# RWAlgorithms/ConjugateGradientOptim.jl

Hardware: AMD Instinct MI355X
Metric: CG iterations/sec at n=1e8 (outer iterations of minimizeobjective, PR-CG) (higher is better)
Workload: dtype f64

## Files before the change

conjugategradientoptim.jl_amd/_lib.py:

```python
from __future__ import annotations

import ctypes as C
import os
import subprocess

_PKG = os.path.dirname(os.path.abspath(__file__))
LIB_PATH = os.environ.get("CGO_LIB_PATH") or os.path.join(_PKG, "lib", "libcgo_hip.so")
CSRC = os.path.join(_PKG, "csrc")

dp = C.POINTER(C.c_double)
i64p = C.POINTER(C.c_int64)


class BetaConfig(C.Structure):
    _fields_ = [("kind", C.c_int32), ("lbfgs_m", C.c_int32), ("mu", C.c_double)]


class CGConfigC(C.Structure):
    _fields_ = [("eps", C.c_double), ("beta", BetaConfig), ("max_iters", C.c_int64),
                ("verbose", C.c_int32), ("trace_enabled", C.c_int32)]


class LSConfigC(C.Structure):
    _fields_ = [("kind", C.c_int32), ("cond_kind", C.c_int32), ("c1", C.c_double),
# ... 24 lines not shown

class BatchPolicyC(C.Structure):
    _fields_ = [("size", C.c_int32), ("rows", C.c_int32), ("reserved", C.c_int32 * 6)]


class SolverPolicyC(C.Structure):
    _fields_ = [("size", C.c_int32), ("points", C.c_int32), ("resident", C.c_int32), ("controller_depth", C.c_int32),
                ("controller_graph", C.c_int32), ("controller_fused", C.c_int32), ("stored_gradient", C.c_int32),
                ("fused_tail", C.c_int32), ("strict_tail", C.c_int32), ("placement_search", C.c_int32),
                ("placement_stages", C.c_int32), ("placement_max_bytes", C.c_int64), ("lbfgs_form", C.c_int32),
                ("lbfgs_fuse_grad", C.c_int32), ("lbfgs_fuse_trial", C.c_int32), ("lse_fixed_reference", C.c_int32),
                ("resident_points", C.c_int32), ("resident_chunk", C.c_int32), ("hbm_stream_bytes", C.c_double),
                ("reserved", C.c_int32 * 8)]


class LbfgsProbeC(C.Structure):
    _fields_ = [("pass_", C.c_int32), ("slot", C.c_int32), ("count", C.c_int32), ("list", C.c_int32 * 16),
                ("a", C.c_double), ("a_s", C.c_double), ("a_trial", C.c_double), ("cg", C.c_double), ("M", C.c_double),
                ("S", C.c_double), ("cy", C.c_double * 16), ("cs", C.c_double * 16), ("deferred_push", C.c_int32),
                ("lite_slot", C.c_int32), ("a_lite", C.c_double), ("a_s_lite", C.c_double), ("M_lite", C.c_double),
                ("S_lite", C.c_double), ("loop_mode", C.c_int32), ("final_step", C.c_int32), ("apply_scale", C.c_int32),
                ("k", C.c_int32), ("q_from_g", C.c_int32), ("v_ring", C.c_int32), ("v_slot", C.c_int32), ("w_ring", C.c_int32),
                ("w_slot", C.c_int32), ("dot_count", C.c_int32), ("rho", C.c_double), ("scale", C.c_double),
                ("dot_host", C.c_double), ("dots", dp), ("alpha", C.c_double * 64), ("spec_check", C.c_int32),
                ("spec_slot", C.c_int32), ("spec_count", C.c_int32), ("spec_list", C.c_int32 * 16), ("spec_a_x", C.c_double),
                ("spec_a_s", C.c_double), ("spec_ok", C.c_int32), ("new_in_list", C.c_int32), ("sums_len", C.c_int32),
                ("reserved", C.c_int32), ("gram", C.c_double * 85), ("sums", C.c_double * 64), ("symbol", C.c_char * 256)]


class ResidentPassC(C.Structure):
    _fields_ = [("kind", C.c_int32), ("k", C.c_int32), ("a", C.c_double * 7), ("a_acc", C.c_double), ("beta", C.c_double)]


class ResidentPassOutC(C.Structure):
    _fields_ = [("ts", (C.c_double * 7) * 7), ("gu", C.c_double), ("uu", C.c_double), ("width", C.c_int64)]


class ResidentProbeC(C.Structure):
    _fields_ = [("npass", C.c_int32), ("reserved", C.c_int32), ("pass_", ResidentPassC * 32), ("grid", C.c_int32),
                ("points", C.c_int32), ("chunk", C.c_int64), ("round0", C.c_int64), ("err_word", C.c_uint32),
                ("wrote_back", C.c_int32), ("out", ResidentPassOutC * 32), ("symbol", C.c_char * 128)]


class CtlStateC(C.Structure):
    _fields_ = [("f_x", C.c_double), ("gg", C.c_double), ("a_acc", C.c_double), ("beta", C.c_double), ("a", C.c_double * 7),
                ("npts", C.c_int32), ("go", C.c_int32), ("it", C.c_int64)]


class CtlArgsC(C.Structure):
    _fields_ = [("a_acc", C.c_double), ("beta", C.c_double), ("a", C.c_double * 7), ("go", C.c_int64)]


class CtlRecordC(C.Structure):
    _fields_ = [("sums", C.c_double * 56), ("a_acc", C.c_double), ("beta", C.c_double), ("a", C.c_double * 7),
                ("npts", C.c_int32), ("accepted", C.c_int32), ("xwait", C.c_int64)]


class ArmedProbeC(C.Structure):
    _fields_ = [("rounds", C.c_int32), ("form", C.c_int32), ("use_eps", C.c_int32), ("reserved", C.c_int32),
                ("max_iters", C.c_int64), ("eps", C.c_double), ("st", CtlStateC), ("row", C.c_double * 56),
                ("width", C.c_int32), ("maxp", C.c_int32), ("round_out", C.c_uint64), ("st_out", CtlStateC),
                ("args_out", CtlArgsC), ("out_dev", C.c_double * 56), ("rec", CtlRecordC * 32), ("symbol", C.c_char * 4096)]


class BatchPassC(C.Structure):
    _fields_ = [("kind", C.c_int32), ("k", C.c_int32), ("a", C.c_double * 7), ("a_acc", C.c_double), ("beta", C.c_double),
                ("co_set", C.c_int32), ("co_count", C.c_int32), ("co_gamma", C.c_double), ("co_cy", C.c_double * 10),
                ("co_cs", C.c_double * 10)]


class BatchPassOutC(C.Structure):
    _fields_ = [("ts", (C.c_double * 7) * 7), ("gu", C.c_double), ("uu", C.c_double), ("width", C.c_int64), ("stored", C.c_int64)]


class BatchProbeC(C.Structure):
    _fields_ = [("tier", C.c_int32), ("obj_kind", C.c_int32), ("m", C.c_int32), ("n_params", C.c_int32), ("model", C.c_void_p),
                ("n", C.c_int64), ("batch", C.c_int64), ("x", dp), ("u", dp), ("params", dp * 4), ("scalars", dp),
                ("skip", C.POINTER(C.c_uint8)), ("S", dp), ("Y", dp), ("qn", C.c_void_p), ("npass", C.c_int32),
                ("reserved", C.c_int32), ("pass_", BatchPassC * 32), ("rows", dp), ("out", C.POINTER(BatchPassOutC)),
                ("x_out", dp), ("u_out", dp), ("g_out", dp), ("S_out", dp), ("Y_out", dp), ("qn_out", C.c_void_p),
                ("reason", C.POINTER(C.c_int32)), ("done", i64p), ("passes", i64p), ("points", C.c_int32),
                ("reserved2", C.c_int32), ("ld", C.c_int64), ("symbol", C.c_char * 128)]


ALLGATHER_FN = C.CFUNCTYPE(C.c_int, C.c_void_p, dp, dp, C.c_int32)
FDF_FN = C.CFUNCTYPE(C.c_double, C.c_void_p, dp, dp, C.c_int64)

_vp = C.c_void_p
_pp = C.POINTER(C.c_void_p)
SIGNATURES = {
    "cgo_version": (C.c_int, []),
    "cgo_build_id": (C.c_char_p, []),
    "cgo_last_error": (C.c_char_p, []),
    "cgo_status_name": (C.c_char_p, [C.c_int32]),
    "cgo_device_count": (C.c_int, [C.POINTER(C.c_int32)]),
    "cgo_check_cg_config": (C.c_int, [C.POINTER(CGConfigC)]),
    "cgo_check_ls_config": (C.c_int, [C.POINTER(LSConfigC)]),
    "cgo_ctx_create": (C.c_int, [C.c_int32, _pp]),
    "cgo_solver_policy_init": (None, [C.POINTER(SolverPolicyC)]),
    "cgo_ctx_set_default_policy": (C.c_int, [_vp, C.POINTER(SolverPolicyC)]),
    "cgo_solver_get_policy": (C.c_int, [_vp, C.POINTER(SolverPolicyC)]),
    "cgo_solver_create_ex": (C.c_int, [_vp, _vp, C.POINTER(CGConfigC), C.POINTER(LSConfigC), C.POINTER(SolverPolicyC), _pp]),
    "cgo_solver_create_sys_ex": (C.c_int, [_vp, _vp, C.POINTER(CGConfigC), C.POINTER(LSSConfigC), C.POINTER(SolverPolicyC), _pp]),
    "cgo_ctx_destroy": (C.c_int, [_vp]),
    "cgo_comm_unique_id": (C.c_int, [_vp]),
    "cgo_ctx_set_comm_rccl": (C.c_int, [_vp, C.c_int32, C.c_int32, _vp]),
    "cgo_ctx_set_comm_callback": (C.c_int, [_vp, C.c_int32, C.c_int32, ALLGATHER_FN, _vp]),
    "cgo_ctx_set_comm_shm": (C.c_int, [_vp, C.c_int32, C.c_int32, C.c_char_p, C.c_int32]),
    "cgo_shm_unlink": (C.c_int, [C.c_char_p]),
    "cgo_ctx_comm_info": (C.c_int, [_vp, C.POINTER(C.c_int32), C.POINTER(C.c_int32), C.POINTER(C.c_int32), C.POINTER(C.c_int32)]),
    "cgo_ctx_exchange_stats": (C.c_int, [_vp, i64p, dp, dp, C.c_int32]),
    "cgo_ctx_comm_connect_devices": (C.c_int, [_vp, C.POINTER(C.c_int32)]),
    "cgo_rccl_available": (C.c_int, []),
    "cgo_objective_create": (C.c_int, [_vp, C.c_int32, C.c_int64, C.c_int64, C.c_int64, _pp]),
    "cgo_objective_create_from_source": (C.c_int, [_vp, C.c_char_p, C.c_int32, C.c_int64, C.c_int64, C.c_int64, _pp]),
    "cgo_objective_create_callback": (C.c_int, [_vp, FDF_FN, _vp, C.c_int64, C.c_int64, C.c_int64, _pp]),
    "cgo_objective_destroy": (C.c_int, [_vp]),
    "cgo_objective_create_from_source_ex": (C.c_int, [_vp, C.c_char_p, C.c_int32, C.c_int64, C.c_int64, C.c_int64, _pp]),
    "cgo_objective_num_params": (C.c_int, [_vp, C.POINTER(C.c_int32)]),
    "cgo_objective_set_param_host": (C.c_int, [_vp, C.c_int32, dp]),
    "cgo_objective_set_param_device": (C.c_int, [_vp, C.c_int32, _vp]),
    "cgo_objective_fill_param": (C.c_int, [_vp, C.c_int32, C.c_int32, C.c_uint64, C.c_double, C.c_double]),
    "cgo_objective_set_scalar": (C.c_int, [_vp, C.c_int32, C.c_double]),
    "cgo_objective_set_cost_class": (C.c_int, [_vp, C.c_int32]),
    "cgo_objective_eval_host": (C.c_int, [_vp, dp, dp, dp]),
    "cgo_solver_create": (C.c_int, [_vp, _vp, C.POINTER(CGConfigC), C.POINTER(LSConfigC), _pp]),
    "cgo_solver_destroy": (C.c_int, [_vp]),
    "cgo_solver_set_x0_host": (C.c_int, [_vp, dp]),
    "cgo_solver_set_x0_fill": (C.c_int, [_vp, C.c_int32, C.c_uint64, C.c_double, C.c_double]),
    "cgo_solver_set_x0_device": (C.c_int, [_vp, _vp]),
    "cgo_solver_results_device": (C.c_int, [_vp, _vp, _vp]),
    "cgo_solver_start": (C.c_int, [_vp]),
    "cgo_solver_iterate": (C.c_int, [_vp, C.c_int64, C.POINTER(C.c_int32)]),
    "cgo_solver_results": (C.c_int, [_vp, C.POINTER(ResultsC)]),
    "cgo_solver_trial_log": (C.c_int, [_vp, C.c_int64, dp, dp, dp, i64p]),
    "cgo_solver_profile_enable": (C.c_int, [_vp, C.c_int32]),
    "cgo_solver_profile_reset": (C.c_int, [_vp]),
    "cgo_solver_profile_get": (C.c_int, [_vp, C.c_int32, i64p, dp, dp]),
    "cgo_kernel_kind_name": (C.c_char_p, [C.c_int32]),
    "cgo_solver_kernel_family": (C.c_char_p, [_vp]),
    "cgo_solver_controller_launches": (C.c_int64, [_vp]),
    "cgo_solver_resident_stats": (C.c_int, [_vp, i64p, i64p, i64p]),
    "cgo_solver_lbfgs_stats": (C.c_int, [_vp, i64p, i64p, i64p]),
    "cgo_num_kernel_kinds": (C.c_int, []),
    "cgo_solver_set_lazy_direction": (C.c_int, [_vp, C.c_int32]),
    "cgo_solver_probe_set_beta_prev": (C.c_int, [_vp, C.c_double]),
    "cgo_solver_set_replay_depth": (C.c_int, [_vp, C.c_int32]),
    "cgo_solver_set_lean_sums": (C.c_int, [_vp, C.c_int32]),
    "cgo_solver_set_path_prediction": (C.c_int, [_vp, C.c_int32]),
    "cgo_solver_path_stats": (C.c_int, [_vp, i64p, i64p, i64p, i64p]),
    "cgo_solver_probe_set_path": (C.c_int, [_vp, C.c_int32]),
    "cgo_solver_debug_set_path_skew": (C.c_int, [_vp, C.c_double]),
    "cgo_solver_probe_set_replay": (C.c_int, [_vp, C.c_int32, dp, dp]),
    "cgo_solver_kernel_symbol": (C.c_int, [_vp, C.c_int32, C.c_char_p, C.c_int32]),
    "cgo_evalwolfeconditions": (C.c_int, [C.POINTER(LSConfigC), C.c_double, C.c_double, C.c_double, C.c_double,
                                          C.c_double, C.c_double, C.POINTER(C.c_int32), C.POINTER(C.c_int32)]),
    "cgo_evalbacktrackcondition": (C.c_int, [C.POINTER(LSConfigC), C.c_double, C.c_double, C.c_double, C.c_double,
                                             C.POINTER(C.c_int32)]),
    "cgo_check_lss_config": (C.c_int, [C.POINTER(LSSConfigC)]),
    "cgo_lss_default_max_iters": (C.c_int64, [C.c_double]),
    "cgo_solver_create_sys": (C.c_int, [_vp, _vp, C.POINTER(CGConfigC), C.POINTER(LSSConfigC), _pp]),
    "cgo_solvesystem": (C.c_int, [_vp, _vp, dp, C.POINTER(CGConfigC), C.POINTER(LSSConfigC), C.POINTER(ResultsC)]),
    "cgo_minimize": (C.c_int, [_vp, _vp, dp, C.POINTER(CGConfigC), C.POINTER(LSConfigC), C.POINTER(ResultsC)]),
    "cgo_minimize_rerun": (C.c_int, [_vp, _vp, dp, C.POINTER(CGConfigC), C.POINTER(LSConfigC),
                                     C.POINTER(CGConfigC), C.POINTER(LSConfigC), C.c_int32,
                                     C.POINTER(ResultsC), C.POINTER(C.c_int32)]),
    "cgo_minimize_batch": (C.c_int, [_vp, C.c_int32, C.c_int64, C.c_int64, dp, dp, C.POINTER(CGConfigC), C.POINTER(LSConfigC),
                                     C.c_int64, C.POINTER(BatchResultsC)]),
    "cgo_batch_max_n": (C.c_int64, [_vp, C.c_int32]),
    "cgo_minimize_batch_obj": (C.c_int, [_vp, _vp, C.c_int64, dp, C.POINTER(dp), C.c_int32, C.POINTER(CGConfigC), C.POINTER(LSConfigC),
                                         C.c_int64, C.POINTER(BatchResultsC)]),
    "cgo_batch_max_n_obj": (C.c_int64, [_vp]),
    "cgo_batch_open": (C.c_int, [_vp, _vp, C.c_int64, C.POINTER(dp), C.c_int32, C.POINTER(_vp)]),
    "cgo_batch_solve": (C.c_int, [_vp, dp, dp, C.POINTER(C.c_uint8), C.POINTER(CGConfigC), C.POINTER(LSConfigC), C.c_int64,
                                  C.POINTER(BatchResultsC)]),
    "cgo_batch_close": (C.c_int, [_vp]),
    "cgo_batch_policy_init": (None, [C.POINTER(BatchPolicyC)]),
    "cgo_minimize_batch_ex": (C.c_int, [_vp, C.c_int32, C.c_int64, C.c_int64, dp, dp, C.POINTER(CGConfigC), C.POINTER(LSConfigC),
                                        C.c_int64, C.POINTER(BatchPolicyC), C.POINTER(BatchResultsC), C.POINTER(C.c_int32)]),
    "cgo_minimize_batch_obj_ex": (C.c_int, [_vp, _vp, C.c_int64, dp, C.POINTER(dp), C.c_int32, C.POINTER(CGConfigC), C.POINTER(LSConfigC),
                                            C.c_int64, C.POINTER(BatchPolicyC), C.POINTER(BatchResultsC), C.POINTER(C.c_int32)]),
    "cgo_batch_open_ex": (C.c_int, [_vp, _vp, C.c_int64, C.POINTER(dp), C.c_int32, C.POINTER(BatchPolicyC), C.POINTER(_vp)]),
    "cgo_batch_rows": (C.c_int, [_vp, C.POINTER(C.c_int32)]),
    "cgo_batch_max_n_ex": (C.c_int64, [_vp, C.c_int32, C.POINTER(BatchPolicyC)]),
    "cgo_batch_max_n_obj_ex": (C.c_int64, [_vp, C.POINTER(BatchPolicyC)]),
    "cgo_batch_rows_shape": (None, [C.POINTER(C.c_int32), C.POINTER(C.c_int32)]),
    "cgo_minimize_batch_lbfgs": (C.c_int, [_vp, C.c_int32, C.c_int64, C.c_int64, dp, dp, C.POINTER(CGConfigC), C.POINTER(LSConfigC),
                                           C.c_int64, C.POINTER(BatchResultsC)]),
    "cgo_batch_lbfgs_max_m": (C.c_int32, []),
    "cgo_batch_lbfgs_max_n": (C.c_int64, [_vp, C.c_int32]),
    "cgo_batch_lbfgs_shape": (None, [C.POINTER(C.c_int32), C.POINTER(C.c_int32)]),
    "cgo_minimize_batch_lbfgs_obj": (C.c_int, [_vp, _vp, C.c_int64, dp, C.POINTER(dp), C.c_int32, dp, C.POINTER(CGConfigC), C.POINTER(LSConfigC),
                                               C.c_int64, C.POINTER(BatchResultsC)]),
    "cgo_batch_lbfgs_max_n_obj": (C.c_int64, [_vp]),
    "cgo_batch_lbfgs_shape_obj": (None, [C.c_int32, C.POINTER(C.c_int32), C.POINTER(C.c_int32)]),
    "cgo_minimize_batch_lbfgs_ex": (C.c_int, [_vp, C.c_int32, C.c_int64, C.c_int64, dp, dp, C.POINTER(CGConfigC), C.POINTER(LSConfigC),
                                              C.c_int64, C.POINTER(BatchPolicyC), C.POINTER(BatchResultsC), C.POINTER(C.c_int32)]),
    "cgo_minimize_batch_lbfgs_obj_ex": (C.c_int, [_vp, _vp, C.c_int64, dp, C.POINTER(dp), C.c_int32, dp, C.POINTER(CGConfigC),
                                                  C.POINTER(LSConfigC), C.c_int64, C.POINTER(BatchPolicyC), C.POINTER(BatchResultsC),
                                                  C.POINTER(C.c_int32)]),
    "cgo_batch_lbfgs_max_n_ex": (C.c_int64, [_vp, C.c_int32, C.c_int32, C.POINTER(BatchPolicyC)]),
    "cgo_batch_lbfgs_max_n_obj_ex": (C.c_int64, [_vp, C.c_int32, C.POINTER(BatchPolicyC)]),
    "cgo_batch_lbfgs_lds_rows": (C.c_int32, [C.c_int32, C.c_int32]),
    "cgo_batch_lbfgs_lds_shape": (None, [C.c_int32, C.POINTER(C.c_int32), C.POINTER(C.c_int32)]),
    "cgo_batch_lbfgs_open": (C.c_int, [_vp, _vp, C.c_int64, C.POINTER(dp), C.c_int32, C.c_int32, C.POINTER(BatchPolicyC), C.POINTER(_vp)]),
    "cgo_batch_lbfgs_solve": (C.c_int, [_vp, dp, dp, C.POINTER(C.c_uint8), C.POINTER(CGConfigC), C.POINTER(LSConfigC), C.c_int64,
                                        C.POINTER(BatchResultsC)]),
    "cgo_batch_lbfgs_m": (C.c_int, [_vp, C.POINTER(C.c_int32)]),
    "cgo_batch_probe": (C.c_int, [_vp, C.POINTER(BatchProbeC)]),
    "cgo_batch_probe_qn_bytes": (C.c_int64, []),
    "cgo_stop_status": (C.c_int32, [C.c_int64, C.c_int64, C.c_double, C.c_double, C.c_double, C.c_double, i64p]),
    "cgo_kernel_dir": (C.c_int, [_vp, dp, dp, C.c_double, C.c_int64, dp]),
    "cgo_kernel_beta_partials": (C.c_int, [_vp, dp, dp, dp, C.c_int64, dp]),
    "cgo_getbeta": (C.c_int, [_vp, C.POINTER(BetaConfig), dp, dp, dp, C.c_int64, dp]),
    "cgo_kernel_trial": (C.c_int, [_vp, dp, dp, C.c_double, dp, dp]),
    "cgo_bench_kernel": (C.c_int, [_vp, _vp, C.c_int32, C.c_int64, C.c_int32, dp, dp]),
    "cgo_bench_stream_mix": (C.c_int, [_vp, C.c_int64, C.c_int32, dp, dp]),
    "cgo_solver_placement_info": (C.c_int, [_vp, dp, dp, C.POINTER(C.c_int32)]),
    "cgo_solver_probe_launch": (C.c_int, [_vp, C.c_int32, C.c_int32, C.c_double, C.c_double, dp, C.c_int32, dp, dp, dp,
                                          dp, C.c_int32, C.POINTER(C.c_int32), dp, dp, dp, C.c_char_p, C.c_int32]),
    "cgo_solver_probe_lbfgs": (C.c_int, [_vp, C.POINTER(LbfgsProbeC)] + [dp] * 13),
    "cgo_solver_probe_resident": (C.c_int, [_vp, C.POINTER(ResidentProbeC), dp, dp, dp, C.c_int64, dp, dp]),
    "cgo_solver_probe_armed": (C.c_int, [_vp, C.POINTER(ArmedProbeC), dp, dp, dp, dp]),
}


class CgoError(RuntimeError):
    def __init__(self, code: int, msg: str):
        super().__init__(f"[cgo error {code}] {msg}")
        self.code = code
        self.msg = msg


def build(force: bool = False) -> str:
    if force:
        subprocess.run(["make", "-C", CSRC, "clean", "-s"], check=True)
    subprocess.run(["make", "-C", CSRC, "-s", "-j4"], check=True)
    if not os.path.exists(LIB_PATH):
        raise RuntimeError("hipcc build did not produce " + LIB_PATH)
    return LIB_PATH


_lib = None


def lib() -> C.CDLL:
    global _lib
    if _lib is None:
        if not os.path.exists(LIB_PATH):
            raise ImportError(
                f"{LIB_PATH} is missing: build it with `make -C {CSRC}` "
                "(or __graft_entry__.build()). There is no CPU fallback.")
        L = C.CDLL(LIB_PATH, mode=C.RTLD_GLOBAL)
        for name, (res, args) in SIGNATURES.items():
            fn = getattr(L, name)
            fn.restype = res
            fn.argtypes = args
        _lib = L
    return _lib


def check(rc: int) -> None:
    if rc != 0:
        msg = lib().cgo_last_error()
        text = msg.decode("utf-8", "replace") if msg else ""
        if rc == 1 and text.startswith("AssertionError"):
            raise AssertionError(text[len("AssertionError: "):])
        raise CgoError(rc, text)
```

conjugategradientoptim.jl_amd/api.py:

```python
from __future__ import annotations

import ctypes as C
import math
import re
from dataclasses import dataclass, field
from typing import List, Optional, Sequence, Union

import numpy as np

from . import _lib
from ._lib import BetaConfig, CGConfigC, LSConfigC, LSSConfigC, ResultsC, check, dp, i64p



class TraceTrait:
    pass


class EnableTrace(TraceTrait):
    def __repr__(self):
        return "EnableTrace()"


class DisableTrace(TraceTrait):
# ... 488 lines not shown
    slots = _param_list(param)
    if slots is not None:
        assert len(slots) <= MAX_PARAM_SLOTS, f"at most {MAX_PARAM_SLOTS} parameter vectors"
        o = DeviceObjective("user", n, ctx, source=source, n_params=len(slots))
        for j, p in enumerate(slots):
            if p is not None:
                o.set_param(np.asarray(p, dtype=np.float64), slot=j)
        param = None
    else:
        o = DeviceObjective("user", n, ctx, source=source, has_param=param is not None)
    if param is not None:
        o.set_param(np.asarray(param, dtype=np.float64))
    if cheap:
        check(_lib.lib().cgo_objective_set_cost_class(o._h, 1))
    return o


def Booth(ctx: Optional[Context] = None) -> DeviceObjective:
    return DeviceObjective("booth", 2, ctx)


def _dev_ptr(t, n: int):
    if t is None:
        return None
    if isinstance(t, int):
        return C.c_void_p(t)
    if hasattr(t, "data_ptr"):
        import torch
        if t.dtype != torch.float64 or not t.is_contiguous() or t.numel() != n or not t.is_cuda:
            raise ValueError(f"device vector must be a contiguous float64 GPU tensor of {n} elements")
        return C.c_void_p(t.data_ptr())
    raise TypeError("expected a torch.Tensor on the GPU or a raw device pointer")


LBFGS_FORMS = {"auto": 0, "one_pass": 1, "one_pass_own_update": 2, "gram": 3, "two_loop": 4}


@dataclass
class SolverPolicy:
    points: Optional[int] = None
    resident: Optional[bool] = None
    controller_depth: Optional[int] = None
    controller_graph: Optional[bool] = None
    controller_fused: Optional[bool] = None
    stored_gradient: Optional[bool] = None
    fused_tail: Optional[bool] = None
    strict_tail: Optional[bool] = None
    placement_search: Optional[bool] = None
    placement_stages: Optional[int] = None
    placement_max_bytes: Optional[int] = None
    lbfgs_form: Optional[str] = None
    lbfgs_fuse_grad: Optional[bool] = None
    lbfgs_fuse_trial: Optional[bool] = None
    lse_fixed_reference: Optional[bool] = None
    resident_points: Optional[int] = None
    resident_chunk: Optional[int] = None
    hbm_stream_bytes: Optional[float] = None

    def _c(self) -> "_lib.SolverPolicyC":
        c = _lib.SolverPolicyC()
        _lib.lib().cgo_solver_policy_init(C.byref(c))
        tri = lambda v: -1 if v is None else (1 if v else 0)
        c.points = self.points or 0
        c.resident = tri(self.resident)
        c.controller_depth = -1 if self.controller_depth is None else int(self.controller_depth)
        c.controller_graph, c.controller_fused = tri(self.controller_graph), tri(self.controller_fused)
        c.stored_gradient = 1 if self.stored_gradient else 0
        c.fused_tail, c.strict_tail = tri(self.fused_tail), tri(self.strict_tail)
        c.placement_search = tri(self.placement_search)
        c.placement_stages = self.placement_stages or 0
        c.placement_max_bytes = int(self.placement_max_bytes or 0)
        c.lbfgs_form = LBFGS_FORMS[self.lbfgs_form or "auto"]
        c.lbfgs_fuse_grad, c.lbfgs_fuse_trial = tri(self.lbfgs_fuse_grad), tri(self.lbfgs_fuse_trial)
        c.lse_fixed_reference = tri(self.lse_fixed_reference)
        c.resident_points = self.resident_points or 0
        c.resident_chunk = self.resident_chunk or 0
        c.hbm_stream_bytes = float(self.hbm_stream_bytes or 0.0)
        return c


class Solver:
    def __init__(self, fdf: DeviceObjective, config: CGConfig, linesearch_config: LineSearchConfig,
                 policy: Optional[SolverPolicy] = None):
        if not isinstance(fdf, DeviceObjective):
            raise TypeError(
                "fdf! must be an objective descriptor: a device objective (QuadDiag, RosenbrockPaired, Booth, "
                "ElementwiseObjective, ...) or HostObjective(closure, n) — there is no CPU solver path in this package")
        self.obj, self.config, self.ls = fdf, config, linesearch_config
        self._cfg_c, self._ls_c = config._c(), linesearch_config._c()
        self._h = C.c_void_p()
        create = (_lib.lib().cgo_solver_create_sys_ex if isinstance(linesearch_config, LinesearchSolveSys)
                  else _lib.lib().cgo_solver_create_ex)
        self._pol_c = policy._c() if policy is not None else None
        check(create(fdf.ctx._h, fdf._h, C.byref(self._cfg_c), C.byref(self._ls_c),
                     C.byref(self._pol_c) if self._pol_c is not None else None, C.byref(self._h)))

    def policy(self) -> dict:
        c = _lib.SolverPolicyC()
        check(_lib.lib().cgo_solver_get_policy(self._h, C.byref(c)))
        return {n: getattr(c, n) for n, _ in c._fields_ if n not in ("size", "reserved")}

    def set_x0(self, x_initial_global: np.ndarray):
        loc = self.obj.local(np.asarray(x_initial_global, dtype=np.float64))
        check(_lib.lib().cgo_solver_set_x0_host(self._h, loc.ctypes.data_as(dp)))

    def set_x0_fill(self, fill: str, lo: float, hi: float = 0.0, seed: int = 0):
        check(_lib.lib().cgo_solver_set_x0_fill(self._h, FILL_KINDS[fill], seed, lo, hi))

    def set_x0_device(self, x0):
        check(_lib.lib().cgo_solver_set_x0_device(self._h, _dev_ptr(x0, self.obj.n_local)))

    def results_device(self, minimizer=None, gradient=None):
        check(_lib.lib().cgo_solver_results_device(self._h, _dev_ptr(minimizer, self.obj.n_local), _dev_ptr(gradient, self.obj.n_local)))

    def start(self):
        check(_lib.lib().cgo_solver_start(self._h))

    def iterate(self, iters: int) -> bool:
        fin = C.c_int32(0)
        check(_lib.lib().cgo_solver_iterate(self._h, iters, C.byref(fin)))
        return bool(fin.value)

    def enable_trial_log(self):
        cnt = C.c_int64()
        check(_lib.lib().cgo_solver_trial_log(self._h, -1, None, None, None, C.byref(cnt)))

    def trial_log(self):
        cnt = C.c_int64()
        check(_lib.lib().cgo_solver_trial_log(self._h, 0, None, None, None, C.byref(cnt)))
        k = cnt.value
        a, p, d = np.zeros(max(k, 1)), np.zeros(max(k, 1)), np.zeros(max(k, 1))
        check(_lib.lib().cgo_solver_trial_log(self._h, k, a.ctypes.data_as(dp), p.ctypes.data_as(dp),
                                              d.ctypes.data_as(dp), C.byref(cnt)))
        return a[:k], p[:k], d[:k]

    def kernel_family(self) -> str:
        return _lib.lib().cgo_solver_kernel_family(self._h).decode()

    def kernel_symbol(self, kind_name: str) -> str:
        L = _lib.lib()
        buf = C.create_string_buffer(200)
        for k in range(L.cgo_num_kernel_kinds()):
            if L.cgo_kernel_kind_name(k).decode() == kind_name:
                check(L.cgo_solver_kernel_symbol(self._h, k, buf, 200))
                return buf.value.decode()
        return ""

    def set_lazy_direction(self, on: bool = True):
        check(_lib.lib().cgo_solver_set_lazy_direction(self._h, int(bool(on))))

    def set_replay_depth(self, d: int):
        check(_lib.lib().cgo_solver_set_replay_depth(self._h, int(d)))

    def set_lean_sums(self, on: bool):
        check(_lib.lib().cgo_solver_set_lean_sums(self._h, int(bool(on))))

    def set_path_prediction(self, on: bool):
        check(_lib.lib().cgo_solver_set_path_prediction(self._h, int(bool(on))))

    def path_stats(self):
        by = (C.c_int64 * 8)()
        p, t, m = C.c_int64(0), C.c_int64(0), C.c_int64(0)
        check(_lib.lib().cgo_solver_path_stats(self._h, by, C.byref(p), C.byref(t), C.byref(m)))
        return dict(by_nact={j: int(by[j]) for j in (1, 2, 3, 4, 5, 7)}, predicted=p.value, tree=t.value, misses=m.value)

    def debug_set_path_skew(self, factor: float):
        check(_lib.lib().cgo_solver_debug_set_path_skew(self._h, float(factor)))

    def probe_launch(self, kind_name: str, variant: int, a_acc: float, beta: float, a: Sequence[float], x, u=None, aux=None,
                     beta_prev: Optional[float] = None, replay: Optional[Sequence] = None, path_nact: Optional[int] = None):
        L = _lib.lib()
        kk = [L.cgo_kernel_kind_name(k).decode() for k in range(L.cgo_num_kernel_kinds())].index(kind_name)
        if beta_prev is not None:
            check(L.cgo_solver_probe_set_beta_prev(self._h, float(beta_prev)))
        if replay is not None:
            ra = np.ascontiguousarray([p[0] for p in replay], dtype=np.float64)
            rb = np.ascontiguousarray([p[1] for p in replay], dtype=np.float64)
            check(L.cgo_solver_probe_set_replay(self._h, len(replay), ra.ctypes.data_as(dp), rb.ctypes.data_as(dp)))
        if path_nact is not None:
            check(L.cgo_solver_probe_set_path(self._h, int(path_nact)))
        n = self.obj.n_local
        vec = lambda v: None if v is None else np.ascontiguousarray(v, dtype=np.float64)
        x, u, aux = vec(x), vec(u), vec(aux)
        for v in (x, u, aux):
            if v is not None and v.size != n:
                raise ValueError(f"probe vectors hold n_local = {n} elements")
        av = np.ascontiguousarray(a, dtype=np.float64) if len(a) else np.zeros(1)
        sums, ln = np.full(64, np.nan), C.c_int32(0)
        xo, uo, go = np.empty(n), np.empty(n), np.empty(n)
        sym = C.create_string_buffer(200)
        ptr = lambda v: None if v is None else v.ctypes.data_as(dp)
        check(L.cgo_solver_probe_launch(self._h, kk, int(variant), float(a_acc), float(beta), ptr(av), len(a), ptr(x), ptr(u),
                                        ptr(aux), ptr(sums), 64, C.byref(ln), ptr(xo), ptr(uo), ptr(go), sym, 200))
        return dict(sums=sums[:ln.value].copy(), x=xo, u=uo, g=go, symbol=sym.value.decode())

    LBFGS_PASSES = ("push", "push_gram", "direction_gram", "direction_trial", "push_lite", "loop")

    def probe_lbfgs(self, pass_name: str, x=None, u=None, g=None, gt=None, S=None, Y=None, **kw):
        n = self.obj.n_local
        P = self._cfg_c.beta.lbfgs_m + 1
        vec = lambda v: None if v is None else np.ascontiguousarray(v, dtype=np.float64)
        x, u, g, gt = vec(x), vec(u), vec(g), vec(gt)
        for v in (x, u, g, gt):
            if v is not None and v.size != n:
                raise ValueError(f"probe vectors hold n_local = {n} elements")
        S = None if S is None else np.ascontiguousarray(S, dtype=np.float64).reshape(P, n)
        Y = None if Y is None else np.ascontiguousarray(Y, dtype=np.float64).reshape(P, n)
        p = _lib.LbfgsProbeC()
        p.pass_ = self.LBFGS_PASSES.index(pass_name)
        dots = None
        for key, val in kw.items():
            if key in ("list", "spec_list"):
                getattr(p, key)[:len(val)] = [int(v) for v in val]
                setattr(p, "count" if key == "list" else "spec_count", len(val))
            elif key in ("cy", "cs", "alpha"):
                getattr(p, key)[:len(val)] = [float(v) for v in val]
            elif key == "stats":
                p.M, p.S = float(val[0]), float(val[1])
            elif key == "dots":
                dots = np.ascontiguousarray(val, dtype=np.float64).reshape(-1, 10)
                p.dots, p.dot_count = dots.ctypes.data_as(dp), dots.shape[0]
            else:
                if not hasattr(p, key):
                    raise TypeError(f"probe_lbfgs: no field {key}")
                setattr(p, key, val)
        outs = {k: np.full(n, np.nan) for k in ("x", "xo", "u", "g", "gt")}
        So, Yo = np.full((P, n), np.nan), np.full((P, n), np.nan)
        ptr = lambda v: None if v is None else v.ctypes.data_as(dp)
        check(_lib.lib().cgo_solver_probe_lbfgs(self._h, C.byref(p), ptr(x), ptr(u), ptr(g), ptr(gt), ptr(S), ptr(Y),
                                                *[ptr(outs[k]) for k in ("x", "xo", "u", "g", "gt")], ptr(So), ptr(Yo)))
        sym = p.symbol.decode()
        return dict(sums=np.array(p.sums[:p.sums_len]), S=So, Y=Yo, alpha=np.array(p.alpha[:]), symbols=sym.split(" + ") if sym else [],
                    new_in_list=p.new_in_list, spec_ok=bool(p.spec_ok),
                    gram=np.array(p.gram[:5 + 5 * p.spec_count]) if p.spec_ok else None, **outs)

    def probe_resident(self, script, x, u):
        n = self.obj.n_local
        x, u = np.ascontiguousarray(x, dtype=np.float64), np.ascontiguousarray(u, dtype=np.float64)
        if x.size != n or u.size != n:
            raise ValueError(f"probe vectors hold n_local = {n} elements")
        p = _lib.ResidentProbeC()
        if len(script) > 32:
            raise ValueError("probe_resident: at most 32 passes")
        p.npass = len(script)
        for q, item in enumerate(script):
            c = p.pass_[q]
            if item[0] == "trial":
                c.kind, a = 0, item[1]
            elif item[0] == "accept_dir_trial":
                c.kind, c.a_acc, c.beta, a = 1, float(item[1]), float(item[2]), item[3]
            else:
                raise ValueError(f"probe_resident: no pass kind {item[0]!r}")
            if len(a) > 7:
                raise ValueError("probe_resident: at most 7 trial steps")
            c.k = len(a)
            c.a[:len(a)] = [float(v) for v in a]
        rows = np.full((max(p.npass, 1), 256, 56), np.nan)
        xo, uo = np.empty(n), np.empty(n)
        check(_lib.lib().cgo_solver_probe_resident(self._h, C.byref(p), x.ctypes.data_as(dp), u.ctypes.data_as(dp),
                                                   rows.ctypes.data_as(dp), rows.size, xo.ctypes.data_as(dp), uo.ctypes.data_as(dp)))
        g = p.grid
        got = rows.ravel()[:p.npass * g * 56].reshape(p.npass, g, 56)
        outs, rws, tails = [], [], []
        for q in range(p.npass):
            w = int(p.out[q].width)
            rws.append(got[q, :, :w].copy()); tails.append(got[q, :, w:].copy())
            outs.append(dict(ts=np.array([list(r) for r in p.out[q].ts]), gu=p.out[q].gu, uu=p.out[q].uu))
        return dict(rows=rws, tail=tails, out=outs, grid=g, chunk=p.chunk, points=p.points, round0=p.round0,
                    wrote_back=bool(p.wrote_back), x=xo, u=uo, symbol=p.symbol.decode())

    ARMED_FORMS = ("rounds", "graph", "controller")

    def probe_armed(self, state, rounds=1, form="rounds", x=None, u=None, max_iters=1 << 40, eps=None, row=None):
        n = self.obj.n_local
        p = _lib.ArmedProbeC()
        p.rounds, p.form = int(rounds), self.ARMED_FORMS.index(form)
        p.max_iters = int(max_iters)
        if eps is not None:
            p.use_eps, p.eps = 1, float(eps)
        a = [float(v) for v in state["a"]]
        if not 1 <= len(a) <= 7:
            raise ValueError("probe_armed: 1 to 7 trial steps")
        p.st.f_x, p.st.gg = float(state["f_x"]), float(state["gg"])
        p.st.a_acc, p.st.beta = float(state["a_acc"]), float(state["beta"])
        p.st.a[:] = a + [a[-1]] * (7 - len(a))
        p.st.npts, p.st.go, p.st.it = int(state.get("npts", len(a))), int(state.get("go", 1)), int(state.get("it", 0))
        if row is not None:
            r = [float(v) for v in row]
            p.row[:len(r)] = r
        vec = lambda v: None if v is None else np.ascontiguousarray(v, dtype=np.float64)
        x, u = vec(x), vec(u)
        for v in (x, u):
            if v is not None and v.size != n:
                raise ValueError(f"probe vectors hold n_local = {n} elements")
        xo, uo = np.full(n, np.nan), np.full(n, np.nan)
        ptr = lambda v: None if v is None else v.ctypes.data_as(dp)
        check(_lib.lib().cgo_solver_probe_armed(self._h, C.byref(p), ptr(x), ptr(u), ptr(xo), ptr(uo)))

        def block(c, names):
            d = {k: (np.array(getattr(c, k)[:]) if k in ("a", "sums") else getattr(c, k)) for k in names}
            d["bytes"] = bytes(c)
            return d
        recs = [block(p.rec[r], ("sums", "a_acc", "beta", "a", "npts", "accepted", "xwait")) for r in range(p.rounds)]
        sym = p.symbol.decode()
        return dict(records=recs, st=block(p.st_out, ("f_x", "gg", "a_acc", "beta", "a", "npts", "go", "it")),
                    args=block(p.args_out, ("a_acc", "beta", "a", "go")), round=int(p.round_out), out_dev=np.array(p.out_dev[:]),
                    width=p.width, maxp=p.maxp, x=xo, u=uo, symbols=sym.split(" + ") if sym else [])

    def placement_info(self):
        a, b, c = C.c_double(), C.c_double(), C.c_int32()
        check(_lib.lib().cgo_solver_placement_info(self._h, C.byref(a), C.byref(b), C.byref(c)))
        return a.value, b.value, c.value

    def controller_launches(self) -> int:
        return int(_lib.lib().cgo_solver_controller_launches(self._h))

    def resident_stats(self):
        a, b, c = C.c_int64(), C.c_int64(), C.c_int64()
        check(_lib.lib().cgo_solver_resident_stats(self._h, C.byref(a), C.byref(b), C.byref(c)))
        self.resident_gave_up = c.value
        return a.value, b.value

    def lbfgs_stats(self):
        a, b, c = C.c_int64(), C.c_int64(), C.c_int64()
        check(_lib.lib().cgo_solver_lbfgs_stats(self._h, C.byref(a), C.byref(b), C.byref(c)))
        return a.value, b.value, c.value

    def profile(self, on: bool = True):
        check(_lib.lib().cgo_solver_profile_enable(self._h, int(on)))

    def profile_reset(self):
        check(_lib.lib().cgo_solver_profile_reset(self._h))

# ... 995 lines not shown
```

conjugategradientoptim.jl_amd/csrc/cgo_backend_cg.hip:

```cpp
#include "cgo_backend_internal.hpp"

#include "cgo_kernels.hip.hpp"
#include "cgo_kernels_cg.hip.hpp"
#include "cgo_kernels_cg_path.hip.hpp"
#include "cgo_kernels_chain.hip.hpp"
#include "cgo_kernels_lse.hip.hpp"
#include "cgo_kernels_resident.hip.hpp"

namespace cgo {

using namespace dev;

double bytes_r(int obj_kind, int mode, int64_t n, int n_params) {
    const int p = std::max(obj_kind == CGO_OBJ_QUAD_DIAG ? 1 : 0, n_params);
    return 8.0 * (double)n * (double)r_vectors(mode, p);
}

template <int N> using Pts = std::integral_constant<int, N>;
template <int MAXPTS, class F>
static inline void with_points(int npts, F f) {
    static_assert(MAXPTS == 1 || MAXPTS == 3 || MAXPTS == 5 || MAXPTS == 7, "a launch evaluates 1, 3, 5 or 7 trial points");
    if constexpr (MAXPTS >= 3) { if (npts == 3) return f(Pts<3>{}); }
    if constexpr (MAXPTS >= 5) { if (npts == 5) return f(Pts<5>{}); }
    if constexpr (MAXPTS >= 7) { if (npts != 1) return f(Pts<7>{}); }
    return f(Pts<1>{});
}

template <class Obj, bool BIG>
static int launch_cg(int mode, int npts, const RParams &P, int grid, hipStream_t st) {
#define ROW(MODE, MAXPTS) if (mode == (MODE) && P.tail.ctl) { with_points<MAXPTS>(npts, [&](auto n) { k_cg_armed<Obj, decltype(n)::value><<<grid, BLOCK, 0, st>>>(P); }); return 0; }
    CGO_CG_ARMED_ROWS(ROW)
#undef ROW
    switch (mode) {
#define ROW(MODE, MAXPTS) case (MODE): with_points<MAXPTS>(npts, [&](auto n) { k_cg<Obj, (MODE), decltype(n)::value, BIG><<<grid, BLOCK, 0, st>>>(P); }); return 0;
    CGO_CG_ROWS(ROW)
#undef ROW
    default: break;
    }
    if constexpr (BIG) {
        switch (mode) {
#define ROW(MODE, MAXPTS) case (MODE): with_points<MAXPTS>(npts, [&](auto n) { k_cg<Obj, (MODE), decltype(n)::value, true><<<grid, BLOCK, 0, st>>>(P); }); return 0;
        CGO_CG_LAG_ROWS(ROW)
        CGO_CG_REPLAY_ROWS(ROW)
        CGO_CG_LEAN_ROWS(ROW)
#undef ROW
        default: break;
        }
    }
    return -1;
}

template <class Obj>
static int launch_cg_path(int mode, int nact, const RParams &P, int grid, hipStream_t st) {
#define ROW(MODE, NACT) if (mode == (MODE) && nact == (NACT)) { k_cg_path<Obj, (MODE), (NACT), true><<<grid, BLOCK, 0, st>>>(P); return 0; }
    CGO_CG_PATH_ROWS(ROW)
#undef ROW
    return -1;
}
static inline bool path_row(int mode, int nact) {
#define ROW(MODE, NACT) if (mode == (MODE) && nact == (NACT)) return true;
    CGO_CG_PATH_ROWS(ROW)
#undef ROW
    return false;
}
static inline bool path_objective(int kind) {
#define ROW(KIND, T) if (kind == KIND) return true;
    CGO_OBJ_CURV_ROWS(ROW)
#undef ROW
    return false;
}
bool HipBackend::path_rows() const {
    if (!path_on_ || !path_objective(obj_->kind) || replay_depth_ < 2 || !lazy_eligible()) return false;
    const int mode_n = r_mode_of(KK_ACCEPT_TRIAL_NOSTORE), mode_s = R_REPLAY | R_ADT;
    return path_row(mode_n | lean_for(mode_n), MAXP) && path_row(mode_s | lean_for(mode_s), MAXP);
}

static inline bool lean_row(int mode) {
#define ROW(MODE, MAXPTS) if (mode == (MODE)) return true;
    CGO_CG_LEAN_ROWS(ROW)
#undef ROW
    return false;
}
int HipBackend::lean_for(int mode) const { return (lean_bits_ && lean_row(mode | lean_bits_)) ? lean_bits_ : 0; }

void unpack_r(const double *s, int k, Scal *out, bool dir, int npts) {
    if (npts == 0) npts = npts_for(k);
    for (int j = 0; j < k; ++j) {
        const double *q = s + RS_PER_POINT * j;
        out[j].f = q[RS_F]; out[j].gtu = q[RS_GTU]; out[j].gtgt = q[RS_GTGT]; out[j].gtg = q[RS_GTG];
        out[j].yy = q[RS_YY]; out[j].uy = q[RS_UY]; out[j].ygt = q[RS_YGT];
    }
    if (dir) { out[0].gu = s[RS_PER_POINT * npts]; out[0].uu = s[RS_PER_POINT * npts + 1]; }
}

static inline int chain_npts(int mode, int npts) { return ((mode & R_TRIAL) && npts >= 3) ? 3 : 1; }

RPlan HipBackend::r_plan(int mode, int npts) const {
    const double bytes = bytes_r(obj_->kind, mode, obj_->n_local, obj_->nparams());
    const bool big = r_big_only(mode) || bytes > big_bytes(r_read_only(mode));
    return {big, big ? GRID_BIG : grid_cg(obj_->n_local, chain() ? 1 : npts), chain() ? chain_npts(mode, npts) : npts, bytes};
}
bool HipBackend::adt_is_big() const { return bytes_r(obj_->kind, R_ADT, obj_->n_local, obj_->nparams()) > big_bytes(false); }

int HipBackend::launch_r(int kk, int mode, double a_acc, double beta, const double *a, int k, bool fetch,
                         double *sums) {
    if (int rc = pipe_drain()) return rc;
    pipe_streak_ = 0;
    if (u_lag_ && !(mode & R_ULAG)) {
        if (r_reads_u(mode)) { if (int rc = materialize_u()) return rc; }
        else if (mode & (R_INIT | R_RESET)) u_lag_ = false;
    }
    if (rep_n_ > 0 && !(mode & R_REPLAY)) { if (int rc = materialize_lag()) return rc; }
    RPlan plan;
    const int npts = path_nact_ ? MAXP : npts_for(k);
    if (int rc = launch_r_kernel(kk, mode, a_acc, beta, a, k, npts, nullptr, &plan)) return rc;
    const int grid = plan.grid;
    total_launches_++;
    const bool has_sums = r_has_sums(mode);
    const bool fused = has_sums && tail_fused(grid);
    if (has_sums && chain()) {
        const bool three = plan.npts == 3;
        const int W = three ? NRC3 : NRC, edge = three ? RC3_EDGE : RC_EDGE, nsums = three ? NR : NR1;
        if (!fused) { if (int rc = finalize_rows(ctx_, grid, W, true)) return rc; }
        const int Wd = ctx_->world(), me = ctx_->rank();
        std::vector<double> raw((size_t)W * Wd);
        double all[NRC3];
        if (int rc = fetch_sums(ctx_, all, MERGE_SUM, W, raw.data())) return rc;
        if (sums) std::memcpy(sums, all, sizeof(double) * nsums);
        if (me > 0) {
            const double *e = raw.data() + (size_t)(me - 1) * W + edge + 4;
            halo_xl_[0] = e[0]; halo_xl_[1] = e[1]; halo_ul_[0] = e[2]; halo_ul_[1] = e[3];
        }
        if (me < Wd - 1) {
            const double *e = raw.data() + (size_t)(me + 1) * W + edge;
            halo_xr_[0] = e[0]; halo_xr_[1] = e[1]; halo_ur_[0] = e[2]; halo_ur_[1] = e[3];
        }
        if (probe_) { std::memcpy(probe_row_, all, sizeof(double) * W); probe_len_ = W; }
    } else if (has_sums) {
        if (!fused) { if (int rc = finalize_rows(ctx_, grid, rows_for(npts), true)) return rc; }
        if (fetch) {
            if (int rc = fetch_sums(ctx_, sums, MERGE_SUM, rows_for(npts))) return rc;
        }
        if (probe_ && fetch) { std::memcpy(probe_row_, sums, sizeof(double) * rows_for(npts)); probe_len_ = rows_for(npts); }
    }
    if (prof_on_) prof_commit(kk, plan.bytes);
    return CGO_OK;
}

bool HipBackend::lazy_eligible() const {
    if (!lazy_on_ || !rmode_ || chain() || sys_on_ || probe_ || pingpong_ == 1) return false;
    bool aot = false;
#define ROW(KIND, T) aot = aot || obj_->kind == KIND;
    CGO_OBJ_ROWS(ROW)
#undef ROW
    if (!aot) return false;
    if (const char *e = getenv("CGO_PINGPONG")) { if (e[0] == '1') return false; }
    if (ctl_depth() > 0) return false;
    return adt_is_big() && r_plan(R_TRIAL, 1).big;
}

int HipBackend::materialize_u() {
    if (!u_lag_) return CGO_OK;
    const int64_t asked = total_launches_;
    const int nact = path_nact_;
    path_nact_ = 0;
    const int rc = launch_rk(KK_MATERIALIZE_U, 0.0, 0.0, nullptr, 0, false, nullptr);
    path_nact_ = nact;
    total_launches_ = asked;
    if (rc) return rc;
    u_lag_ = false;
    return CGO_OK;
}

int HipBackend::materialize_lag() {
    if (int rc = materialize_u()) return rc;
    if (rep_n_ == 0) return CGO_OK;
    const int64_t asked = total_launches_;
    const int nact = path_nact_;
    path_nact_ = 0;
    const int rc = launch_rk(KK_MATERIALIZE_XU, 0.0, 0.0, nullptr, 0, false, nullptr);
    path_nact_ = nact;
    total_launches_ = asked;
    if (rc) return rc;
    rep_n_ = 0;
    return CGO_OK;
}

int HipBackend::set_replay_depth_now(int d) {
    if (d < 1 || d > RMAX + 1) { set_error("replay depth: 1 … 8"); return CGO_EINVAL; }
    if (d != replay_depth_) { if (int rc = materialize_lag()) return rc; }
    replay_depth_ = d;
    return CGO_OK;
}

void HipBackend::set_probe_replay(int nrep, const double *a, const double *beta) {
    probe_rep_n_ = std::max(0, std::min(nrep, (int)RMAX));
    for (int j = 0; j < probe_rep_n_; ++j) { probe_rep_a_[j] = a[j]; probe_rep_b_[j] = beta[j]; }
}

int HipBackend::accept_dir_trial_r(double a_acc, double beta, const double *a, int k, double *s) {
    if (!lazy_eligible()) return launch_rk(KK_ACCEPT_DIR_TRIAL, a_acc, beta, a, k, true, s);
    if (replay_depth_ >= 2) {
        if (int rc = materialize_u()) return rc;
        if (rep_n_ < replay_depth_ - 1 && rep_n_ < RMAX) {
            const int mode_n = r_mode_of(KK_ACCEPT_TRIAL_NOSTORE);
            if (int rc = launch_r(KK_ACCEPT_TRIAL_NOSTORE, mode_n | lean_for(mode_n), a_acc, beta, a, k, true, s)) return rc;
            if (path_nact_) { path_last_n_ = path_nact_; path_count_[path_nact_]++; }
            rep_a_[rep_n_] = a_acc; rep_b_[rep_n_] = beta; rep_n_++;
            return CGO_OK;
        }
        const int mode_s = R_REPLAY | R_ADT;
        if (int rc = launch_r(KK_ACCEPT_DIR_TRIAL, mode_s | lean_for(mode_s), a_acc, beta, a, k, true, s)) return rc;
        if (path_nact_) { path_last_s_ = path_nact_; path_count_[path_nact_]++; }
        rep_n_ = 0;
        return CGO_OK;
    }
    if (!u_lag_) {
        if (int rc = launch_rk(KK_ACCEPT_TRIAL_LAZY, a_acc, beta, a, k, true, s)) return rc;
        u_lag_ = true; beta_lag_ = beta;
        return CGO_OK;
    }
    if (int rc = launch_r(KK_ACCEPT_DIR_TRIAL, R_ULAG | R_ADT, a_acc, beta, a, k, true, s)) return rc;
    u_lag_ = false;
    return CGO_OK;
}
int HipBackend::trial_r(const double *a, int k, double *s) {
    if (rep_n_ > 0 && lazy_eligible()) return launch_r(KK_TRIAL, R_REPLAY | R_TRIAL, 0, 0, a, k, true, s);
    if (u_lag_ && lazy_eligible()) return launch_r(KK_TRIAL, R_ULAG | R_TRIAL, 0, 0, a, k, true, s);
    return launch_rk(KK_TRIAL, 0, 0, a, k, true, s);
}

bool HipBackend::pipe_fused(int grid) const {
    return tail_fused(grid) && obj_->kind != CGO_OBJ_USER && !chain() && ctl_fused_;
}
bool HipBackend::tail_fused(int grid) const {
    static const int cap = [] { const char *e = getenv("CGO_FUSED_TAIL_MAX_GRID"); int v = e ? atoi(e) : 0; return v > 0 ? v : 1024; }();
    return ctx_->fused_tail && grid <= cap && grid <= TAIL_GROUP * TAIL_GROUP;
}
Tail HipBackend::make_tail(bool on) {
    Tail t{};
    if (!on) return t;
    ctx_->seq++;
    t.partials2 = ctx_->partials2_f; t.tickets = ctx_->tickets; t.out = ctx_->out_dev;
    t.strict = ctx_->tail_strict ? 1 : 0;
    ctx_->pub_target(&t.host_out, &t.host_seq);
    ctx_->pub_checked = (t.host_out != nullptr) && !ctx_->tail_strict;
    t.seq = ctx_->seq;
    return t;
}

int HipBackend::launch_r_kernel(int kk, int mode, double a_acc, double beta, const double *a, int k, int npts,
                                const CtlArgs *ctl, RPlan *plan_out) {
    HIPCHK(hipSetDevice(ctx_->device));
    if (obj_->unset_slot() >= 0) return param_unset_error(obj_->unset_slot());
    const int64_t n = obj_->n_local;
    if (mode & (R_GRAD | R_GRADT)) { if (int rc = ensure_ga()) return rc; }
    const bool has_sums = r_has_sums(mode);
    const RPlan plan = *plan_out = r_plan(mode, npts);
    const bool big = plan.big; const int grid = plan.grid;
    last_mode_ = mode; last_npts_ = plan.npts; last_big_ = big; last_nact_ = path_nact_;
    if (path_nact_ && (chain() || !big || ctl || !path_row(mode, path_nact_) || !path_objective(obj_->kind))) { set_error("internal: not a path row"); return CGO_EINVAL; }
    if (chain()) {
        if (int rc = prof_begin(kk)) return rc;
        if (int rc = launch_chain_kernel(mode, a_acc, beta, a, k, plan.npts, big, grid, make_tail(has_sums && !ctl && tail_fused(grid)))) return rc;
        return prof_end();
    }
    RParams P;
    P.x = xc_; P.u = uc_; P.gout = ga_.p; obj_->param_args(P); P.n = n;
    P.xo = xc_; P.uo = uc_;
    P.a_acc = a_acc; P.beta = beta; P.s0 = obj_->s0; P.partials = ctx_->partials;
    P.beta_prev = beta_lag_;
    P.nrep = (mode & R_REPLAY) ? rep_n_ : 0;
    for (int j = 0; j < RMAX; ++j) { P.ra[j] = j < P.nrep ? rep_a_[j] : 0.0; P.rb[j] = j < P.nrep ? rep_b_[j] : 0.0; }
    P.ctl = ctl;
    P.x2 = xn_;
    for (int j = 0; j < MAXP; ++j) P.a[j] = (a && j < k) ? a[j] : ((a && k > 0) ? a[k - 1] : 0.0);
    P.tail = make_tail(has_sums && !ctl && tail_fused(grid));
    if (ctl && pipe_fused(grid)) {
        P.tail.partials2 = ctx_->partials2_f; P.tail.tickets = ctx_->tickets; P.tail.out = ctx_->out_dev;
        P.tail.strict = ctx_->tail_strict ? 1 : 0;
        P.tail.ctl = ctl_dev_; P.tail.ctl_rec = ctl_rec_; P.tail.ctl_seq = ctl_seq_;
        if (!ctx_->single()) {
            P.tail.xw = ctx_->world(); P.tail.xme = ctx_->rank(); P.tail.xseq0 = epoch_ << 40;
            for (int r = 0; r < P.tail.xw && r < 8; ++r) P.tail.xmail[r] = ctx_->comm->dev_mailbox(r);
        }
    }
    if (P.tail.tickets) P.partials = ctx_->partials_f;
    const bool wr_x = r_writes_x(mode), wr_u = r_writes_u(mode);
    const bool pp = big && !ctl && (wr_x || wr_u) && !(mode & R_PROJ) && pingpong_ready();
    if (pp && wr_x) P.xo = xalt_;
    if (pp && wr_u) P.uo = ualt_;
    if (mode == R_PROJ && !xn_) { set_error("internal: no second iterate buffer"); return CGO_ESTATE; }
    hipStream_t st = ctx_->stream;
    if (int rc = prof_begin(kk)) return rc;
    int r = -2;
    if (path_nact_) {
        switch (obj_->kind) {
#define ROW(KIND, T) case KIND: r = launch_cg_path<T>(mode, path_nact_, P, grid, st); break;
        CGO_OBJ_CURV_ROWS(ROW)
#undef ROW
        default: break;
        }
    } else switch (obj_->kind) {
#define ROW(KIND, T) case KIND: r = big ? launch_cg<T, true>(mode, npts, P, grid, st) : launch_cg<T, false>(mode, npts, P, grid, st); break;
    CGO_OBJ_ROWS(ROW)
#undef ROW
    case CGO_OBJ_USER:
        if (!obj_->rtc) { set_error("user objective has no compiled module"); return CGO_EINVAL; }
        if (r_big_only(mode)) break;
        if (int rc = launch_module(obj_->rtc->cg(mode, npts, big), &P, grid, st)) return rc;
        r = 0;
        break;
    default: break;
    }
    if (r) { set_error("internal: CG kernel mode not instantiated"); return CGO_EINVAL; }
    HIPCHK(hipGetLastError());
    if (pp && wr_x) std::swap(xc_, xalt_);
    if (pp && wr_u) std::swap(uc_, ualt_);
    return prof_end();
}

template <bool BIG>
static int launch_chain(int mode, int npts, const ChainParams &P, int grid, hipStream_t st) {
    switch (mode) {
#define ROW(MODE, MAXPTS) case (MODE): with_points<MAXPTS>(npts, [&](auto n) { k_chain<(MODE), decltype(n)::value, BIG><<<grid, BLOCK, 0, st>>>(P); }); return 0;
    CGO_CHAIN_ROWS(ROW)
#undef ROW
    default: return -1;
    }
}

int HipBackend::launch_chain_kernel(int mode, double a_acc, double beta, const double *a, int k, int npts, bool big, int grid, const Tail &tail) {
    ChainParams P;
    P.tail = tail;
    for (int j = 0; j < 3; ++j) P.a[j] = (a && j < k) ? a[j] : ((a && k > 0) ? a[k - 1] : 0.0);
    P.x = xc_; P.u = uc_; P.xo = xc_; P.uo = uc_; P.gout = ga_.p;
    P.odd = (int)(obj_->n_local & 1);
    P.n = obj_->n_local + P.odd; P.a_acc = a_acc; P.beta = beta; P.partials = tail.tickets ? ctx_->partials_f : ctx_->partials;
    for (int j = 0; j < 2; ++j) { P.hxl[j] = halo_xl_[j]; P.hul[j] = halo_ul_[j]; P.hxr[j] = halo_xr_[j]; P.hur[j] = halo_ur_[j]; }
    P.has_left = obj_->offset > 0 ? 1 : 0;
    P.has_right = obj_->offset + obj_->n_local < obj_->n_global ? 1 : 0;
    const bool wr_x = r_writes_x(mode), wr_u = r_writes_u(mode);
    if (wr_x) P.xo = xalt_;
    if (wr_u) P.uo = ualt_;
    const int r = big ? launch_chain<true>(mode, npts, P, grid, ctx_->stream) : launch_chain<false>(mode, npts, P, grid, ctx_->stream);
    if (r) { set_error("internal: chain kernel mode not instantiated"); return CGO_EINVAL; }
    HIPCHK(hipGetLastError());
    if (wr_x) std::swap(xc_, xalt_);
    if (wr_u) std::swap(uc_, ualt_);
    return CGO_OK;
}

std::string HipBackend::r_symbol(int mode, int npts, bool big, int nact) const {
    char buf[160];
    if (chain()) snprintf(buf, sizeof buf, "k_chain<%d, %d, %s>", mode, npts, big ? "true" : "false");
    else if (nact) snprintf(buf, sizeof buf, "k_cg_path<%s, %d, %d, true>", obj_tname(), mode, nact);
    else snprintf(buf, sizeof buf, "k_cg<%s, %d, %d, %s>", obj_tname(), mode, npts, big ? "true" : "false");
    return buf;
}

std::string HipBackend::kernel_symbol(int kk) const {
    if (!rmode_) {
        if (obj_->two_phase() || kk == KK_LBFGS_PUSH || kk == KK_LBFGS_LOOP || kk == KK_LBFGS_FINAL) return lbfgs_symbol(kk);
        const int mode = fused_mode(kk);
        return mode < 0 ? "" : fused_symbol(obj_tname(), mode, is_big(obj_->kind, mode, obj_->n_local, obj_->nparams(), pol_.hbm_stream_bytes));
    }
    const RKind *rk = r_kind(kk);
    if (!rk) return "";
    int mode = rk->mode;
    const bool lazy = lazy_eligible();
    switch (kk) {
    case KK_ACCEPT_DIR_TRIAL: if (lazy) mode |= replay_depth_ >= 2 ? R_REPLAY : R_ULAG; break;
    case KK_ACCEPT_TRIAL_LAZY: case KK_MATERIALIZE_U: if (!lazy || replay_depth_ >= 2) return ""; break;
    case KK_ACCEPT_TRIAL_NOSTORE: case KK_MATERIALIZE_XU: if (!lazy || replay_depth_ < 2) return ""; break;
    default: break;
    }
    const RPlan plan = r_plan(mode, rk->pts == PTS_ONE ? 1 : npts_for(rk->pts == PTS_MAX ? max_points() : std::min(max_points(), 3)));
    if ((mode & R_REPLAY) && (mode & R_ACCEPT)) mode |= lean_for(mode);
    if ((mode & R_REPLAY) && (mode & R_ACCEPT) && path_rows()) {
        const int last = kk == KK_ACCEPT_TRIAL_NOSTORE ? path_last_n_ : path_last_s_;
        return r_symbol(mode, plan.npts, plan.big, last ? last : MAXP);
    }
    return r_symbol(mode, plan.npts, plan.big);
}


__global__ void k_ctl_init(CtlDev *d, const CtlConfig cfg, const CtlState st, unsigned long long round) {
    d->cfg = cfg;
    d->st = st;
    d->round = round;
    d->args = ctl_args_of(st);
}



template <int N, int THREADS>
__global__ __launch_bounds__(THREADS) void k_finalize_ctl(const double *partials, int rows, double *out, CtlDev *d,
                                                          CtlRecord *rec_ring, unsigned long long *seq_ring) {
    constexpr int G = BLOCK / N;
    constexpr int WD = sizeof(CtlDev) / 8, WR = sizeof(CtlRecord) / 8;
    __shared__ double sm[G][N];
    __shared__ double fin[CTL_NSUMS];
    __shared__ CtlDev sd;
    __shared__ CtlRecord sr;
    const int tid = threadIdx.x;
    if (tid < WD) ((unsigned long long *)&sd)[tid] = ((const unsigned long long *)d)[tid];
    if (tid < CTL_NSUMS) fin[tid] = 0.0;
    __syncthreads();
    const bool go = sd.st.go != 0;
    const unsigned long long round = sd.round, seq = round + 1;
    CtlRecord *rec_host = rec_ring + (round % PIPE_RING);
    unsigned long long *seq_host = seq_ring + (round % PIPE_RING);
    if (go) {
        if (tid < G * N) {
            double t = 0.0;
            const long long total = (long long)rows * N;
            for (long long i = tid; i < total; i += G * N) t += partials[i];
            sm[tid / N][tid % N] = t;
        }
        __syncthreads();
        if (tid < N) {
            double v = 0.0;
#pragma unroll
            for (int g = 0; g < G; ++g) v += sm[g][tid];
            out[tid] = v;
            fin[tid] = v;
        }
        __syncthreads();
    }
    if (tid == 0) {
        if (go) {
            ctl_step(sd.cfg, sd.st, fin, sr);
            sd.args = ctl_args_of(sd.st);
        } else ctl_idle_record(sr);
        sd.round = round + 1;
    }
    __syncthreads();
    if (go && tid < WD) ((unsigned long long *)d)[tid] = ((const unsigned long long *)&sd)[tid];
    if (!go && tid == 0) d->round = round + 1;
    if (tid < WR) {
        ((unsigned long long *)rec_host)[tid] = ((const unsigned long long *)&sr)[tid];
        __threadfence_system();
    }
    __syncthreads();
    if (tid == 0) __hip_atomic_store(seq_host, seq, __ATOMIC_RELEASE, __HIP_MEMORY_SCOPE_SYSTEM);
}

int HipBackend::ctl_depth() const {
    if (!(rmode_ && ctx_->host_publish && !obj_->two_phase())) return 0;
    if (ctx_->single()) return ctl_depth_;
    if (!ctx_->dev_exchange() || ctx_->force_gather) return 0;
    return (!adt_is_big() && pipe_fused(grid_cg(obj_->n_local, policy_points()))) ? ctl_depth_ : 0;
}

int HipBackend::pipe_alloc() {
    if (ctl_dev_) return CGO_OK;
    HIPCHK(hipMalloc(&ctl_dev_, sizeof(CtlDev)));
    HIPCHK(hipHostMalloc((void **)&ctl_rec_, sizeof(CtlRecord) * PIPE_RING, hipHostMallocDefault));
    HIPCHK(hipHostMalloc((void **)&ctl_seq_, sizeof(unsigned long long) * PIPE_RING, hipHostMallocDefault));
    std::memset(ctl_rec_, 0, sizeof(CtlRecord) * PIPE_RING);
    std::memset(ctl_seq_, 0, sizeof(unsigned long long) * PIPE_RING);
    pipe_prof_.assign(PIPE_RING, {-1, 0u});
    return CGO_OK;
}

int HipBackend::prepare_controller() {
    if (ctl_depth() <= 0) return CGO_OK;
    if (int rc = pipe_alloc()) return rc;
    if (obj_->unset_slot() >= 0) return CGO_OK;
    HIPCHK(hipSetDevice(ctx_->device));
    CtlConfig cc{};
    CtlState st{};
    st.go = 0;
    pipe_npts_ = max_points();
    k_ctl_init<<<1, 1, 0, ctx_->stream>>>((CtlDev *)ctl_dev_, cc, st, pipe_enq_);
    HIPCHK(hipGetLastError());
    if (int rc = pipe_enqueue_round()) return rc;
    return pipe_drain();
}

int HipBackend::pipe_round_kernels() {
    RPlan plan;
    const int npts = pipe_npts_, ns = rows_for(npts);
    CtlDev *d = (CtlDev *)ctl_dev_;
    if (int rc = launch_r_kernel(KK_ACCEPT_DIR_TRIAL, R_ADT, 0.0, 0.0, nullptr, 0, npts, &d->args, &plan)) return rc;
    const int grid = plan.grid;
    pipe_checked_ = pipe_fused(grid) && !ctx_->tail_strict;
    if (pipe_fused(grid)) {
        if (probe_) probe_note(nullptr, 0, "k_cg_armed<%s, %d>", obj_tname(), last_npts_);
        return CGO_OK;
    }
    if (probe_) probe_note(nullptr, 0, "%s", r_symbol(last_mode_, last_npts_, last_big_).c_str());
    hipStream_t st = ctx_->stream;
    const double *src = ctx_->partials;
    int nrows = grid;
    if (grid > TAIL_GROUP) {
        const int nb = (grid + TAIL_GROUP - 1) / TAIL_GROUP;
        with_width<NR, NR5, NR7, NS>(ns, true, [&](auto w) { k_finalize_t<decltype(w)::value, BLOCK><<<nb, BLOCK, 0, st>>>(ctx_->partials, TAIL_GROUP, grid, ctx_->partials2, nullptr, nullptr, 0); });
        HIPCHK(hipGetLastError());
        if (probe_) probe_note(nullptr, 0, "k_finalize_t<%d>", ns);
        src = ctx_->partials2;
        nrows = nb;
    }
    return pipe_finalize_ctl(src, nrows, ns);
}

int HipBackend::pipe_finalize_ctl(const double *src, int nrows, int ns) {
    CtlDev *d = (CtlDev *)ctl_dev_;
    CtlRecord *rec = (CtlRecord *)ctl_rec_;
    hipStream_t st = ctx_->stream;
    with_width<NR, NR5, NR7, NS>(ns, true, [&](auto w) { constexpr int N = decltype(w)::value, T = N == NS ? BLOCK : 768; k_finalize_ctl<N, T><<<1, T, 0, st>>>(src, nrows, ctx_->out_dev, d, rec, ctl_seq_); });
    HIPCHK(hipGetLastError());
    if (probe_) probe_note(nullptr, 0, "k_finalize_ctl<%d>", ns);
    return CGO_OK;
}

int HipBackend::pipe_enqueue_round() {
    if (int rc = pipe_round_kernels()) return rc;
    const int idx = (int)(pipe_enq_ % PIPE_RING);
    pipe_prof_[idx] = {prof_cur_ ? ring_used_ - 1 : -1, prof_gen_};
    prof_cur_ = false;
    pipe_enq_++;
    return CGO_OK;
}

int HipBackend::pipe_launch_graph(int rounds) {
    HIPCHK(hipSetDevice(ctx_->device));
    PipeGraph *g = nullptr;
    for (auto &c : graphs_)
        if (c.rounds == rounds && c.npts == pipe_npts_ && c.x == xc_ && c.u == uc_ && c.p0 == obj_->p[0].p && c.n == obj_->n_local) { g = &c; break; }
    if (!g) {
        hipStream_t st = ctx_->stream;
        hipGraph_t graph = nullptr;
        capturing_ = true;
        const size_t syms0 = probe_syms_.size();
// ... 38 lines not shown
}

int HipBackend::pipe_wait(unsigned long long id, CtlRecord &rec) {
    const int idx = (int)(id % PIPE_RING);
    if (pipe_checked_) {
        static_assert(sizeof(CtlRecord) % 8 == 0, "record = 8-byte words");
        constexpr int WR = (int)(sizeof(CtlRecord) / 8);
        double words[WR];
        if (int rc = wait_checked(ctx_, ctl_seq_ + idx, id + 1, reinterpret_cast<const double *>(ctl_rec_) + (size_t)idx * WR, WR, words)) return rc;
        std::memcpy(&rec, words, sizeof(CtlRecord));
        if (rec.npts >= 0 && !ctx_->single()) {
            ctx_->xch_count++; ctx_->xch_dev_ms += (double)rec.xwait * 1e-5; ctx_->xch_dev_n++;
        }
        return CGO_OK;
    }
    if (int rc = wait_word(ctx_, ctl_seq_ + idx, id + 1)) return rc;
    rec = ((CtlRecord *)ctl_rec_)[idx];
    return CGO_OK;
}

int HipBackend::pipe_drain() {
    while (pipe_done_ < pipe_enq_) {
        CtlRecord rec;
        if (int rc = pipe_wait(pipe_done_, rec)) return rc;
        pipe_done_++;
        if (rec.npts >= 0) {
            set_error("internal: the on-device controller ran a launch the host state machine did not ask for");
            return CGO_ESTATE;
        }
    }
    return CGO_OK;
}

int HipBackend::accept_dir_trial_ctl(const CtlConfig &cc, const CtlState &s0, int64_t rounds, Scal *out) {
    if (ctl_depth() <= 0) return accept_dir_trial(s0.a_acc, s0.beta, s0.a, s0.npts, out);
    if (int rc = pipe_alloc()) return rc;
    const int64_t ahead = std::min<int64_t>(std::min<int64_t>(ctl_depth_, pipe_streak_), rounds - 1);
    if (pipe_done_ == pipe_enq_) {
        if (ahead <= 0) { pipe_streak_++; return accept_dir_trial_keep_streak(s0, out); }
        HIPCHK(hipSetDevice(ctx_->device));
        pipe_npts_ = cc.maxp;
        k_ctl_init<<<1, 1, 0, ctx_->stream>>>((CtlDev *)ctl_dev_, cc, s0, pipe_enq_);
        HIPCHK(hipGetLastError());
        pipe_stopped_ = false;
        if (int rc = pipe_enqueue(1 + ahead)) return rc;
    }
    CtlRecord rec;
    const unsigned long long id = pipe_done_;
    if (int rc = pipe_wait(id, rec)) return rc;
    pipe_done_++;
    if (rec.npts < 0) {
        if (int rc = pipe_drain()) return rc;
        pipe_streak_++;
        return accept_dir_trial_keep_streak(s0, out);
    }
    if (std::memcmp(&rec.a_acc, &s0.a_acc, 8) || std::memcmp(&rec.beta, &s0.beta, 8) || rec.npts != s0.npts ||
        std::memcmp(rec.a, s0.a, 8 * (size_t)s0.npts)) {
        set_error("internal: the on-device controller and the host state machine disagree on a launch");
        return CGO_ESTATE;
    }
    unpack_r(rec.sums, s0.npts, out, true, pipe_npts_);
    total_launches_++;
    pipe_served_++;
    pipe_streak_++;
    const auto &pp = pipe_prof_[(int)(id % PIPE_RING)];
    if (prof_on_) {
        prof_cnt_[KK_ACCEPT_DIR_TRIAL]++;
        prof_bytes_[KK_ACCEPT_DIR_TRIAL] = bytes_r(obj_->kind, R_ADT, obj_->n_local, obj_->nparams());
        if (pp.first >= 0 && pp.second == prof_gen_ && pp.first < ring_used_) {
            ring_[pp.first].kk = KK_ACCEPT_DIR_TRIAL;
            ring_[pp.first].bytes = prof_bytes_[KK_ACCEPT_DIR_TRIAL];
        }
    }
    if (!rec.accepted) pipe_stopped_ = true;
    if (!pipe_stopped_) {
        const int64_t want = std::min<int64_t>(std::min<int64_t>(ctl_depth_, pipe_streak_), rounds - 1);
        const int64_t have = (int64_t)(pipe_enq_ - pipe_done_);
        if (have < want && (want - have >= (want + 1) / 2 || have == 0))
            if (int rc = pipe_enqueue(want - have)) return rc;
    }
    return CGO_OK;
}

int HipBackend::accept_dir_trial_keep_streak(const CtlState &s0, Scal *out) {
    const int64_t keep = pipe_streak_;
    const int rc = accept_dir_trial(s0.a_acc, s0.beta, s0.a, s0.npts, out);
    pipe_streak_ = keep;
    return rc;
}



int HipBackend::probe_prepare() {
    if (probe_) return CGO_OK;
    if (int rc = pipe_drain()) return rc;
    u_lag_ = false; rep_n_ = 0;
    HIPCHK(hipSetDevice(ctx_->device));
    HIPCHK(hipStreamSynchronize(ctx_->stream));
    (void)pingpong_ready();
    const size_t n = (size_t)obj_->n_local, na = n + (chain() ? (n & 1) : 0), np = probe_padded(na);
    DevBuf *bufs[] = {&x_, &u_, &x2_, &u2_, &ga_, &gb_};
    for (DevBuf *b : bufs) {
        if (b == &x2_ || b == &u2_) { if (pingpong_ != 1) continue; }
        if (int rc = b->alloc(np)) return rc;
        HIPCHK(hipMemsetAsync(b->p, 0, na * sizeof(double), ctx_->stream));
        HIPCHK(hipMemsetD32Async((hipDeviceptr_t)(b->p + na), (int)PROBE_NAN32, (np - na) * 2, ctx_->stream));
    }
    for (int j = 0; j < obj_->nparams(); ++j) {
        if (!obj_->p_set[j]) continue;
        DevBuf p;
        if (int rc = p.alloc(np)) return rc;
        HIPCHK(hipMemcpyAsync(p.p, obj_->p[j].p, n * sizeof(double), hipMemcpyDeviceToDevice, ctx_->stream));
        HIPCHK(hipMemsetD32Async((hipDeviceptr_t)(p.p + n), (int)PROBE_NAN32, (np - n) * 2, ctx_->stream));
        HIPCHK(hipStreamSynchronize(ctx_->stream));
        std::swap(p.p, obj_->p[j].p); std::swap(p.n, obj_->p[j].n);
    }
    HIPCHK(hipStreamSynchronize(ctx_->stream));
    xc_ = x_.p; uc_ = u_.p; xalt_ = x2_.p; ualt_ = u2_.p;
    g_ = ga_.p; gt_ = gb_.p; xn_ = gb_.p;
    lse_have_ = false;
    probe_ = true;
    return CGO_OK;
}

int HipBackend::probe_slack_intact() {
    const size_t n = (size_t)obj_->n_local, na = n + (chain() ? (n & 1) : 0);
    struct { const DevBuf *b; const char *name; size_t used; int slot; } v[] = {
        {&x_, "x", na, -1}, {&u_, "u", na, -1}, {&x2_, "x (ping-pong)", na, -1}, {&u2_, "u (ping-pong)", na, -1},
        {&ga_, "gradient A", na, -1}, {&gb_, "gradient B / x2", na, -1}, {&obj_->p[0], "parameter vector", n, 0},
        {&obj_->p[1], "parameter vector 1", n, 1}, {&obj_->p[2], "parameter vector 2", n, 2}, {&obj_->p[3], "parameter vector 3", n, 3}};
    std::vector<unsigned> h;
    for (const auto &e : v) {
        if (!e.b->p || (e.slot >= 0 && !(e.slot < obj_->nparams() && obj_->p_set[e.slot]))) continue;
        const size_t words = (e.b->n - e.used) * 2;
        h.assign(words, 0u);
        HIPCHK(hipMemcpyAsync(h.data(), e.b->p + e.used, words * 4, hipMemcpyDeviceToHost, ctx_->stream));
        HIPCHK(hipStreamSynchronize(ctx_->stream));
        for (size_t w = 0; w < words; ++w)
            if (h[w] != PROBE_NAN32) {
                set_error(std::string("probe: the launch wrote past the ") + std::to_string(e.used) + " elements of " + e.name +
                          " (element " + std::to_string(e.used + w / 2) + ")");
                return CGO_ESTATE;
            }
    }
    return CGO_OK;
}

int HipBackend::probe_launch(int kk, int variant, double a_acc, double beta, const double *a, int k, const double *x,
                             const double *u, const double *aux, double *sums, int sums_cap, int *sums_len, double *x_out,
                             double *u_out, double *g_out, std::string &symbol) {
    *sums_len = 0;
    const int want_nact = probe_nact_;
    probe_nact_ = 0;
    const bool lse = obj_->two_phase();
    if (k < 0 || k > MAXP || (k > 0 && !a)) { set_error("probe: 0 ≤ k ≤ 7 trial steps"); return CGO_EINVAL; }
    if (!rmode_ && !lse) return probe_launch_stored(kk, variant, a_acc, beta, a, k, x, u, aux, sums, sums_cap, sums_len, x_out, u_out, g_out, symbol);
    int mode = -1;
    if (lse) {
        if (kk == KK_LSE_STATS && (variant == 0 || variant == LM_NOU || variant == (LM_ACCEPT | LM_DIR))) mode = variant;
        if (kk == KK_LSE_GRAD && variant >= 0 && variant <= 2) mode = variant;
        if (kk == KK_LSE_STATS && mode != LM_NOU && k < 1) mode = -1;
        if (kk == KK_LSE_GRAD && mode != 2 && k < 1) mode = -1;
    } else {
        static constexpr RKind norm_passes{KK_SCALED_NORM, R_GRAD, PTS_ONE, {R_GRADT, 0}};
        const RKind *rk = kk == KK_SCALED_NORM ? &norm_passes : r_kind(kk);
        if (rk && (variant & R_LEAN)) {
            const int full = kk == KK_ACCEPT_DIR_TRIAL ? (R_REPLAY | R_ADT) : (kk == KK_ACCEPT_TRIAL_NOSTORE ? rk->mode : -1);
            if (lean_row(variant) && (variant & ~R_LEAN) == full) mode = variant;
        } else if (rk) {
            const int m = variant ? variant : rk->mode;
            if (r_kind_allows(*rk, m) || (kk == KK_INIT && chain() && m == R_EDGES)) mode = m;
        }
        if (mode > 0 && (mode & (R_TRIAL | R_GRADT | R_PROJ)) && k < 1) mode = -1;
        if (mode > 0 && chain() && k > 3) mode = -1;
        if (mode > 0 && r_big_only(mode) && (chain() || obj_->kind == CGO_OBJ_USER)) mode = -1;
    }
    if (mode < 0) { set_error("probe: kernel kind / variant / trial steps not a launch this solver's engine issues"); return CGO_EINVAL; }
    if (int rc = probe_prepare()) return rc;
    HIPCHK(hipSetDevice(ctx_->device));
    hipStream_t st = ctx_->stream;
    const size_t n = (size_t)obj_->n_local, nb = n * sizeof(double);
    double *ub = lse ? u_.p : uc_;
    double *gb = lse ? gt_ : ga_.p;
    double *auxb = lse ? g_ : xn_;
    auto put = [&](double *dst, const double *src) -> int {
        if (src) HIPCHK(hipMemcpyAsync(dst, src, nb, hipMemcpyHostToDevice, st));
        else HIPCHK(hipMemsetD32Async((hipDeviceptr_t)dst, (int)PROBE_NAN32, n * 2, st));
        return CGO_OK;
    };
    if (int rc = put(xc_, x)) return rc;
    if (int rc = put(ub, u)) return rc;
    if (int rc = put(auxb, aux)) return rc;
    if (gb != auxb) { if (int rc = put(gb, nullptr)) return rc; }
    if (!lse && pingpong_ == 1) {
        if (int rc = put(xalt_, nullptr)) return rc;
        if (int rc = put(ualt_, nullptr)) return rc;
    }
    HIPCHK(hipStreamSynchronize(st));
    probe_len_ = 0;
    last_mode_ = -1;
    beta_lag_ = probe_beta_prev_;
    rep_n_ = (!lse && (mode & R_REPLAY)) ? probe_rep_n_ : 0;
    for (int j = 0; j < rep_n_; ++j) { rep_a_[j] = probe_rep_a_[j]; rep_b_[j] = probe_rep_b_[j]; }
    int rc = CGO_OK;
    char buf[160];
    if (lse) {
        Scal o;
        if (kk == KK_LSE_STATS) {
            lse_have_ = false;
            rc = lse_stats(mode, a_acc, beta, k ? a[0] : 0.0, o, mode == (LM_ACCEPT | LM_DIR));
            snprintf(buf, sizeof buf, "k_lse_stats<%d, %s, %s>", last_mode_, last_big_ ? "true" : "false", last_npts_ ? "true" : "false");
        } else {
            const bool nb0 = need_beta_;
            need_beta_ = mode == 1;
            rc = lse_grad(mode == 2, k ? a[0] : 0.0, o);
            need_beta_ = nb0;
            snprintf(buf, sizeof buf, "k_lse_grad<%s, %s, %s>", last_mode_ == 1 ? "true" : "false", last_mode_ == 2 ? "true" : "false",
                     last_big_ ? "true" : "false");
        }
        if (rc) return rc;
        symbol = buf;
    } else {
        double s[64];
        if (want_nact) {
            if (!path_row(mode, want_nact) || !path_objective(obj_->kind) || k > want_nact) { rep_n_ = 0; set_error("probe: not a path row of this solver, or more steps than it evaluates"); return CGO_EINVAL; }
            path_nact_ = want_nact;
        }
        rc = launch_r(kk, mode, a_acc, beta, a, k, true, s);
        path_nact_ = 0;
        rep_n_ = 0;
        if (rc) return rc;
        symbol = r_symbol(last_mode_, last_npts_, last_big_, last_nact_);
    }
    HIPCHK(hipStreamSynchronize(st));
    if (x_out) HIPCHK(hipMemcpyAsync(x_out, xc_, nb, hipMemcpyDeviceToHost, st));
    if (u_out) HIPCHK(hipMemcpyAsync(u_out, lse ? u_.p : uc_, nb, hipMemcpyDeviceToHost, st));
    if (g_out) HIPCHK(hipMemcpyAsync(g_out, mode == R_PROJ && !lse ? xn_ : gb, nb, hipMemcpyDeviceToHost, st));
    HIPCHK(hipStreamSynchronize(st));
    if (int rc2 = probe_slack_intact()) return rc2;
    *sums_len = probe_len_;
    if (probe_len_ > sums_cap) { set_error("probe: sums_cap smaller than the launch's row"); return CGO_EINVAL; }
    if (probe_len_) std::memcpy(sums, probe_row_, sizeof(double) * probe_len_);
    return CGO_OK;
}

void HipBackend::probe_append(const double *row, int len) {
    if (probe_len_ + len > (int)(sizeof probe_row_ / sizeof probe_row_[0])) return;
    std::memcpy(probe_row_ + probe_len_, row, sizeof(double) * len);
    probe_len_ += len;
}

int HipBackend::probe_launch_stored(int kk, int variant, double a_acc, double beta, const double *a, int k, const double *x,
                                    const double *u, const double *aux, double *sums, int sums_cap, int *sums_len, double *x_out,
                                    double *u_out, double *g_out, std::string &symbol) {
    if (ctx_->world() != 1) { set_error("probe: a single-rank solver"); return CGO_EINVAL; }
    const bool host = obj_->host_closure();
    int mode = -1;
    if (const MKind *mk = m_kind(kk)) {
        const int m = variant ? variant : (host ? mk->host : fused_mode(kk));
        if (host ? m == mk->host : (m == mk->mode || (mk->alt && m == mk->alt))) mode = m;
    } else if (kk == KK_SCALED_NORM) {
        mode = (variant == 0 || variant == 1 || variant == 3 || variant == 4) ? variant : -1;
    }
    const bool trial_step = kk == KK_TRIAL || kk == KK_ACCEPT_DIR_TRIAL;
    if (mode >= 0 && trial_step && k != 1) mode = -1;
    if (mode < 0) { set_error("probe: kernel kind / variant / trial steps not a launch this solver's engine issues"); return CGO_EINVAL; }
    if (int rc = probe_prepare()) return rc;
    HIPCHK(hipSetDevice(ctx_->device));
    hipStream_t st = ctx_->stream;
    const size_t n = (size_t)obj_->n_local, nb = n * sizeof(double);
    auto put = [&](double *dst, const double *src) -> int {
        if (src) HIPCHK(hipMemcpyAsync(dst, src, nb, hipMemcpyHostToDevice, st));
        else HIPCHK(hipMemsetD32Async((hipDeviceptr_t)dst, (int)PROBE_NAN32, n * 2, st));
        return CGO_OK;
    };
    const bool norm = kk == KK_SCALED_NORM;
    const bool gt_in_x = norm && (mode == 1 || mode == 4);
    const bool swaps = kk == KK_ACCEPT_DIR_TRIAL || kk == KK_ACCEPT_DIR || kk == KK_ACCEPT_ONLY;
    if (int rc = put(xc_, gt_in_x ? nullptr : x)) return rc;
    if (int rc = put(u_.p, u)) return rc;
    if (int rc = put(swaps ? gt_ : g_, aux)) return rc;
    if (int rc = put(swaps ? g_ : gt_, gt_in_x ? x : nullptr)) return rc;
    HIPCHK(hipStreamSynchronize(st));
    probe_len_ = 0;
    probe_syms_.clear();
    probe_stored_ = true;
    int rc = CGO_OK;
    Scal o[MAXP];
    switch (kk) {
    case KK_INIT: {
        double s[NS];
        rc = host ? host_trial(0.0, true, o[0]) : launch_k(KK_INIT, 0, 0, 0, true, s);
        break;
    }
    case KK_TRIAL: {
        const bool nb0 = need_beta_;
        need_beta_ = mode == m_mode_of(KK_TRIAL);
        rc = trial(a, 1, o);
        need_beta_ = nb0;
        break;
    }
    case KK_ACCEPT_DIR_TRIAL: rc = accept_dir_trial(a_acc, beta, a, 1, o); break;
    case KK_ACCEPT_DIR: rc = accept_dir(a_acc, beta, o[0]); break;
    case KK_ACCEPT_ONLY: rc = accept_only(a_acc); break;
    case KK_RESET_DIR: rc = reset_dir(o[0]); break;
    case KK_UPG_NORM: { double uu; rc = upg_sumsq(uu); break; }
    default: { double mx, ss; bool nan; rc = scaled_norm_parts(mode, 0.0, mx, ss, nan); break; }
    }
    probe_stored_ = false;
    if (rc) return rc;
    symbol = probe_syms_;
    HIPCHK(hipStreamSynchronize(st));
    if (x_out) HIPCHK(hipMemcpyAsync(x_out, xc_, nb, hipMemcpyDeviceToHost, st));
    if (u_out) HIPCHK(hipMemcpyAsync(u_out, u_.p, nb, hipMemcpyDeviceToHost, st));
    if (g_out) HIPCHK(hipMemcpyAsync(g_out, gt_, nb, hipMemcpyDeviceToHost, st));
    HIPCHK(hipStreamSynchronize(st));
    if (int rc2 = probe_slack_intact()) return rc2;
    *sums_len = probe_len_;
    if (probe_len_ > sums_cap) { set_error("probe: sums_cap smaller than the launch's rows"); return CGO_EINVAL; }
    if (probe_len_) std::memcpy(sums, probe_row_, sizeof(double) * probe_len_);
    return CGO_OK;
}

static_assert(sizeof(cgo_ctl_state) == sizeof(CtlState) && sizeof(cgo_ctl_args) == sizeof(CtlArgs) && sizeof(cgo_ctl_record) == sizeof(CtlRecord),
              "include/cgo.h repeats the controller's blocks word for word");
static_assert(offsetof(cgo_ctl_state, npts) == offsetof(CtlState, npts) && offsetof(cgo_ctl_state, it) == offsetof(CtlState, it) &&
              offsetof(cgo_ctl_args, go) == offsetof(CtlArgs, go) && offsetof(cgo_ctl_record, a_acc) == offsetof(CtlRecord, a_acc) &&
              offsetof(cgo_ctl_record, npts) == offsetof(CtlRecord, npts) && offsetof(cgo_ctl_record, xwait) == offsetof(CtlRecord, xwait),
              "include/cgo.h repeats the controller's blocks word for word");

int HipBackend::probe_armed(const cgo_cg_config &cfg, const cgo_ls_config &ls, cgo_armed_probe &p, const double *x, const double *u,
                            double *x_out, double *u_out) {
    p.symbol[0] = 0;
    if (ctx_->world() != 1) { set_error("probe: a single-rank solver"); return CGO_EINVAL; }
    if (ctl_depth() <= 0) { set_error("probe: this solver's engine arms no rounds (controller depth 0)"); return CGO_EINVAL; }
    if (p.form < 0 || p.form > 2 || p.rounds < 1 || p.rounds > CGO_ARMED_PROBE_MAX_ROUNDS || (p.form == 2 && p.rounds != 1)) {
        set_error("probe: form 0 | 1 | 2, 1 ≤ rounds ≤ 32, the controller alone (form 2) runs one round"); return CGO_EINVAL;
    }
    if (p.st.npts < 0 || p.st.npts > CTL_MAXP) { set_error("probe: 0 ≤ npts ≤ 7 trial steps"); return CGO_EINVAL; }
    if (p.form != 2 && !(x && u)) { set_error("probe: armed rounds read x and u"); return CGO_EINVAL; }
    if (int rc = probe_prepare()) return rc;
    if (int rc = pipe_drain()) return rc;
    if (int rc = pipe_alloc()) return rc;
    HIPCHK(hipSetDevice(ctx_->device));
    hipStream_t st = ctx_->stream;
    const size_t nb = (size_t)obj_->n_local * sizeof(double);
    CtlConfig cc;
    cc.ls = ls; cc.eps = p.use_eps ? p.eps : cfg.eps; cc.mu = cfg.beta.mu;
    cc.beta_kind = cfg.beta.kind; cc.maxp = max_points();
    cc.max_iters = p.max_iters;
    CtlState s0;
    std::memcpy(&s0, &p.st, sizeof s0);
    const int ns = rows_for(cc.maxp);
    if (x) HIPCHK(hipMemcpyAsync(xc_, x, nb, hipMemcpyHostToDevice, st));
    if (u) HIPCHK(hipMemcpyAsync(uc_, u, nb, hipMemcpyHostToDevice, st));
    if (p.form == 2) HIPCHK(hipMemcpyAsync(ctx_->partials, p.row, sizeof(double) * ns, hipMemcpyHostToDevice, st));
    HIPCHK(hipStreamSynchronize(st));
    u_lag_ = false; rep_n_ = 0;
    pipe_npts_ = cc.maxp;
    probe_syms_.clear();
    const unsigned long long first = pipe_enq_;
    k_ctl_init<<<1, 1, 0, st>>>((CtlDev *)ctl_dev_, cc, s0, pipe_enq_);
    HIPCHK(hipGetLastError());
    pipe_stopped_ = false;
    int rc = CGO_OK;
    if (p.form == 2) {
        pipe_checked_ = false;
        rc = pipe_finalize_ctl(ctx_->partials, 1, ns);
        if (!rc) { pipe_prof_[(int)(pipe_enq_ % PIPE_RING)] = {-1, prof_gen_}; pipe_enq_++; }
    } else {
        const bool graph0 = graph_on_;
        graph_on_ = p.form == 1;
        rc = pipe_enqueue(p.rounds);
        graph_on_ = graph0;
    }
    for (unsigned long long id = first; !rc && id < pipe_enq_; ++id) {
        CtlRecord rec;
        rc = pipe_wait(id, rec);
        if (!rc) { std::memcpy(&p.rec[id - first], &rec, sizeof rec); pipe_done_++; }
    }
    if (rc) {
        (void)hipStreamSynchronize(st);
// ... 362 lines not shown
```

conjugategradientoptim.jl_amd/csrc/cgo_capi.hip:

```cpp
#include <sys/mman.h>

#include <cmath>
#include <cstdio>
#include <cstdlib>
#include <cstring>
#include <new>
#include <vector>

#include "cgo_capi_internal.hpp"
#include "cgo_build_id.inc"

using namespace cgo;

extern "C" {

int cgo_version(void) { return CGO_VERSION; }
const char *cgo_build_id(void) { return CGO_BUILD_ID; }
const char *cgo_last_error(void) { return get_error(); }
const char *cgo_status_name(int32_t s) { return status_name(s); }
const char *cgo_kernel_kind_name(int32_t k) {
    if (k == 100) return "dir";
    if (k == 101) return "beta_partials";
    return kernel_kind_name(k);
}
// ... 162 lines not shown
    API_GUARD_BEGIN
    REQUIRE(ctx && source && out, "null argument");
    *out = nullptr;
    REQUIRE(n_params >= 0 && n_params <= CGO_MAX_PARAM_SLOTS, "n_params must be 0 … CGO_MAX_PARAM_SLOTS");
    REQUIRE(n_local >= 1 && offset >= 0 && offset + n_local <= n_global, "bad shard extents");
    REQUIRE(offset % 2 == 0, "shard offset must be even");
    std::shared_ptr<RtcModule> mod;
    std::string log;
    int rc = rtc_compile_objective(ctx->c.device, source, n_params, mod, log);
    if (rc) { set_error("user objective did not compile:\n" + log); return rc; }
    cgo_objective *o = new cgo_objective();
    o->owner = ctx; ctx->refs++;
    o->o.ctx = &ctx->c; o->o.kind = CGO_OBJ_USER; o->o.n_global = n_global; o->o.offset = offset; o->o.n_local = n_local;
    o->o.rtc = mod; o->o.user_nparams = n_params;
    for (int j = 0; j < n_params; ++j) {
        HIPCHK2(hipSetDevice(ctx->c.device));
        rc = o->o.p[j].alloc((size_t)n_local);
        if (rc) { obj_unref(o); return rc; }
    }
    *out = o;
    return CGO_OK;
    API_GUARD_END
}

int cgo_objective_create_callback(cgo_ctx *ctx, cgo_fdf_fn fn, void *user, int64_t n_global, int64_t offset,
                                  int64_t n_local, cgo_objective **out) {
    API_GUARD_BEGIN
    REQUIRE(ctx && fn && out, "null argument");
    *out = nullptr;
    REQUIRE(n_local >= 1 && offset >= 0 && offset + n_local <= n_global, "bad shard extents");
    HIPCHK2(hipSetDevice(ctx->c.device));
    cgo_objective *o = new cgo_objective();
    o->owner = ctx; ctx->refs++;
    o->o.ctx = &ctx->c; o->o.kind = CGO_OBJ_HOST; o->o.n_global = n_global; o->o.offset = offset; o->o.n_local = n_local;
    o->o.host_fn = fn; o->o.host_user = user;
    const size_t bytes = sizeof(double) * (size_t)n_local;
    if (hipHostMalloc((void **)&o->o.host_x, bytes, hipHostMallocDefault) != hipSuccess ||
        hipHostMalloc((void **)&o->o.host_g, bytes, hipHostMallocDefault) != hipSuccess) {
        (void)hipGetLastError();
        obj_unref(o);
        set_error("could not pin host staging buffers for the callback objective");
        return CGO_ENOMEM;
    }
    *out = o;
    return CGO_OK;
    API_GUARD_END
}

int cgo_objective_destroy(cgo_objective *obj) {
    API_GUARD_BEGIN
    obj_unref(obj);
    return CGO_OK;
    API_GUARD_END
}

int cgo_objective_set_param_host(cgo_objective *obj, int32_t slot, const double *host) {
    API_GUARD_BEGIN
    REQUIRE(obj && host, "null argument");
    REQUIRE(slot >= 0 && slot < obj->o.nparams(), "objective has no such parameter vector");
    HipCtx *c = obj->o.ctx;
    HIPCHK2(hipSetDevice(c->device));
    HIPCHK2(hipMemcpyAsync(obj->o.p[slot].p, host, sizeof(double) * (size_t)obj->o.n_local, hipMemcpyHostToDevice, c->stream));
    HIPCHK2(hipStreamSynchronize(c->stream));
    obj->o.p_set[slot] = true;
    return CGO_OK;
    API_GUARD_END
}

int cgo_objective_set_param_device(cgo_objective *obj, int32_t slot, const double *dev_local) {
    API_GUARD_BEGIN
    REQUIRE(obj && dev_local, "null argument");
    REQUIRE(slot >= 0 && slot < obj->o.nparams(), "objective has no such parameter vector");
    HipCtx *c = obj->o.ctx;
    HIPCHK2(hipSetDevice(c->device));
    HIPCHK2(hipMemcpyAsync(obj->o.p[slot].p, dev_local, sizeof(double) * (size_t)obj->o.n_local, hipMemcpyDeviceToDevice, c->stream));
    HIPCHK2(hipStreamSynchronize(c->stream));
    obj->o.p_set[slot] = true;
    return CGO_OK;
    API_GUARD_END
}

int cgo_objective_num_params(cgo_objective *obj, int32_t *n_params) {
    API_GUARD_BEGIN
    REQUIRE(obj && n_params, "null argument");
    *n_params = obj->o.nparams();
    return CGO_OK;
    API_GUARD_END
}

int cgo_objective_fill_param(cgo_objective *obj, int32_t slot, int32_t fill_kind, uint64_t seed,
                             double lo, double hi) {
    API_GUARD_BEGIN
    REQUIRE(obj, "null argument");
    REQUIRE(slot >= 0 && slot < obj->o.nparams(), "objective has no such parameter vector");
    REQUIRE(fill_kind >= 0 && fill_kind <= 2, "unknown fill kind");
    HipCtx *c = obj->o.ctx;
    HIPCHK2(hipSetDevice(c->device));
    if (int rc = fill_device(c, obj->o.p[slot].p, obj->o.n_local, obj->o.offset, fill_kind, seed, lo, hi)) return rc;
    HIPCHK2(hipStreamSynchronize(c->stream));
    obj->o.p_set[slot] = true;
    return CGO_OK;
    API_GUARD_END
}

int cgo_objective_set_scalar(cgo_objective *obj, int32_t slot, double value) {
    API_GUARD_BEGIN
    REQUIRE(obj && slot == 0, "bad argument");
    obj->o.s0 = value;
    return CGO_OK;
    API_GUARD_END
}

int cgo_objective_set_cost_class(cgo_objective *obj, int32_t cost_class) {
    API_GUARD_BEGIN
    REQUIRE(obj && (cost_class == 0 || cost_class == 1), "bad argument");
    REQUIRE(obj->o.kind == CGO_OBJ_USER, "built-in objectives carry their own cost class");
    obj->o.user_cheap = cost_class == 1;
    return CGO_OK;
    API_GUARD_END
}

int cgo_objective_eval_host(cgo_objective *obj, const double *x, double *g, double *f) {
    API_GUARD_BEGIN
    REQUIRE(obj && x && f, "null argument");
    if (obj->o.host_closure()) {
        std::vector<double> tmp;
        if (!g) { tmp.resize((size_t)obj->o.n_local); g = tmp.data(); }
        *f = obj->o.host_fn(obj->o.host_user, g, x, obj->o.n_local);
        return CGO_OK;
    }
    return HipBackend::run_eval(&obj->o, x, g, f);
    API_GUARD_END
}

void cgo_solver_policy_init(cgo_solver_policy *p) {
    if (!p) return;
    std::memset(p, 0, sizeof(*p));
    p->size = (int32_t)sizeof(*p);
    p->resident = p->controller_depth = p->controller_graph = p->controller_fused = -1;
    p->fused_tail = p->strict_tail = p->placement_search = -1;
    p->lbfgs_fuse_grad = p->lbfgs_fuse_trial = p->lse_fixed_reference = -1;
}

int cgo_ctx_set_default_policy(cgo_ctx *ctx, const cgo_solver_policy *policy) {
    API_GUARD_BEGIN
    REQUIRE(ctx, "null argument");
    if (!policy) { ctx->has_defpol = false; return CGO_OK; }
    REQUIRE(policy->size == (int32_t)sizeof(cgo_solver_policy), "cgo_solver_policy.size does not match this library (call cgo_solver_policy_init first)");
    ctx->defpol = *policy; ctx->has_defpol = true;
    return CGO_OK;
    API_GUARD_END
}

static const int kReplayDepth = 8;
static const bool kLeanSums = true;
static const bool kPathPredict = true;
static int env_tri(const char *name) { const char *e = getenv(name); return e ? (e[0] != '0' ? 1 : 0) : -1; }
extern "C++" int resolve_policy(cgo_ctx *ctx, const cgo_solver_policy *arg, cgo_solver_policy &r, std::string &why) {
    cgo_solver_policy lib; cgo_solver_policy_init(&lib);
    const cgo_solver_policy *defp = ctx->has_defpol ? &ctx->defpol : nullptr;
    for (const cgo_solver_policy *p : {arg, defp})
        if (p && p->size != (int32_t)sizeof(cgo_solver_policy)) { why = "cgo_solver_policy.size does not match this library (call cgo_solver_policy_init first)"; return CGO_EINVAL; }
    r = lib;
    const cgo_solver_policy *layers[2] = {defp, arg};
    for (const cgo_solver_policy *p : layers) {
        if (!p) continue;
        if (p->points) r.points = p->points;
        if (p->resident >= 0) r.resident = p->resident;
        if (p->controller_depth >= 0) r.controller_depth = p->controller_depth;
        if (p->controller_graph >= 0) r.controller_graph = p->controller_graph;
        if (p->controller_fused >= 0) r.controller_fused = p->controller_fused;
        if (p->stored_gradient) r.stored_gradient = p->stored_gradient;
        if (p->fused_tail >= 0) r.fused_tail = p->fused_tail;
        if (p->strict_tail >= 0) r.strict_tail = p->strict_tail;
        if (p->placement_search >= 0) r.placement_search = p->placement_search;
        if (p->placement_stages) r.placement_stages = p->placement_stages;
        if (p->placement_max_bytes) r.placement_max_bytes = p->placement_max_bytes;
        if (p->lbfgs_form) r.lbfgs_form = p->lbfgs_form;
        if (p->lbfgs_fuse_grad >= 0) r.lbfgs_fuse_grad = p->lbfgs_fuse_grad;
        if (p->lbfgs_fuse_trial >= 0) r.lbfgs_fuse_trial = p->lbfgs_fuse_trial;
        if (p->lse_fixed_reference >= 0) r.lse_fixed_reference = p->lse_fixed_reference;
        if (p->resident_points) r.resident_points = p->resident_points;
        if (p->resident_chunk) r.resident_chunk = p->resident_chunk;
        if (p->hbm_stream_bytes > 0.0) r.hbm_stream_bytes = p->hbm_stream_bytes;
    }
    if (!(r.points == 0 || r.points == 1 || r.points == 3 || r.points == 5 || r.points == 7)) { why = "cgo_solver_policy.points must be 0, 1, 3, 5 or 7"; return CGO_EINVAL; }
    if (r.lbfgs_form < 0 || r.lbfgs_form > 4) { why = "cgo_solver_policy.lbfgs_form must be 0 … 4"; return CGO_EINVAL; }
    if (!(r.resident_points == 0 || r.resident_points == 1 || r.resident_points == 3 || r.resident_points == 7)) { why = "cgo_solver_policy.resident_points must be 0, 1, 3 or 7"; return CGO_EINVAL; }
    if (r.placement_stages < 0 || r.placement_stages > 3 || r.placement_max_bytes < 0) { why = "cgo_solver_policy.placement_* out of range"; return CGO_EINVAL; }
    if (r.resident < 0) r.resident = env_tri("CGO_RESIDENT");
    if (r.controller_depth < 0) { if (const char *e = getenv("CGO_CTL_DEPTH")) r.controller_depth = std::max(0, atoi(e)); }
    if (r.controller_graph < 0) r.controller_graph = env_tri("CGO_CTL_GRAPH");
    if (r.controller_fused < 0) r.controller_fused = env_tri("CGO_CTL_FUSED");
    if (!r.stored_gradient) { const char *e = getenv("CGO_STORED_G"); r.stored_gradient = (e && e[0] == '1') ? 1 : 0; }
    if (r.placement_search < 0) r.placement_search = env_tri("CGO_PLACE_TUNE");
    if (!r.placement_stages) { if (const char *e = getenv("CGO_PLACE_STAGES")) { const int v = atoi(e); if (v >= 1 && v <= 3) r.placement_stages = v; } }
    if (!r.lbfgs_form) {
        const char *tl = getenv("CGO_LBFGS_TWO_LOOP"), *sp = getenv("CGO_LBFGS_SPEC");
        if (tl && tl[0] == '1') r.lbfgs_form = 4;
        else if (sp && sp[0] == '0') r.lbfgs_form = 3;
        else if (sp && sp[0] == '1') r.lbfgs_form = 2;
    }
    if (r.lbfgs_fuse_grad < 0) r.lbfgs_fuse_grad = env_tri("CGO_LBFGS_FUSE_GRAD");
    if (r.lbfgs_fuse_trial < 0) r.lbfgs_fuse_trial = env_tri("CGO_LBFGS_FUSE_TRIAL");
    if (r.lse_fixed_reference < 0) r.lse_fixed_reference = env_tri("CGO_LSE_REF");
    if (!r.resident_points) { if (const char *e = getenv("CGO_RES_POINTS")) { const int v = atoi(e); if (v == 1 || v == 3 || v == 7) r.resident_points = v; } }
    if (!r.resident_chunk) { if (const char *e = getenv("CGO_RES_CHUNK")) { const long long v = atoll(e); if (v >= 2 && v < (1LL << 30)) r.resident_chunk = (int32_t)(v & ~1LL); } }
    if (!(r.hbm_stream_bytes > 0.0)) { if (const char *e = getenv("CGO_BIG_BYTES")) { const double v = atof(e); if (v > 0.0) r.hbm_stream_bytes = v; } }
    if (r.controller_graph < 0) r.controller_graph = 0;
    if (r.controller_fused < 0) r.controller_fused = 1;
    if (r.lbfgs_fuse_grad < 0) r.lbfgs_fuse_grad = 1;
    if (r.lbfgs_fuse_trial < 0) r.lbfgs_fuse_trial = 1;
    if (r.lse_fixed_reference < 0) r.lse_fixed_reference = 1;
    if (r.placement_search < 0) r.placement_search = 0;
    return CGO_OK;
}

int cgo_solver_get_policy(cgo_solver *s, cgo_solver_policy *out) {
    API_GUARD_BEGIN
    REQUIRE(s && out, "null argument");
    *out = s->pol;
    out->points = s->be->policy_points();
    out->resident = s->be->resident_enabled() ? 1 : 0;
    out->controller_depth = s->be->ctl_depth_setting();
    out->fused_tail = s->ctx->c.fused_tail ? 1 : 0;
    out->strict_tail = s->ctx->c.tail_strict ? 1 : 0;
    return CGO_OK;
    API_GUARD_END
}

static bool path_applies(const cgo_objective *obj, const cgo_cg_config *cfg, const cgo_ls_config *ls) {
    if (!ls || obj->o.kind != CGO_OBJ_QUAD_DIAG || cfg->beta.kind != CGO_BETA_POLAK_RIBIERE) return false;
    if (ls->kind == CGO_LS_STRONG_WOLFE_BISECTION) return true;
    return ls->kind == CGO_LS_WOLFE_BISECTION && ls->cond_kind == CGO_COND_WOLFE;
}

extern "C++" int make_solver(cgo_ctx *ctx, cgo_objective *obj, const cgo_cg_config *cfg, const cgo_ls_config *ls,
                       const cgo_lss_config *lss, const cgo_solver_policy *policy, cgo_solver **out) {
    *out = nullptr;
    REQUIRE(obj->o.ctx == &ctx->c, "objective belongs to another ctx");
    std::string why;
    if (int rc = check_cg_config(cfg, why)) { set_error(why); return rc; }
    if (ls) { if (int rc = check_ls_config(ls, why)) { set_error(why); return rc; } }
    else {
        if (int rc = check_lss_config(lss, why)) { set_error(why); return rc; }
        REQUIRE(cfg->beta.kind < CGO_BETA_LBFGS, "solvesystem takes a CGβConfig (solve_system.jl:69), not a QNβConfig");
        REQUIRE(!obj->o.two_phase() && !obj->o.host_closure() && obj->o.kind != CGO_OBJ_ROSENBROCK_CHAINED,
                "solvesystem needs an element-wise device objective (k_cg kernel family)");
    }
    const bool chain = obj->o.kind == CGO_OBJ_ROSENBROCK_CHAINED;
    if (chain) REQUIRE(cfg->beta.kind != CGO_BETA_LBFGS, "the chained (stencil) Rosenbrock objective runs on the gradient-free CG kernels: CG β kinds only");
    cgo_solver_policy pol;
    { std::string pw; if (int rc = resolve_policy(ctx, policy, pol, pw)) { set_error(pw); return rc; } }
    cgo_solver *s = new cgo_solver();
    s->ctx = ctx; s->obj = obj; s->pol = pol;
    obj->refs++;
    obj->o.users++;
    s->be = new HipBackend(&ctx->c, &obj->o);
    s->sv = nullptr;
    s->be->set_policy(pol);
    s->be->set_need_beta(cfg->beta.kind != CGO_BETA_LBFGS);
    s->be->set_rmode(chain || (!obj->o.two_phase() && !obj->o.host_closure() && cfg->beta.kind != CGO_BETA_LBFGS && (!ls || !pol.stored_gradient)));
    int rc = s->be->alloc();
    if (rc) { delete s; obj_unref(obj); return rc; }
    const bool cheap = obj->o.kind == CGO_OBJ_QUAD_DIAG || obj->o.kind == CGO_OBJ_BOOTH ||
                       (obj->o.kind == CGO_OBJ_USER && obj->o.user_cheap);
    s->be->set_multi_min_n(0);
    s->be->set_multi5_min_n(cheap ? 0 : INT64_MAX);
    s->be->set_multi7_min_n(cheap ? 0 : INT64_MAX);
    s->be->set_three_point_band(0, 0);
    const char *mm = getenv("CGO_MULTI_MIN_N"), *m5 = getenv("CGO_MULTI5_MIN_N"), *m7 = getenv("CGO_MULTI7_MIN_N");
    if (chain) m5 = m7 = nullptr;
    if (mm || m5 || m7) s->be->set_three_point_band(0, 0);
    if (mm) s->be->set_multi_min_n(atoll(mm));
    if (m5) s->be->set_multi5_min_n(atoll(m5));
    if (m7) s->be->set_multi7_min_n(atoll(m7));
    if (pol.points) {
        const int pts = chain ? std::min(pol.points, 3) : pol.points;
        s->be->set_three_point_band(0, 0);
        s->be->set_multi_min_n(pts >= 3 ? 0 : INT64_MAX);
        s->be->set_multi5_min_n(pts >= 5 ? 0 : INT64_MAX);
        s->be->set_multi7_min_n(pts >= 7 ? 0 : INT64_MAX);
    }
    s->be->set_ctl_depth((ls && !cheap && !chain && s->be->policy_points() <= 3 && (ctx->c.world() == 1 || ctx->c.dev_exchange()) && obj->o.n_local <= 100000) ? 4 : 0);
    if (pol.controller_depth >= 0) s->be->set_ctl_depth(chain ? 0 : pol.controller_depth);
    s->be->set_ctl_graph(pol.controller_graph != 0);
    {
        bool lazy = obj->o.kind == CGO_OBJ_QUAD_DIAG;
        const int forced = env_tri("CGO_LAZY_DIR");
        if (forced >= 0) lazy = forced != 0;
        s->be->set_lazy_direction(lazy);
    }
    {
        int depth = 1;
        if (obj->o.kind == CGO_OBJ_QUAD_DIAG && 8.0 * (double)obj->o.n_local * 5.0 > 1.4e9) depth = kReplayDepth;
        if (const char *e = getenv("CGO_REPLAY_DEPTH")) { const int v = atoi(e); if (v >= 1 && v <= 8) depth = v; }
        s->be->set_replay_depth(depth);
    }
    {
        bool lean = kLeanSums && obj->o.kind == CGO_OBJ_QUAD_DIAG && 8.0 * (double)obj->o.n_local * 5.0 > 1.4e9;
        const int forced = env_tri("CGO_LEAN_SUMS");
        if (forced >= 0) lean = forced != 0;
        s->be->set_beta_unread(beta_unread_sums(cfg->beta.kind));
        s->be->set_lean_sums(lean);
    }
    {
        bool predict = kPathPredict && kLeanSums && obj->o.kind == CGO_OBJ_QUAD_DIAG && 8.0 * (double)obj->o.n_local * 5.0 > 1.4e9;
        const int forced = env_tri("CGO_PATH_PREDICT");
        if (forced >= 0) predict = forced != 0;
        s->be->set_path_prediction(predict && path_applies(obj, cfg, ls));
    }
    if (int prc = s->be->place()) { delete s; obj_unref(obj); return prc; }
    if (pol.resident >= 0) s->be->set_resident(pol.resident != 0);
    if (int prc = s->be->prepare_controller()) { delete s; obj_unref(obj); return prc; }
    s->sv = ls ? new Solver(s->be, *cfg, *ls) : new Solver(s->be, *cfg, *lss);
    *out = s;
    return CGO_OK;
}

int cgo_solver_create(cgo_ctx *ctx, cgo_objective *obj, const cgo_cg_config *cfg,
                      const cgo_ls_config *ls, cgo_solver **out) {
    API_GUARD_BEGIN
    REQUIRE(ctx && obj && cfg && ls && out, "null argument");
    return make_solver(ctx, obj, cfg, ls, nullptr, nullptr, out);
    API_GUARD_END
}

int cgo_solver_create_ex(cgo_ctx *ctx, cgo_objective *obj, const cgo_cg_config *cfg, const cgo_ls_config *ls,
                         const cgo_solver_policy *policy, cgo_solver **out) {
    API_GUARD_BEGIN
    REQUIRE(ctx && obj && cfg && ls && out, "null argument");
    return make_solver(ctx, obj, cfg, ls, nullptr, policy, out);
    API_GUARD_END
}

int cgo_solver_create_sys(cgo_ctx *ctx, cgo_objective *obj, const cgo_cg_config *cfg,
                          const cgo_lss_config *ls, cgo_solver **out) {
    API_GUARD_BEGIN
    REQUIRE(ctx && obj && cfg && ls && out, "null argument");
    return make_solver(ctx, obj, cfg, nullptr, ls, nullptr, out);
    API_GUARD_END
}

int cgo_solver_create_sys_ex(cgo_ctx *ctx, cgo_objective *obj, const cgo_cg_config *cfg, const cgo_lss_config *ls,
                             const cgo_solver_policy *policy, cgo_solver **out) {
    API_GUARD_BEGIN
    REQUIRE(ctx && obj && cfg && ls && out, "null argument");
    return make_solver(ctx, obj, cfg, nullptr, ls, policy, out);
    API_GUARD_END
}

int cgo_check_lss_config(const cgo_lss_config *ls) {
    API_GUARD_BEGIN
    std::string why;
    if (int rc = check_lss_config(ls, why)) { set_error(why); return rc; }
    return CGO_OK;
    API_GUARD_END
}

int64_t cgo_lss_default_max_iters(double rho) { return lss_default_max_iters(rho); }

int cgo_solver_destroy(cgo_solver *s) {
    API_GUARD_BEGIN
    if (s) {
        (void)hipSetDevice(s->ctx->c.device);
        cgo_objective *o = s->obj;
        delete s;
        obj_unref(o);
    }
    return CGO_OK;
    API_GUARD_END
}

int cgo_solver_set_x0_host(cgo_solver *s, const double *x0) {
    API_GUARD_BEGIN
    REQUIRE(s && x0, "null argument");
    return s->be->set_x0_host(x0);
    API_GUARD_END
}

int cgo_solver_set_x0_device(cgo_solver *s, const double *x0_dev) {
    API_GUARD_BEGIN
    REQUIRE(s && x0_dev, "null argument");
    hipPointerAttribute_t at;
    if (hipPointerGetAttributes(&at, x0_dev) != hipSuccess || at.type != hipMemoryTypeDevice || at.device != s->ctx->c.device) {
        (void)hipGetLastError();
        set_error("cgo_solver_set_x0_device: not a device pointer of this context's GPU");
        return CGO_EINVAL;
    }
    return s->be->set_x0_device(x0_dev);
    API_GUARD_END
}

int cgo_solver_results_device(cgo_solver *s, double *minimizer_dev, double *gradient_dev) {
    API_GUARD_BEGIN
    REQUIRE(s, "null argument");
    for (double *p : {minimizer_dev, gradient_dev}) {
        if (!p) continue;
        hipPointerAttribute_t at;
        if (hipPointerGetAttributes(&at, p) != hipSuccess || at.type != hipMemoryTypeDevice || at.device != s->ctx->c.device) {
            (void)hipGetLastError();
            set_error("cgo_solver_results_device: not a device pointer of this context's GPU");
            return CGO_EINVAL;
        }
    }
    return s->be->download_device(minimizer_dev, gradient_dev);
    API_GUARD_END
}

int cgo_solver_set_x0_fill(cgo_solver *s, int32_t kind, uint64_t seed, double lo, double hi) {
    API_GUARD_BEGIN
    REQUIRE(s, "null argument");
    REQUIRE(kind >= 0 && kind <= 2, "unknown fill kind");
    return s->be->set_x0_fill(kind, seed, lo, hi);
    API_GUARD_END
}

int cgo_solver_start(cgo_solver *s) {
    API_GUARD_BEGIN
    REQUIRE(s, "null argument");
    if (s->be->probed()) { set_error("a solver that a probe (cgo_solver_probe_launch / _lbfgs / _resident / _armed) has used is for probing only"); return CGO_ESTATE; }
    return s->sv->start();
    API_GUARD_END
}

int cgo_solver_iterate(cgo_solver *s, int64_t iters, int32_t *finished) {
    API_GUARD_BEGIN
    REQUIRE(s, "null argument");
    if (s->be->probed()) { set_error("a solver that a probe (cgo_solver_probe_launch / _lbfgs / _resident / _armed) has used is for probing only"); return CGO_ESTATE; }
    bool fin = false;
    int rc = s->sv->iterate(iters, fin);
    if (rc == CGO_ESTATE) set_error("cgo_solver_iterate before cgo_solver_start");
    if (finished) *finished = fin ? 1 : 0;
    if (rc == CGO_OK && fin) rc = s->be->tail_errors();
    return rc;
    API_GUARD_END
}

int cgo_solver_results(cgo_solver *s, cgo_results *out) {
    API_GUARD_BEGIN
    REQUIRE(s && out, "null argument");
    Solver &sv = *s->sv;
    out->objective = sv.objective();
    out->iters_ran = sv.finished() ? sv.iters_ran() : (int64_t)sv.trace_objective().size();
    out->status = sv.status();
    out->total_fdf_evals = sv.total_evals();
    out->total_launches = s->be->launches();
    if (!sv.finished() && !sv.config().trace_enabled) out->iters_ran = -1;
    const size_t k = sv.trace_objective().size();
    if (out->trace_objective && k) std::memcpy(out->trace_objective, sv.trace_objective().data(), k * sizeof(double));
    if (out->trace_grad_norm && k) std::memcpy(out->trace_grad_norm, sv.trace_grad_norm().data(), k * sizeof(double));
    if (out->trace_step_size && k) std::memcpy(out->trace_step_size, sv.trace_step_size().data(), k * sizeof(double));
    if (out->trace_objective_evals && k) std::memcpy(out->trace_objective_evals, sv.trace_evals().data(), k * sizeof(int64_t));
    if (int rc = s->be->tail_errors()) return rc;
    if (out->minimizer || out->gradient) return s->be->download(out->minimizer, out->gradient);
    return CGO_OK;
    API_GUARD_END
}

int cgo_solver_trial_log(cgo_solver *s, int64_t cap, double *a, double *phi, double *dphi, int64_t *count) {
    API_GUARD_BEGIN
    REQUIRE(s && count, "null argument");
    if (cap < 0) { s->sv->set_log_enabled(true); *count = 0; return CGO_OK; }
    const auto &L = s->sv->trial_log();
    *count = (int64_t)L.size();
    const int64_t m = std::min<int64_t>(cap, (int64_t)L.size());
    for (int64_t i = 0; i < m; ++i) {
        if (a) a[i] = L[i].a;
        if (phi) phi[i] = L[i].phi;
        if (dphi) dphi[i] = L[i].dphi;
    }
    return CGO_OK;
    API_GUARD_END
}

const char *cgo_solver_kernel_family(cgo_solver *s) {
    if (!s) return "";
    const bool qn = s->sv->config().beta.kind == CGO_BETA_LBFGS;
    if (s->obj->o.two_phase()) return qn ? "k_lse (two-phase) + k_lbfgs" : "k_lse (two-phase)";
    if (s->be->rmode()) {
        const int mp = s->be->max_points();
        return mp >= 7 ? "k_cg (gradient-free, 7-point)" : mp >= 5 ? "k_cg (gradient-free, 5-point)" : (mp >= 3 ? "k_cg (gradient-free, 3-point)" : "k_cg (gradient-free, 1-point)");
    }
    return qn ? "k_fused (stored gradient) + k_lbfgs" : "k_fused (stored gradient)";
}

int64_t cgo_solver_controller_launches(cgo_solver *s) { return s ? s->be->ctl_served() : 0; }

int cgo_solver_resident_stats(cgo_solver *s, int64_t *slices, int64_t *iterations, int64_t *gave_up) {
    API_GUARD_BEGIN
    REQUIRE(s, "null argument");
    if (slices) *slices = s->be->resident_slices();
    if (iterations) *iterations = s->be->resident_iters();
    if (gave_up) *gave_up = s->be->resident_gave_up();
    return CGO_OK;
    API_GUARD_END
}

int cgo_solver_lbfgs_stats(cgo_solver *s, int64_t *speculated, int64_t *fused, int64_t *plain) {
    API_GUARD_BEGIN
    REQUIRE(s, "null argument");
    if (speculated) *speculated = s->be->push_count(0);
    if (fused) *fused = s->be->push_count(1);
    if (plain) *plain = s->be->push_count(2);
    return CGO_OK;
    API_GUARD_END
}

int cgo_solver_kernel_symbol(cgo_solver *s, int32_t kernel_kind, char *buf, int32_t cap) {
    API_GUARD_BEGIN
    REQUIRE(s && buf && cap > 0, "bad argument");
    const std::string sym = s->be->kernel_symbol(kernel_kind);
    std::snprintf(buf, (size_t)cap, "%s", sym.c_str());
    return CGO_OK;
    API_GUARD_END
}

int cgo_solver_set_lazy_direction(cgo_solver *s, int32_t on) {
    API_GUARD_BEGIN
    REQUIRE(s, "null argument");
    return s->be->set_lazy_direction_now(on != 0);
    API_GUARD_END
}

int cgo_solver_set_replay_depth(cgo_solver *s, int32_t d) {
    API_GUARD_BEGIN
    REQUIRE(s, "null argument");
    REQUIRE(d >= 1 && d <= 8, "replay depth: 1 … 8");
    return s->be->set_replay_depth_now(d);
    API_GUARD_END
}

int cgo_solver_set_lean_sums(cgo_solver *s, int32_t on) {
    API_GUARD_BEGIN
    REQUIRE(s, "null argument");
    s->be->set_lean_sums(on != 0);
    return CGO_OK;
    API_GUARD_END
}

int cgo_solver_set_path_prediction(cgo_solver *s, int32_t on) {
    API_GUARD_BEGIN
    REQUIRE(s, "null argument");
    const bool applies = s->sv && !s->sv->is_sys() && path_applies(s->obj, &s->sv->config(), &s->sv->linesearch());
    s->be->set_path_prediction(on != 0 && applies);
    return CGO_OK;
    API_GUARD_END
}

int cgo_solver_path_stats(cgo_solver *s, int64_t *by_nact, int64_t *predicted, int64_t *tree, int64_t *misses) {
    API_GUARD_BEGIN
    REQUIRE(s && s->sv, "null argument");
    if (by_nact) for (int j = 0; j < 8; ++j) by_nact[j] = s->be->path_launches(j);
    int64_t p = 0, t = 0, m = 0;
    s->sv->path_stats(p, t, m);
    if (predicted) *predicted = p;
    if (tree) *tree = t;
    if (misses) *misses = m;
    return CGO_OK;
    API_GUARD_END
}

int cgo_solver_debug_set_path_skew(cgo_solver *s, double factor) {
    API_GUARD_BEGIN
    REQUIRE(s && s->sv, "null argument");
    REQUIRE(factor > 0.0 && std::isfinite(factor), "path skew: a positive factor");
    s->sv->set_path_skew(factor);
    return CGO_OK;
    API_GUARD_END
}

int cgo_solver_probe_set_path(cgo_solver *s, int32_t nact) {
    API_GUARD_BEGIN
    REQUIRE(s, "null argument");
    REQUIRE(nact >= 0 && nact <= 7, "probe path row: 0 … 7 active points");
    s->be->set_probe_path(nact);
    return CGO_OK;
    API_GUARD_END
}

int cgo_solver_probe_set_replay(cgo_solver *s, int32_t nrep, const double *a, const double *beta) {
    API_GUARD_BEGIN
    REQUIRE(s, "null argument");
    REQUIRE(nrep >= 0 && nrep <= 7 && (nrep == 0 || (a && beta)), "probe replay list: 0 … 7 (a*, β) pairs");
    s->be->set_probe_replay(nrep, a, beta);
    return CGO_OK;
    API_GUARD_END
}

int cgo_solver_probe_set_beta_prev(cgo_solver *s, double beta_prev) {
    API_GUARD_BEGIN
    REQUIRE(s, "null argument");
    s->be->set_probe_beta_prev(beta_prev);
    return CGO_OK;
    API_GUARD_END
}

int cgo_solver_profile_enable(cgo_solver *s, int32_t on) {
    API_GUARD_BEGIN
    REQUIRE(s, "null argument");
    s->be->profile_enable(on != 0);
    return CGO_OK;
    API_GUARD_END
}
int cgo_solver_profile_reset(cgo_solver *s) {
    API_GUARD_BEGIN
    REQUIRE(s, "null argument");
    s->be->profile_reset();
    return CGO_OK;
    API_GUARD_END
}
int cgo_solver_profile_get(cgo_solver *s, int32_t kind, int64_t *launches, double *ms, double *bytes) {
    API_GUARD_BEGIN
    REQUIRE(s && launches && ms && bytes, "null argument");
    s->be->profile_get(kind, launches, ms, bytes);
    return CGO_OK;
    API_GUARD_END
}

int cgo_minimize(cgo_ctx *ctx, cgo_objective *obj, const double *x0, const cgo_cg_config *cfg,
                 const cgo_ls_config *ls, cgo_results *out) {
    API_GUARD_BEGIN
    REQUIRE(x0 && out, "null argument");
    cgo_solver *s = nullptr;
    int rc = cgo_solver_create(ctx, obj, cfg, ls, &s);
    if (rc) return rc;
    rc = s->be->set_x0_host(x0);
    if (!rc) rc = s->sv->start();
    bool fin = false;
    while (!rc && !fin) rc = s->sv->iterate(INT64_MAX / 2, fin);
    if (!rc) rc = cgo_solver_results(s, out);
    std::string keep = get_error();
    cgo_solver_destroy(s);
    if (rc) set_error(keep);
    return rc;
    API_GUARD_END
}

int cgo_evalwolfeconditions(const cgo_ls_config *ls, double phi_a, double dphi_a, double a, double uu,
                            double phi_0, double dphi_0, int32_t *valid_large, int32_t *valid_small) {
    API_GUARD_BEGIN
    REQUIRE(ls && valid_large && valid_small, "null argument");
    REQUIRE(ls->cond_kind == CGO_COND_WOLFE || ls->cond_kind == CGO_COND_YUAN_WEI_LU, "not a Wolfe-type condition");
    if (ls->cond_kind == CGO_COND_WOLFE) {
        if (!(0.0 < ls->c1 && ls->c1 < ls->c2 && ls->c2 < 1.0)) { set_error("AssertionError: zero(T) < c1 < c2 < one(T)  (wolfe.jl:278)"); return CGO_EINVAL; }
    } else if (!(0.0 < ls->delta1 && ls->delta1 < ls->c1 && ls->c1 < ls->c2 && ls->c2 < 1.0)) {
        set_error("AssertionError: zero(T) < δ1 < c1 < c2 < one(T)  (wolfe.jl:233)"); return CGO_EINVAL;
    }
    bool okl = false, oks = false;
    wolfe_tests(*ls, phi_0, dphi_0, uu, phi_a, dphi_a, a, okl, oks);
    *valid_large = okl; *valid_small = oks;
    return CGO_OK;
    API_GUARD_END
}

int cgo_evalbacktrackcondition(const cgo_ls_config *ls, double phi_a, double a, double phi_0, double dphi_0,
                               int32_t *valid) {
    API_GUARD_BEGIN
    REQUIRE(ls && valid, "null argument");
    if (!(0.0 < ls->c1 && ls->c1 < 1.0)) { set_error("AssertionError: zero(T) < c1 < one(T)  (geometric.jl:169)"); return CGO_EINVAL; }
    *valid = armijo_test(ls->c1, phi_a, a, phi_0, dphi_0);
    return CGO_OK;
    API_GUARD_END
}

int cgo_solvesystem(cgo_ctx *ctx, cgo_objective *obj, const double *x0, const cgo_cg_config *cfg,
                    const cgo_lss_config *ls, cgo_results *out) {
    API_GUARD_BEGIN
    REQUIRE(x0 && out, "null argument");
    cgo_solver *s = nullptr;
    int rc = cgo_solver_create_sys(ctx, obj, cfg, ls, &s);
    if (rc) return rc;
    rc = s->be->set_x0_host(x0);
    if (!rc) rc = s->sv->start();
    bool fin = false;
    while (!rc && !fin) rc = s->sv->iterate(INT64_MAX / 2, fin);
    if (!rc) rc = cgo_solver_results(s, out);
    std::string keep = get_error();
    cgo_solver_destroy(s);
    if (rc) set_error(keep);
    return rc;
    API_GUARD_END
}

static int rerun_stage(cgo_ctx *ctx, cgo_objective *obj, const double *x0_host, const double *x0_dev, const cgo_cg_config *cfg,
                       const cgo_ls_config *ls, cgo_results *out, double *seed_out) {
    cgo_solver *s = nullptr;
    int rc = cgo_solver_create(ctx, obj, cfg, ls, &s);
    if (rc) return rc;
    rc = x0_dev ? s->be->set_x0_device(x0_dev) : s->be->set_x0_host(x0_host);
    if (!rc) rc = s->sv->start();
    bool fin = false;
    while (!rc && !fin) rc = s->sv->iterate(INT64_MAX / 2, fin);
    if (!rc) rc = cgo_solver_results(s, out);
    if (!rc && seed_out && out->status != CGO_SUCCESS) rc = s->be->download_device(seed_out, nullptr);
    std::string keep = get_error();
    cgo_solver_destroy(s);
    if (rc) set_error(keep);
    return rc;
}

int cgo_minimize_rerun(cgo_ctx *ctx, cgo_objective *obj, const double *x0, const cgo_cg_config *cfg,
                       const cgo_ls_config *ls, const cgo_cg_config *rerun_cfgs,
                       const cgo_ls_config *rerun_ls, int32_t npairs, cgo_results *outs, int32_t *nouts) {
    API_GUARD_BEGIN
    REQUIRE(ctx && obj && x0 && outs && nouts && npairs >= 0, "bad argument");
    REQUIRE(npairs == 0 || (rerun_cfgs && rerun_ls), "null rerun configs");
    DevBuf seed;
    if (npairs > 0) {
        if (hipSetDevice(ctx->c.device) != hipSuccess) { set_error("hipSetDevice failed"); return CGO_EHIP; }
        if (int rc = seed.alloc((size_t)obj->o.n_local)) return rc;
    }
    int rc = rerun_stage(ctx, obj, x0, nullptr, cfg, ls, &outs[0], npairs > 0 ? seed.p : nullptr);
    if (rc) return rc;
    int cnt = 1;
    for (int k = 0; k < npairs; ++k) {
        if (outs[cnt - 1].status == CGO_SUCCESS) break;
        rc = rerun_stage(ctx, obj, nullptr, seed.p, &rerun_cfgs[k], &rerun_ls[k], &outs[cnt], k + 1 < npairs ? seed.p : nullptr);
        if (rc) return rc;
        cnt++;
    }
    *nouts = cnt;
    return CGO_OK;
    API_GUARD_END
}

int cgo_kernel_dir(cgo_ctx *ctx, double *u, const double *g, double beta, int64_t n, double *out2) {
    API_GUARD_BEGIN
    REQUIRE(ctx && u && g && out2 && n >= 1, "bad argument");
    return HipBackend::run_dir(&ctx->c, u, g, beta, n, out2);
    API_GUARD_END
}

int cgo_kernel_beta_partials(cgo_ctx *ctx, const double *gn, const double *g, const double *u,
                             int64_t n, double *out9) {
    API_GUARD_BEGIN
    REQUIRE(ctx && gn && g && u && out9 && n >= 1, "bad argument");
    return HipBackend::run_beta_partials(&ctx->c, gn, g, u, n, out9);
// ... 113 lines not shown
```

conjugategradientoptim.jl_amd/csrc/cgo_hip_backend.hpp:

```cpp
#pragma once

#include <hip/hip_runtime.h>

#include <memory>
#include <string>
#include <vector>

#include "cgo_engine.hpp"
#include "cgo_launch_kinds.hpp"
#include "cgo_rtc.hpp"

namespace cgo {

namespace dev { struct CtlArgs; struct Tail; struct LoopParams; struct ResParams; struct BatchParams; struct BatchLbfgsParams; }

void set_error(const std::string &msg);
const char *get_error();

struct DevBuf {
    double *p = nullptr;
    size_t n = 0;
    DevBuf() {}
    DevBuf(const DevBuf &) = delete;
    DevBuf &operator=(const DevBuf &) = delete;
// ... 39 lines not shown
    int placed_candidates = 0;
    std::string arch;
    int num_cu = 0;
    ~HipCtx();
    int init(int device);
    int ensure_gather();
    int rank() const { return comm ? comm->rank : 0; }
    int world() const { return comm ? comm->world : 1; }
};

struct HipObjective {
    HipCtx *ctx = nullptr;
    int kind = 0;
    int64_t n_global = 0, offset = 0, n_local = 0;
    DevBuf p[CGO_MAX_PARAM_SLOTS];
    bool p_set[CGO_MAX_PARAM_SLOTS] = {};
    double s0 = 0.0;
    std::shared_ptr<RtcModule> rtc;
    int user_nparams = 0;
    bool user_cheap = false;
    int users = 0;
    cgo_fdf_fn host_fn = nullptr;
    void *host_user = nullptr;
    double *host_x = nullptr, *host_g = nullptr;
    bool host_closure() const { return kind == CGO_OBJ_HOST; }
    ~HipObjective();
    int nparams() const { return kind == CGO_OBJ_QUAD_DIAG ? 1 : (kind == CGO_OBJ_USER ? user_nparams : 0); }
    bool uses_param() const { return nparams() > 0; }
    int unset_slot() const { for (int j = 0; j < nparams(); ++j) if (!p_set[j]) return j; return -1; }
    template <class A> void param_args(A &P) const { P.p0 = p[0].p; P.p1 = p[1].p; P.p2 = p[2].p; P.p3 = p[3].p; }
    bool two_phase() const { return kind == CGO_OBJ_LSE; }
};

struct RPlan { bool big; int grid, npts; double bytes; };

struct QnState;
class HipBackend : public VecBackend {
  public:
    HipBackend(HipCtx *ctx, HipObjective *obj);
    ~HipBackend() override;
    int alloc();
    int place();
    int64_t n_local() const override { return obj_->n_local; }
    int set_x0_host(const double *x0) override;
    int set_x0_device(const double *x0_dev);
    int download_device(double *x_dev, double *g_dev);
    int tail_errors();
    int set_x0_fill(int kind, uint64_t seed, double lo, double hi) override;
    int init_eval(Scal &out) override;
    int max_points() const override {
        if (!rmode_ || obj_->n_local < multi_min_n_) return 1;
        return policy_points();
    }
    int policy_points() const {
        if (!rmode_ || obj_->n_local < multi_min_n_) return 1;
        if (obj_->n_local >= band3_lo_ && obj_->n_local < band3_hi_) return 3;
        if (obj_->n_local >= multi7_min_n_) return 7;
        return obj_->n_local >= multi5_min_n_ ? 5 : 3;
    }
    int trial(const double *a, int k, Scal *out) override;
    int accept_dir_trial(double a_acc, double beta, const double *a, int k, Scal *out) override;
    int ctl_depth() const override;
    int accept_dir_trial_ctl(const CtlConfig &cc, const CtlState &s0, int64_t rounds, Scal *out) override;
    void set_ctl_depth(int d) { ctl_depth_ = d < 0 ? 0 : (d > 32 ? 32 : d); }
    void set_policy(const cgo_solver_policy &p);
    const cgo_solver_policy &policy() const { return pol_; }
    double big_bytes(bool read_only = false) const;
    int prepare_controller();
    int64_t ctl_served() const { return pipe_served_; }
    int64_t ctl_graph_rounds() const { return graph_rounds_; }
    void placement_info(double *first_us, double *best_us, int *candidates) const { *first_us = place_first_us_; *best_us = place_best_us_; *candidates = place_candidates_; }
    double placement_cap_bytes() const { return place_cap_bytes_; }
    void set_ctl_graph(bool on) { graph_on_ = on; }
    bool resident_ready(const cgo_cg_config &cfg, const cgo_ls_config &ls) const override;
    int resident_run(const ResConfig &c, ResState &s, int64_t budget, std::vector<ResRecord> &recs, std::vector<ResLog> &log) override;
    void set_resident(bool on) { res_on_ = on; }
    bool resident_enabled() const { return res_on_; }
    int ctl_depth_setting() const { return ctl_depth_; }
    int64_t resident_iters() const { return res_iters_; }
    int64_t resident_slices() const { return res_slices_; }
    int64_t resident_gave_up() const { return res_gave_up_; }
    static int64_t batch_max_n(HipCtx *ctx, int obj_kind, const RtcModule *rtc = nullptr);
    int batch_alloc(int64_t batch, int64_t n, const double *const *params, bool device_rows = false);
    static int64_t batch_rows_max_n();
    static int batch_rows_unroll();
    static int batch_rows_block();
    static double batch_rows_bytes(int64_t batch, int64_t n, int nparams);
    bool batch_device_rows() const { return bat_rows_; }
    int batch_reset(const double *x0, const double *scalars, const unsigned char *active, int64_t max_iters, bool trace);
    int batch_launch(const ResConfig &c, int64_t budget, std::vector<ResState> &st, std::vector<double> &f_x0) override;
    int batch_records(int64_t b, int64_t count, std::vector<ResRecord> &out);
    int64_t batch_rec_stride() const { return bat_rec_stride_; }
    int batch_export_row(int64_t b, HipBackend &dst, bool with_u);
    int batch_export_slots(int64_t b, HipBackend &dst);
    int batch_results(double *x , double *g , const unsigned char *active = nullptr);
    int batch_lbfgs_alloc(int m, bool lds = false);
    int batch_lbfgs_reset(int m = 0);
    int batch_lbfgs_m() const { return bat_m_; }
    static int64_t batch_lbfgs_max_n();
    static int batch_lbfgs_unroll();
    static int batch_lbfgs_unroll_for(int nparams);
    static int batch_lbfgs_block();
    static double batch_lbfgs_bytes(int64_t batch, int64_t n, int nparams, int m);
    static int batch_lbfgs_lds_rows(int nparams, int m);
    static int batch_lbfgs_lds_unroll_for(int nparams);
    static int64_t batch_lbfgs_lds_ld_of(int64_t max_lds, int64_t static_lds, int rows);
    static int64_t batch_lbfgs_lds_max_ld(HipCtx *ctx, int obj_kind, int m, const RtcModule *rtc = nullptr);
    bool batch_lbfgs_in_lds() const { return bat_qn_lds_; }
    int batch_probe(cgo_batch_probe_args &p);
    int64_t push_count(int kind) const { return push_counts_[kind]; }
    bool sys_supported() const override { return rmode_; }
    int sys_begin() override;
    int sys_project(double a, double m, Scal &out) override;
    int sys_commit() override;
    int dir_trial(double beta, const double *a, int k, Scal *out) override;
    int accept_dir(double a_acc, double beta, Scal &out) override;
    int accept_only(double a_acc) override;
    int reset_dir(Scal &out) override;
    int upg_sumsq(double &out) override;
    int lbfgs_alloc(int slots) override;
    int lbfgs_gram_max_pairs() const override { return gram_on_ ? 12 : 0; }
    int lbfgs_push_gram(double a_x, double a_s, int slot, const int *prev, int count, GramOut &out) override;
    bool lbfgs_push_materializes(double a_x) override;
    bool lbfgs_push_spec(double a_x, double a_s, int slot, const int *prev, int count, GramOut &out) override;
    int lbfgs_push_commit(bool direction_follows) override;
    int lbfgs_direction_gram(const int *slots, const double *cy, const double *cs, int count, double cg,
                             Scal &out) override;
    bool lbfgs_direction_gram_can_fuse_trial() const override;
    int lbfgs_direction_gram_trial(const int *slots, const double *cy, const double *cs, int count, double cg, double a_trial,
                                   Scal &dir, Scal &trial) override;
    int lbfgs_push(double a_x, double a_s, int slot, double &sy, double &yy) override;
    int lbfgs_direction(const int *slots, const double *rho, int count, double gamma,
                        Scal &out) override;
    bool two_phase() const override { return obj_->two_phase(); }
    int materialize(Scal &out) override;
    void discard_pending() override { push_pending_ = false; push_lite_pending_ = false; lite_deferred_ = false; spec_valid_ = false; spec_unmat_ = false; }
    int download(double *x, double *g) override;
    int scaled_norm_parts(int which, double a_trial, double &maxabs, double &scaled_ss, bool &has_nan) override;
    void profile_enable(bool on) override;
    void profile_reset() override;
    void profile_get(int kind, int64_t *launches, double *ms, double *bytes) override;
    int64_t launches() const override { return total_launches_; }
    void set_need_beta(bool b) { need_beta_ = b; }
    void set_rmode(bool on) { rmode_ = on; }
    void set_multi_min_n(int64_t n) { multi_min_n_ = n; }
    void set_multi5_min_n(int64_t n) { multi5_min_n_ = n; }
    void set_multi7_min_n(int64_t n) { multi7_min_n_ = n; }
    void set_three_point_band(int64_t lo, int64_t hi) { band3_lo_ = lo; band3_hi_ = hi; }
    bool rmode() const { return rmode_; }
    void set_lazy_direction(bool on) { lazy_on_ = on; }
    bool lazy_direction() const { return lazy_on_; }
    int set_lazy_direction_now(bool on) { if (!on) { if (int rc = materialize_lag()) return rc; } lazy_on_ = on; return 0; }
    void set_probe_beta_prev(double b) { probe_beta_prev_ = b; }
    void set_replay_depth(int d) { replay_depth_ = d < 1 ? 1 : (d > 8 ? 8 : d); }
    int replay_depth() const { return replay_depth_; }
    int set_replay_depth_now(int d);
    void set_probe_replay(int nrep, const double *a, const double *beta);
    void set_beta_unread(int bits) { lean_mask_ = bits; if (lean_bits_) lean_bits_ = bits; }
    void set_lean_sums(bool on) { lean_bits_ = on ? lean_mask_ : 0; }
    bool lean_sums() const { return lean_bits_ != 0; }
    void set_path_prediction(bool on) { path_on_ = on; }
    bool path_prediction() const { return path_on_; }
    bool path_rows() const override;
    int accept_dir_trial_path(double a_acc, double beta, const double *a, int k, Scal *out) override;
    int64_t path_launches(int nact) const { return (nact >= 1 && nact <= 7) ? path_count_[nact] : 0; }
    void set_probe_path(int nact) { probe_nact_ = nact; }
    std::string kernel_symbol(int kernel_kind) const;
    int probe_launch(int kernel_kind, int variant, double a_acc, double beta, const double *a, int k, const double *x,
                     const double *u, const double *aux, double *sums, int sums_cap, int *sums_len, double *x_out,
                     double *u_out, double *g_out, std::string &symbol);
    bool probed() const { return probe_; }
    int probe_launch_stored(int kernel_kind, int variant, double a_acc, double beta, const double *a, int k, const double *x,
                            const double *u, const double *aux, double *sums, int sums_cap, int *sums_len, double *x_out,
                            double *u_out, double *g_out, std::string &symbol);
    int probe_lbfgs(int m, cgo_lbfgs_probe &p, const double *x, const double *u, const double *g, const double *gt, const double *S,
                    const double *Y, double *x_out, double *xo_out, double *u_out, double *g_out, double *gt_out, double *S_out,
                    double *Y_out);

    int probe_resident(const cgo_cg_config &cfg, const cgo_ls_config &ls, cgo_resident_probe &p, const double *x, const double *u,
                       double *rows, int64_t rows_cap, double *x_out, double *u_out);

    int probe_armed(const cgo_cg_config &cfg, const cgo_ls_config &ls, cgo_armed_probe &p, const double *x, const double *u,
                    double *x_out, double *u_out);

    static int run_dir(HipCtx *ctx, double *u_host, const double *g_host, double beta, int64_t n,
                       double *out2);
    static int run_beta_partials(HipCtx *ctx, const double *gn, const double *g, const double *u,
                                 int64_t n, double *out9);
    static int run_trial(HipObjective *obj, const double *x, const double *u, double a,
                         double *gn_out, double *out2);
    static int run_eval(HipObjective *obj, const double *x, double *g_out, double *f);
    static int bench_kernel(HipCtx *ctx, HipObjective *obj, int kernel_kind, int64_t n, int reps,
                            double *ms, double *bytes);
    static int bench_stream_mix(HipCtx *ctx, int64_t n, int reps, double *median_us, double *best_us);

  private:
    int launch(int kk, int mode, double a_acc, double beta, double a_trial, bool fetch,
               double *sums );
    int launch_k(int kk, double a_acc, double beta, double a_trial, bool fetch, double *sums) { return launch(kk, fused_mode(kk), a_acc, beta, a_trial, fetch, sums); }
    HipCtx *ctx_;
    HipObjective *obj_;
    DevBuf x_, u_, ga_, gb_;
    DevBuf x2_, u2_;
    double *uc_ = nullptr;
    double *xalt_ = nullptr, *ualt_ = nullptr;
    int pingpong_ = -1;
    bool sys_on_ = false;
    bool chain() const { return obj_->kind == CGO_OBJ_ROSENBROCK_CHAINED; }
    bool probe_ = false;
    double probe_row_[64] = {};
    int probe_len_ = 0;
    int last_mode_ = -1, last_npts_ = 0;
    bool last_big_ = false;
    int probe_prepare();
    int probe_slack_intact();
    std::string r_symbol(int mode, int npts, bool big, int nact = 0) const;
    std::string probe_syms_;
    void probe_note(const double *row, int len, const char *fmt, ...);
    int probe_ring_slack_intact();
    bool probe_stored_ = false;
    void probe_append(const double *row, int len);
    const char *obj_tname() const;
    int launch_loop(const dev::LoopParams &P, int kk, double nvec, bool big, int grid);
    double halo_xl_[2] = {0, 0}, halo_ul_[2] = {0, 0}, halo_xr_[2] = {0, 0}, halo_ur_[2] = {0, 0};
    int launch_chain_kernel(int mode, double a_acc, double beta, const double *a, int k, int npts, bool big, int grid, const dev::Tail &tail);
    bool tail_fused(int grid) const;
    bool pipe_fused(int grid) const;
    dev::Tail make_tail(bool on);
    bool pingpong_ready();
    int tune_placement();
    double place_first_us_ = 0.0, place_best_us_ = 0.0;
    int place_candidates_ = 0;
    double place_cap_bytes_ = 0.0;
    bool placed_ = false;
    int ensure_ga();
    int ensure_gb();
    double *xc_ = nullptr, *xn_ = nullptr;
    double *g_ = nullptr, *gt_ = nullptr;
    bool need_beta_ = true;
    bool rmode_ = false;
    int64_t multi_min_n_ = 3000000;
    int64_t multi5_min_n_ = INT64_MAX;
    int64_t multi7_min_n_ = INT64_MAX;
    int64_t band3_lo_ = 0, band3_hi_ = 0;
    int launch_r(int kk, int mode, double a_acc, double beta, const double *a, int k, bool fetch, double *sums);
    int launch_rk(int kk, double a_acc, double beta, const double *a, int k, bool fetch, double *sums) { return launch_r(kk, r_mode_of(kk), a_acc, beta, a, k, fetch, sums); }
    RPlan r_plan(int mode, int npts) const;
    bool adt_is_big() const;
    int fused_mode(int kk) const { const MKind *mk = m_kind(kk); return !mk ? -1 : ((kk == KK_TRIAL && !need_beta_) ? mk->alt : mk->mode); }
    std::string lbfgs_symbol(int kk) const;
    bool lazy_on_ = false, u_lag_ = false;
    double beta_lag_ = 0.0, probe_beta_prev_ = 0.0;
    bool lazy_eligible() const;
    int materialize_u();
    int replay_depth_ = 1, rep_n_ = 0, probe_rep_n_ = 0;
    double rep_a_[7] = {}, rep_b_[7] = {}, probe_rep_a_[7] = {}, probe_rep_b_[7] = {};
    int materialize_lag();
    int lean_mask_ = 0, lean_bits_ = 0;
    int lean_for(int mode) const;
    bool path_on_ = false;
    int path_nact_ = 0, last_nact_ = 0, probe_nact_ = 0;
    int path_last_n_ = 0, path_last_s_ = 0;
    int64_t path_count_[8] = {};
    int accept_dir_trial_r(double a_acc, double beta, const double *a, int k, double *s);
    int trial_r(const double *a, int k, double *s);
    int launch_r_kernel(int kk, int mode, double a_acc, double beta, const double *a, int k, int npts,
                        const struct dev::CtlArgs *ctl, RPlan *plan_out);
    int ctl_depth_ = 0;
    unsigned long long epoch_ = 0;
    void *ctl_dev_ = nullptr;
    void *ctl_rec_ = nullptr;
    unsigned long long *ctl_seq_ = nullptr;
    unsigned long long pipe_enq_ = 0, pipe_done_ = 0;
    bool pipe_stopped_ = false;
    bool pipe_checked_ = false;
    bool ctl_fused_ = true;
    cgo_solver_policy pol_;
    int pipe_npts_ = 1;
    int64_t pipe_streak_ = 0;
    int64_t pipe_served_ = 0;
    std::vector<std::pair<int, unsigned>> pipe_prof_;
    unsigned prof_gen_ = 0;
    int pipe_alloc();
    int pipe_round_kernels();
    int pipe_finalize_ctl(const double *src, int nrows, int ns);
    int pipe_enqueue_round();
    int pipe_launch_graph(int rounds);
    int pipe_enqueue(int64_t count);
    struct PipeGraph { void *exec; int rounds, npts; double *x, *u; const double *p0; int64_t n; std::string syms; };
    std::vector<PipeGraph> graphs_;
    bool graph_on_ = false;
    bool capturing_ = false;
    unsigned long long pipe_batches_ = 0;
    int64_t graph_rounds_ = 0;
    int pipe_wait(unsigned long long id, CtlRecord &rec);
    int pipe_drain();
    int accept_dir_trial_keep_streak(const CtlState &s0, Scal *out);
    bool res_on_ = true;
    int res_grid_ = 0, res_npts_ = 3;
    int64_t res_chunk_ = 0;
    size_t res_lds_ = 0;
    int res_plan();
    int res_alloc();
    void res_out_buffers(double *&xo, double *&uo) const;
    void res_fill_params(dev::ResParams &P, double *xo, double *uo);
    void res_swap_in(double *xo, double *uo);
    int res_error_reset();
    ResState *res_state_ = nullptr;
    ResRecord *res_recs_ = nullptr;
    ResLog *res_log_ = nullptr;
    ResRecord *res_recs_dev_ = nullptr;
    ResLog *res_log_dev_ = nullptr;
    double *res_xbuf_ = nullptr;
    unsigned int *res_err_ = nullptr;
    DevBuf res_xo_, res_uo_;
    double *res_xin_ = nullptr, *res_uin_ = nullptr;
    unsigned long long *res_done_ = nullptr;
    unsigned long long res_seq_ = 0, res_round_ = 0;
    void *res_pr_script_ = nullptr, *res_pr_out_ = nullptr;
    double *res_pr_rows_ = nullptr;
    bool res_pr_ready_ = false;
    int64_t res_iters_ = 0, res_slices_ = 0, res_gave_up_ = 0;
    int64_t bat_count_ = 0, bat_n_ = 0, bat_ld_ = 0, bat_rec_stride_ = 0;
    bool bat_trace_ = false;
    size_t bat_lds_ = 0;
    bool bat_rows_ = false;
    ResState *bat_st_ = nullptr;
    ResRecord *bat_recs_ = nullptr;
    double *bat_fx0_ = nullptr;
    double *bat_s0v_ = nullptr;
    bool bat_s0v_on_ = false;
    size_t bat_recs_cap_ = 0;
    void batch_fill_rows(std::vector<double> &rows, const double *src) const;
    int batch_recs_reserve(int64_t stride);
    int batch_grad_rows();
    void batch_fill_params(dev::BatchParams &B, const ResConfig &c, int64_t budget) const;
    void batch_lbfgs_fill_params(dev::BatchLbfgsParams &L, const ResConfig &c, int64_t budget) const;
    int bat_m_ = 0;
    double *bat_S_ = nullptr, *bat_Y_ = nullptr;
    QnState *bat_qn_ = nullptr;
    int batch_lbfgs_launch(const ResConfig &c, int64_t budget, std::vector<ResState> &st, std::vector<double> &f_x0);
    bool bat_qn_lds_ = false;
    int batch_lbfgs_lds_on();
    int batch_lbfgs_lds_launch(const dev::BatchLbfgsParams &L);
    bool prof_on_ = false;
    struct ProfSlot { hipEvent_t e0 = nullptr, e1 = nullptr; int kk = -1; double bytes = 0; };
    std::vector<ProfSlot> ring_;
    int ring_used_ = 0;
    int prof_slot(hipEvent_t *e0, hipEvent_t *e1);
    int prof_begin(int kk);
    int prof_end();
    void prof_commit(int kk, double bytes);
    void prof_flush();
    bool prof_pick(int kk);
    int prof_every_ = 4;
    int64_t prof_tick_[KK_COUNT] = {};
    bool prof_cur_ = false;
    int64_t prof_cnt_[KK_COUNT] = {};
    int64_t prof_n_[KK_COUNT] = {};
    double prof_ms_[KK_COUNT] = {};
    double prof_bytes_[KK_COUNT] = {};
    int64_t total_launches_ = 0;
    int qn_m_ = 0;
    bool gram_on_ = true;
    DevBuf qn_S_, qn_Y_;
    double *qn_alpha_dev_ = nullptr;
    double qn_sgt_ = 0.0;
    int qn_sgt_slot_ = -1;
    bool push_pending_ = false, fuse_grad_ = true;
    double *push_xo_ = nullptr;
    bool spec_on_ = false, spec_valid_ = false, push_lite_pending_ = false;
    bool spec_fuse_push_ = true, lite_deferred_ = false, spec_unmat_ = false;
    int flush_lite();
    double spec_s_[64] = {}, spec_Mr_ = 0.0, spec_Sr_ = 1.0, spec_a_ = 0.0, spec_dphi_ = 0.0;
    int64_t spec_refreshed_ = 0;
    int spec_count_ = 0, spec_slots_[16] = {};
    double lite_a_ = 0.0, lite_as_ = 0.0, lite_M_ = 0.0, lite_S_ = 1.0;
    int lite_slot_ = 0;
    int64_t push_counts_[3] = {0, 0, 0};
    int lbfgs_direction_spec(const int *slots, const double *cy, const double *cs, int count, double cg, double a_trial, Scal &dir, Scal &trial);
    int lbfgs_push_lite();
    int chain_sums(int grid, int slot, const double **dot_ptr, int *dot_count, double *dot_host);
    double lse_a_ = 0.0, lse_M_ = 0.0, lse_S_ = 1.0;
    bool lse_have_ = false;
    int lse_stats(int mode, double a_acc, double beta, double a_trial, Scal &out, bool dir);
    int lse_grad(bool init, double a, Scal &out);
    int host_trial(double a, bool init, Scal &out);
};

int launch_fused(HipCtx *ctx, int obj_kind, int mode, const void *kparams, int64_t n,
                 bool timed = false, const HipObjective *obj = nullptr, hipEvent_t e0 = nullptr,
                 hipEvent_t e1 = nullptr, double big_forced = -1.0 );
int grid_for(int64_t n);
double bytes_for(int obj_kind, int mode, int64_t n, int n_params = 0);
int param_unset_error(int slot);
enum MergeKind { MERGE_SUM = 0, MERGE_LSE = 1, MERGE_MAX0 = 2 };
int fetch_sums(HipCtx *ctx, double *sums, int merge = MERGE_SUM, int ns = 10, double *raw = nullptr);
int finalize_launch(HipCtx *ctx, int grid, bool lse);
int finalize_rows(HipCtx *ctx, int rows, int ns, bool canon = false);
int fill_device(HipCtx *ctx, double *v, int64_t n, int64_t offset, int kind, uint64_t seed, double lo,
                double hi);

Comm *make_rccl_comm(HipCtx *ctx, int rank, int world, const void *unique_id128);
Comm *make_callback_comm(int rank, int world, cgo_allgather_fn fn, void *user);
Comm *make_shm_comm(HipCtx *ctx, int rank, int world, const char *name, int create);
int rccl_unique_id(void *out128);
bool rccl_available();

}
// ... 1 lines not shown
```

conjugategradientoptim.jl_amd/csrc/cgo_kernels_cg_path.hip.hpp:

```cpp
#pragma once

#include "cgo_kernels_cg.hip.hpp"

namespace cgo {
namespace dev {

template <class Obj> struct ObjCurv { static constexpr bool declared = false; };
template <> struct ObjCurv<ObjQuadDiag> {
    static constexpr bool declared = true;
    __device__ static inline d2 apply2(d2 v, const PV<ObjQuadDiag> &p) { return d2{p.v[0].x * v.x, p.v[0].y * v.y}; }
    __device__ static inline double apply1(double v, const PS<ObjQuadDiag> &p) { return p.v[0] * v; }
};

constexpr bool path_mode(int mode) {
    return (r_base(mode) == (R_REPLAY | R_ACCEPT | R_DIR | R_TRIAL | R_NOWU | R_NOWX) || r_base(mode) == (R_REPLAY | R_ACCEPT | R_DIR | R_TRIAL)) &&
           (mode & R_NOYY) != 0;
}

template <class Obj, int MODE, int NACT>
__device__ inline void cg_path_pair(const RParams &P, d2 &x, d2 &u, const PV<Obj> &p, double (&acc)[RW<MAXP>::W], bool &wx, bool &wu) {
    constexpr int R_GU = RW<MAXP>::GU, R_UU = RW<MAXP>::UU;
#pragma unroll
    for (int j = 0; j < RMAX; ++j) {
        if (j < P.nrep) {
            d2 gr;
            double fr = 0.0;
            x.x = x.x + P.ra[j] * u.x;
            x.y = x.y + P.ra[j] * u.y;
            obj_eval2<Obj>(x, p, P.s0, fr, gr);
            u.x = -gr.x + P.rb[j] * u.x; u.y = -gr.y + P.rb[j] * u.y;
        }
    }
    x.x = x.x + P.a_acc * u.x;
    x.y = x.y + P.a_acc * u.y;
    wx = r_writes_x(MODE);
    d2 g;
    double f0 = 0.0;
    obj_eval2<Obj>(x, p, P.s0, f0, g);
    {
        d2 un;
        un.x = -g.x + P.beta * u.x; un.y = -g.y + P.beta * u.y;
        acc[R_GU] = dsum(acc[R_GU], g.x, un.x); acc[R_GU] = dsum(acc[R_GU], g.y, un.y);
        acc[R_UU] = dsum(acc[R_UU], un.x, un.x); acc[R_UU] = dsum(acc[R_UU], un.y, un.y);
        u = un;
        wu = r_writes_u(MODE);
    }
#pragma unroll
    for (int j = 0; j < NACT; ++j) {
        const int b = RS_PER_POINT * j;
        d2 xp, gt;
        xp.x = x.x + P.a[j] * u.x;
        xp.y = x.y + P.a[j] * u.y;
        obj_term2<Obj, LateF<Obj, MODE>::on>(xp, p, P.s0, acc[b + RS_F], gt);
        const double y0 = gt.x - g.x, y1 = gt.y - g.y;
        acc[b + RS_GTU] = dsum(acc[b + RS_GTU], gt.x, u.x);   acc[b + RS_GTU] = dsum(acc[b + RS_GTU], gt.y, u.y);
        acc[b + RS_GTGT] = dsum(acc[b + RS_GTGT], gt.x, gt.x); acc[b + RS_GTGT] = dsum(acc[b + RS_GTGT], gt.y, gt.y);
        if (!(MODE & R_NOGTG)) { acc[b + RS_GTG] = dsum(acc[b + RS_GTG], gt.x, g.x);   acc[b + RS_GTG] = dsum(acc[b + RS_GTG], gt.y, g.y); }
        if (!(MODE & R_NOUY)) { acc[b + RS_UY] = dsum(acc[b + RS_UY], u.x, y0);      acc[b + RS_UY] = dsum(acc[b + RS_UY], u.y, y1); }
        if (!(MODE & R_NOYGT)) { acc[b + RS_YGT] = dsum(acc[b + RS_YGT], y0, gt.x);    acc[b + RS_YGT] = dsum(acc[b + RS_YGT], y1, gt.y); }
        if constexpr (ObjCurv<Obj>::declared) {
            const d2 hg = ObjCurv<Obj>::apply2(gt, p);
            acc[b + RS_YY] = dsum(acc[b + RS_YY], gt.x, hg.x); acc[b + RS_YY] = dsum(acc[b + RS_YY], gt.y, hg.y);
        }
    }
}

template <class Obj, int MODE, int NACT>
__device__ inline void cg_path_single(const RParams &P, long long i, double (&acc)[RW<MAXP>::W]) {
    constexpr int R_GU = RW<MAXP>::GU, R_UU = RW<MAXP>::UU;
    double x = P.x[i];
    double u = P.u[i];
    const PS<Obj> p = ps_load<Obj>(P, i);
#pragma unroll
    for (int j = 0; j < RMAX; ++j) {
        if (j < P.nrep) {
            double gr = 0.0, fr = 0.0;
            x = x + P.ra[j] * u;
            obj_eval1<Obj>(x, p, P.s0, fr, gr);
            u = -gr + P.rb[j] * u;
        }
    }
    x = x + P.a_acc * u;
    if (r_writes_x(MODE)) P.xo[i] = x;
    double g = 0.0, f0 = 0.0;
    obj_eval1<Obj>(x, p, P.s0, f0, g);
    const double un = -g + P.beta * u;
    acc[R_GU] = dsum(acc[R_GU], g, un); acc[R_UU] = dsum(acc[R_UU], un, un);
    if (r_writes_u(MODE)) P.uo[i] = un;
    u = un;
#pragma unroll
    for (int j = 0; j < NACT; ++j) {
        const int b = RS_PER_POINT * j;
        const double xp = x + P.a[j] * u;
        double gt;
        obj_term1<Obj, LateF<Obj, MODE>::on>(xp, p, P.s0, acc[b + RS_F], gt);
        const double y = gt - g;
        acc[b + RS_GTU] = dsum(acc[b + RS_GTU], gt, u); acc[b + RS_GTGT] = dsum(acc[b + RS_GTGT], gt, gt);
        if (!(MODE & R_NOGTG)) acc[b + RS_GTG] = dsum(acc[b + RS_GTG], gt, g);
        if (!(MODE & R_NOUY)) acc[b + RS_UY] = dsum(acc[b + RS_UY], u, y);
        if (!(MODE & R_NOYGT)) acc[b + RS_YGT] = dsum(acc[b + RS_YGT], y, gt);
        if constexpr (ObjCurv<Obj>::declared) acc[b + RS_YY] = dsum(acc[b + RS_YY], gt, ObjCurv<Obj>::apply1(gt, p));
    }
}

template <class Obj, int MODE, int NACT, bool BIG>
__global__ __launch_bounds__(BLOCK) void k_cg_path(const RParams P) {
    static_assert(BIG, "path launches exist as pure-HBM streams only");
    static_assert(path_mode(MODE), "a path row is launch N or S of the replay cycle in a lean form that leaves the y·y slot free");
    static_assert(NACT >= 1 && NACT <= MAXP, "1 … 7 of the row's seven points");
    constexpr int W = RW<MAXP>::W;
    double acc[W];
#pragma unroll
    for (int s = 0; s < W; ++s) acc[s] = 0.0;
    const long long n2 = P.n >> 1;
    const long long per = big_chunk_pairs(n2, gridDim.x);
    long long i = per * blockIdx.x + threadIdx.x;
    const long long hi = (per * blockIdx.x + per < n2) ? per * blockIdx.x + per : n2;
    const long long step = BLOCK;
    for (; i + step < hi; i += 2 * step) {
        d2 xa = ldg2<true>(P.x, i), xb = ldg2<true>(P.x, i + step);
        d2 ua = ldg2<true>(P.u, i), ub = ldg2<true>(P.u, i + step);
        const PV<Obj> pa = pv_load<Obj, true>(P, i), pb = pv_load<Obj, true>(P, i + step);
        bool wxa = false, wua = false, wxb = false, wub = false;
        cg_path_pair<Obj, MODE, NACT>(P, xa, ua, pa, acc, wxa, wua);
        cg_path_pair<Obj, MODE, NACT>(P, xb, ub, pb, acc, wxb, wub);
        if (wxa) stg2<true>(P.xo, i, xa);
        if (wua) stg2<true>(P.uo, i, ua);
        if (wxb) stg2<true>(P.xo, i + step, xb);
        if (wub) stg2<true>(P.uo, i + step, ub);
    }
    if (i < hi) {
        d2 xa = ldg2<true>(P.x, i);
        d2 ua = ldg2<true>(P.u, i);
        const PV<Obj> pa = pv_load<Obj, true>(P, i);
        bool wxa = false, wua = false;
        cg_path_pair<Obj, MODE, NACT>(P, xa, ua, pa, acc, wxa, wua);
        if (wxa) stg2<true>(P.xo, i, xa);
        if (wua) stg2<true>(P.uo, i, ua);
    }
    if ((P.n & 1) && blockIdx.x == 0 && threadIdx.x == 0) cg_path_single<Obj, MODE, NACT>(P, P.n - 1, acc);
    if constexpr (LateF<Obj, MODE>::on) {
#pragma unroll
        for (int j = 0; j < NACT; ++j) acc[RS_PER_POINT * j + RS_F] *= ObjFScale<Obj>::scale;
    }
    store_partials_n<W, false>(acc, P.partials, P.tail);
}

}
}
```

include/cgo.h:

```cpp
#ifndef CGO_H
#define CGO_H

#include <stdint.h>

#ifdef __cplusplus
extern "C" {
#endif

#define CGO_VERSION 100

enum {
    CGO_OK = 0,
    CGO_EINVAL = 1,
    CGO_EHIP = 2,
    CGO_ECOMM = 3,
    CGO_ENODEV = 4,
    CGO_ESTATE = 5,
    CGO_ENOMEM = 6
};

enum {
    CGO_INCOMPLETE = 0,
    CGO_SUCCESS = 1,
    CGO_INCREASING_OBJECTIVE = 2,
// ... 52 lines not shown

enum {
    CGO_FILL_CONSTANT = 0,
    CGO_FILL_UNIFORM = 1,
    CGO_FILL_ALTERNATE = 2
};

typedef struct cgo_beta_config {
    int32_t kind;
    int32_t lbfgs_m;
    double mu;
} cgo_beta_config;

typedef struct cgo_cg_config {
    double eps;
    cgo_beta_config beta;
    int64_t max_iters;
    int32_t verbose;
    int32_t trace_enabled;
} cgo_cg_config;

typedef struct cgo_ls_config {
    int32_t kind;
    int32_t cond_kind;
    double c1, c2;
    double a_max_growth_factor;
    double delta1;
    double max_step_size;
    int64_t max_iters;
    int64_t zoom_max_iters;
    int64_t feasibility_max_iters;
    double discount_factor;
} cgo_ls_config;

typedef struct cgo_results {
    double objective;
    double *minimizer;
    double *gradient;
    int64_t iters_ran;
    int32_t status;
    int32_t _pad;
    double *trace_objective;
    double *trace_grad_norm;
    double *trace_step_size;
    int64_t *trace_objective_evals;
    int64_t total_fdf_evals;
    int64_t total_launches;
} cgo_results;

typedef struct cgo_ctx cgo_ctx;
typedef struct cgo_objective cgo_objective;
typedef struct cgo_solver cgo_solver;

typedef int (*cgo_allgather_fn)(void *user, const double *send, double *recv, int32_t count);

int cgo_version(void);
const char *cgo_build_id(void);
const char *cgo_last_error(void);
const char *cgo_status_name(int32_t status);
int cgo_device_count(int32_t *count);

int cgo_check_cg_config(const cgo_cg_config *cfg);
int cgo_check_ls_config(const cgo_ls_config *ls);

int cgo_ctx_create(int32_t device, cgo_ctx **out);
int cgo_ctx_destroy(cgo_ctx *ctx);
int cgo_comm_unique_id(void *out128);
int cgo_ctx_set_comm_rccl(cgo_ctx *ctx, int32_t rank, int32_t world, const void *unique_id128);
int cgo_ctx_set_comm_callback(cgo_ctx *ctx, int32_t rank, int32_t world, cgo_allgather_fn fn,
                              void *user);
int cgo_ctx_set_comm_shm(cgo_ctx *ctx, int32_t rank, int32_t world, const char *name, int32_t create);
int cgo_shm_unlink(const char *name);
int cgo_ctx_comm_connect_devices(cgo_ctx *ctx, int32_t *connected);
int cgo_ctx_comm_info(cgo_ctx *ctx, int32_t *kind, int32_t *rank, int32_t *world, int32_t *ranks_seen);
int cgo_ctx_exchange_stats(cgo_ctx *ctx, int64_t *exchanges, double *peer_wait_us, double *device_exchange_us,
                           int32_t reset);
int cgo_rccl_available(void);

int cgo_objective_create(cgo_ctx *ctx, int32_t kind, int64_t n_global, int64_t offset,
                         int64_t n_local, cgo_objective **out);
int cgo_objective_create_from_source(cgo_ctx *ctx, const char *source, int32_t has_param,
                                     int64_t n_global, int64_t offset, int64_t n_local,
                                     cgo_objective **out);
#define CGO_MAX_PARAM_SLOTS 4
int cgo_objective_create_from_source_ex(cgo_ctx *ctx, const char *source, int32_t n_params ,
                                        int64_t n_global, int64_t offset, int64_t n_local,
                                        cgo_objective **out);
int cgo_objective_num_params(cgo_objective *obj, int32_t *n_params);
typedef double (*cgo_fdf_fn)(void *user, double *g_local, const double *x_local, int64_t n_local);
int cgo_objective_create_callback(cgo_ctx *ctx, cgo_fdf_fn fn, void *user, int64_t n_global, int64_t offset,
                                  int64_t n_local, cgo_objective **out);
int cgo_objective_destroy(cgo_objective *obj);
int cgo_objective_set_param_host(cgo_objective *obj, int32_t slot, const double *host_local);
int cgo_objective_fill_param(cgo_objective *obj, int32_t slot, int32_t fill_kind, uint64_t seed,
                             double lo, double hi);
int cgo_objective_set_param_device(cgo_objective *obj, int32_t slot, const double *dev_local);
int cgo_objective_set_scalar(cgo_objective *obj, int32_t slot, double value);
int cgo_objective_set_cost_class(cgo_objective *obj, int32_t cost_class);
int cgo_objective_eval_host(cgo_objective *obj, const double *x_local, double *g_local,
                            double *f_global);

typedef struct cgo_solver_policy {
    int32_t size;
    int32_t points;
    int32_t resident;
    int32_t controller_depth;
    int32_t controller_graph;
    int32_t controller_fused;
    int32_t stored_gradient;
    int32_t fused_tail;
    int32_t strict_tail;
    int32_t placement_search;
    int32_t placement_stages;
    int64_t placement_max_bytes;
    int32_t lbfgs_form;
    int32_t lbfgs_fuse_grad;
    int32_t lbfgs_fuse_trial;
    int32_t lse_fixed_reference;
    int32_t resident_points;
    int32_t resident_chunk;
    double hbm_stream_bytes;
    int32_t reserved[8];
} cgo_solver_policy;
void cgo_solver_policy_init(cgo_solver_policy *p);
int cgo_ctx_set_default_policy(cgo_ctx *ctx, const cgo_solver_policy *policy);
int cgo_solver_get_policy(cgo_solver *s, cgo_solver_policy *out);

int cgo_solver_create_ex(cgo_ctx *ctx, cgo_objective *obj, const cgo_cg_config *cfg, const cgo_ls_config *ls,
                         const cgo_solver_policy *policy , cgo_solver **out);
int cgo_solver_create(cgo_ctx *ctx, cgo_objective *obj, const cgo_cg_config *cfg,
                      const cgo_ls_config *ls, cgo_solver **out);
int cgo_solver_destroy(cgo_solver *s);
int cgo_solver_set_x0_host(cgo_solver *s, const double *x0_local);
int cgo_solver_set_x0_fill(cgo_solver *s, int32_t fill_kind, uint64_t seed, double lo, double hi);
int cgo_solver_set_x0_device(cgo_solver *s, const double *x0_dev);
int cgo_solver_start(cgo_solver *s);
int cgo_solver_iterate(cgo_solver *s, int64_t iters, int32_t *finished);
int cgo_solver_results(cgo_solver *s, cgo_results *out);
int cgo_solver_results_device(cgo_solver *s, double *minimizer_dev, double *gradient_dev);
int cgo_solver_trial_log(cgo_solver *s, int64_t cap, double *a, double *phi, double *dphi,
                         int64_t *count);
int cgo_solver_profile_enable(cgo_solver *s, int32_t on);
int cgo_solver_profile_reset(cgo_solver *s);
int cgo_solver_profile_get(cgo_solver *s, int32_t kernel_kind, int64_t *launches,
                           double *total_ms, double *bytes_per_launch);
const char *cgo_kernel_kind_name(int32_t kernel_kind);
const char *cgo_solver_kernel_family(cgo_solver *s);
int64_t cgo_solver_controller_launches(cgo_solver *s);
int cgo_solver_resident_stats(cgo_solver *s, int64_t *slices, int64_t *iterations, int64_t *gave_up);
int cgo_solver_lbfgs_stats(cgo_solver *s, int64_t *speculated, int64_t *fused, int64_t *plain);
int cgo_num_kernel_kinds(void);
int cgo_solver_set_lazy_direction(cgo_solver *s, int32_t on);
int cgo_solver_set_replay_depth(cgo_solver *s, int32_t d);
int cgo_solver_set_lean_sums(cgo_solver *s, int32_t on);
int cgo_solver_kernel_symbol(cgo_solver *s, int32_t kernel_kind, char *buf, int32_t cap);

int cgo_evalwolfeconditions(const cgo_ls_config *ls, double phi_a, double dphi_a, double a, double uu,
                            double phi_0, double dphi_0, int32_t *valid_large, int32_t *valid_small);
int cgo_evalbacktrackcondition(const cgo_ls_config *ls, double phi_a, double a, double phi_0, double dphi_0,
                               int32_t *valid);

typedef struct {
    double rho;
    double sigma;
    double s;
    int64_t max_iters;
} cgo_lss_config;
int cgo_check_lss_config(const cgo_lss_config *ls);
int64_t cgo_lss_default_max_iters(double rho);
int cgo_solver_create_sys(cgo_ctx *ctx, cgo_objective *obj, const cgo_cg_config *cfg,
                          const cgo_lss_config *ls, cgo_solver **out);
int cgo_solver_create_sys_ex(cgo_ctx *ctx, cgo_objective *obj, const cgo_cg_config *cfg, const cgo_lss_config *ls,
                             const cgo_solver_policy *policy , cgo_solver **out);
int cgo_solvesystem(cgo_ctx *ctx, cgo_objective *obj, const double *x0_local,
                    const cgo_cg_config *cfg, const cgo_lss_config *ls, cgo_results *out);

int cgo_minimize(cgo_ctx *ctx, cgo_objective *obj, const double *x0_local,
                 const cgo_cg_config *cfg, const cgo_ls_config *ls, cgo_results *out);
int cgo_minimize_rerun(cgo_ctx *ctx, cgo_objective *obj, const double *x0_local,
                       const cgo_cg_config *cfg, const cgo_ls_config *ls,
                       const cgo_cg_config *rerun_cfgs, const cgo_ls_config *rerun_ls,
                       int32_t npairs, cgo_results *outs, int32_t *nouts);

typedef struct cgo_batch_results {
    double  *objective;
    int64_t *iters_ran;
    int32_t *status;
    int64_t *total_fdf_evals;
    double  *minimizer, *gradient;
    double  *trace_objective, *trace_grad_norm, *trace_step_size;
    int64_t *trace_objective_evals;
    int64_t launches, handed_back;
} cgo_batch_results;
int cgo_minimize_batch(cgo_ctx *ctx, int32_t obj_kind, int64_t n, int64_t batch,
                       const double *x0 , const double *param0 ,
                       const cgo_cg_config *cfg, const cgo_ls_config *ls, int64_t slice_iters ,
                       cgo_batch_results *out);
int64_t cgo_batch_max_n(cgo_ctx *ctx, int32_t obj_kind);
int cgo_minimize_batch_obj(cgo_ctx *ctx, cgo_objective *model, int64_t batch, const double *x0 ,
                           const double *const *params, int32_t n_params,
                           const cgo_cg_config *cfg, const cgo_ls_config *ls, int64_t slice_iters ,
                           cgo_batch_results *out);
int64_t cgo_batch_max_n_obj(cgo_objective *model);
typedef struct cgo_batch cgo_batch;
int cgo_batch_open(cgo_ctx *ctx, cgo_objective *model, int64_t batch, const double *const *params, int32_t n_params,
                   cgo_batch **handle);
int cgo_batch_solve(cgo_batch *handle, const double *x0 , const double *scalars ,
                    const unsigned char *active , const cgo_cg_config *cfg, const cgo_ls_config *ls,
                    int64_t slice_iters , cgo_batch_results *out);
int cgo_batch_close(cgo_batch *handle);
enum { CGO_BATCH_ROWS_LDS = 0, CGO_BATCH_ROWS_DEVICE = 1, CGO_BATCH_ROWS_AUTO = 2 };
typedef struct cgo_batch_policy {
    int32_t size;
    int32_t rows;
    int32_t reserved[6];
} cgo_batch_policy;
void cgo_batch_policy_init(cgo_batch_policy *p);
int cgo_minimize_batch_ex(cgo_ctx *ctx, int32_t obj_kind, int64_t n, int64_t batch, const double *x0, const double *param0,
                          const cgo_cg_config *cfg, const cgo_ls_config *ls, int64_t slice_iters,
                          const cgo_batch_policy *policy, cgo_batch_results *out, int32_t *rows_used);
int cgo_minimize_batch_obj_ex(cgo_ctx *ctx, cgo_objective *model, int64_t batch, const double *x0,
                              const double *const *params, int32_t n_params,
                              const cgo_cg_config *cfg, const cgo_ls_config *ls, int64_t slice_iters,
                              const cgo_batch_policy *policy, cgo_batch_results *out, int32_t *rows_used);
int cgo_batch_open_ex(cgo_ctx *ctx, cgo_objective *model, int64_t batch, const double *const *params, int32_t n_params,
                      const cgo_batch_policy *policy, cgo_batch **handle);
int cgo_batch_rows(const cgo_batch *handle, int32_t *rows_used);
int64_t cgo_batch_max_n_ex(cgo_ctx *ctx, int32_t obj_kind, const cgo_batch_policy *policy);
int64_t cgo_batch_max_n_obj_ex(cgo_objective *model, const cgo_batch_policy *policy);
void cgo_batch_rows_shape(int32_t *block, int32_t *pairs_per_trip);
int cgo_minimize_batch_lbfgs(cgo_ctx *ctx, int32_t obj_kind, int64_t n, int64_t batch, const double *x0, const double *param0,
                             const cgo_cg_config *cfg, const cgo_ls_config *ls, int64_t slice_iters, cgo_batch_results *out);
int32_t cgo_batch_lbfgs_max_m(void);
int64_t cgo_batch_lbfgs_max_n(cgo_ctx *ctx, int32_t obj_kind);
void cgo_batch_lbfgs_shape(int32_t *block, int32_t *pairs_per_trip);
int cgo_minimize_batch_lbfgs_obj(cgo_ctx *ctx, cgo_objective *model, int64_t batch, const double *x0 ,
                                 const double *const *params , int32_t n_params,
                                 const double *scalars ,
                                 const cgo_cg_config *cfg, const cgo_ls_config *ls, int64_t slice_iters, cgo_batch_results *out);
int64_t cgo_batch_lbfgs_max_n_obj(cgo_objective *model);
void cgo_batch_lbfgs_shape_obj(int32_t n_params, int32_t *block, int32_t *pairs_per_trip);
int cgo_minimize_batch_lbfgs_ex(cgo_ctx *ctx, int32_t obj_kind, int64_t n, int64_t batch, const double *x0, const double *param0,
                                const cgo_cg_config *cfg, const cgo_ls_config *ls, int64_t slice_iters,
                                const cgo_batch_policy *policy, cgo_batch_results *out, int32_t *rows_used);
int cgo_minimize_batch_lbfgs_obj_ex(cgo_ctx *ctx, cgo_objective *model, int64_t batch, const double *x0,
                                    const double *const *params, int32_t n_params, const double *scalars,
                                    const cgo_cg_config *cfg, const cgo_ls_config *ls, int64_t slice_iters,
                                    const cgo_batch_policy *policy, cgo_batch_results *out, int32_t *rows_used);
int64_t cgo_batch_lbfgs_max_n_ex(cgo_ctx *ctx, int32_t obj_kind, int32_t m, const cgo_batch_policy *policy);
int64_t cgo_batch_lbfgs_max_n_obj_ex(cgo_objective *model, int32_t m, const cgo_batch_policy *policy);
int32_t cgo_batch_lbfgs_lds_rows(int32_t n_params, int32_t m);
void cgo_batch_lbfgs_lds_shape(int32_t n_params, int32_t *block, int32_t *pairs_per_trip);
int cgo_batch_lbfgs_open(cgo_ctx *ctx, cgo_objective *model, int64_t batch, const double *const *params, int32_t n_params,
                         int32_t m_max, const cgo_batch_policy *policy , cgo_batch **handle);
int cgo_batch_lbfgs_solve(cgo_batch *handle, const double *x0 , const double *scalars ,
                          const unsigned char *active , const cgo_cg_config *cfg, const cgo_ls_config *ls,
                          int64_t slice_iters , cgo_batch_results *out);
int cgo_batch_lbfgs_m(const cgo_batch *handle, int32_t *m_max);
#define CGO_BATCH_PROBE_MAX_PASSES 32
typedef struct cgo_batch_pass {
    int32_t kind, k;
    double a[7];
    double a_acc, beta;
    int32_t co_set, co_count;
    double co_gamma, co_cy[10], co_cs[10];
} cgo_batch_pass;
typedef struct cgo_batch_pass_out {
    double ts[7][7];
    double gu, uu;
    int64_t width, stored;
} cgo_batch_pass_out;
typedef struct cgo_batch_probe_args {
    int32_t tier, obj_kind, m, n_params;
    cgo_objective *model;
    int64_t n, batch;
    const double *x, *u;
    const double *params[4];
    const double *scalars;
    const unsigned char *skip;
    const double *S, *Y;
    const void *qn;
    int32_t npass, reserved;
    cgo_batch_pass pass[CGO_BATCH_PROBE_MAX_PASSES];
    double *rows;
    cgo_batch_pass_out *out;
    double *x_out, *u_out, *g_out, *S_out, *Y_out;
    void *qn_out;
    int32_t *reason;
    int64_t *done, *passes;
    int32_t points, reserved2;
    int64_t ld;
    char symbol[128];
} cgo_batch_probe_args;
int cgo_batch_probe(cgo_ctx *ctx, cgo_batch_probe_args *p);
int64_t cgo_batch_probe_qn_bytes(void);
int cgo_solver_set_path_prediction(cgo_solver *s, int32_t on);
int cgo_solver_path_stats(cgo_solver *s, int64_t *by_nact, int64_t *predicted, int64_t *tree, int64_t *misses);
int cgo_solver_probe_set_path(cgo_solver *s, int32_t nact);
int cgo_solver_debug_set_path_skew(cgo_solver *s, double factor);
int32_t cgo_stop_status(int64_t it, int64_t max_iters, double f_x, double grad_norm, double eps, double f_x0, int64_t *iters_ran);

int cgo_kernel_dir(cgo_ctx *ctx, double *u, const double *g, double beta, int64_t n,
                   double *out2);
int cgo_kernel_beta_partials(cgo_ctx *ctx, const double *g_next, const double *g,
                             const double *u, int64_t n, double *out9);
int cgo_getbeta(cgo_ctx *ctx, const cgo_beta_config *b, const double *g_next, const double *g,
                const double *u, int64_t n, double *beta);
int cgo_kernel_trial(cgo_objective *obj, const double *x, const double *u, double a,
                     double *g_next_out, double *out2);
int cgo_solver_probe_set_beta_prev(cgo_solver *s, double beta_prev);
int cgo_solver_probe_set_replay(cgo_solver *s, int32_t nrep, const double *a, const double *beta);
int cgo_solver_probe_launch(cgo_solver *s, int32_t kernel_kind, int32_t variant, double a_acc, double beta,
                            const double *a, int32_t k,
                            const double *x, const double *u, const double *aux,
                            double *sums, int32_t sums_cap, int32_t *sums_len,
                            double *x_out, double *u_out, double *g_out,
                            char *symbol, int32_t symbol_cap);
typedef struct cgo_lbfgs_probe {
    int32_t pass, slot, count, list[16];
    double a, a_s, a_trial, cg, M, S;
    double cy[16], cs[16];
    int32_t deferred_push, lite_slot;
    double a_lite, a_s_lite, M_lite, S_lite;
    int32_t loop_mode, final_step, apply_scale, k, q_from_g, v_ring, v_slot, w_ring, w_slot, dot_count;
    double rho, scale, dot_host;
    const double *dots;
    double alpha[64];
    int32_t spec_check, spec_slot, spec_count, spec_list[16];
    double spec_a_x, spec_a_s;
    int32_t spec_ok, new_in_list, sums_len, reserved;
    double gram[85];
    double sums[64];
    char symbol[256];
} cgo_lbfgs_probe;
int cgo_solver_probe_lbfgs(cgo_solver *s, cgo_lbfgs_probe *p,
                           const double *x, const double *u, const double *g, const double *gt, const double *S, const double *Y,
                           double *x_out, double *xo_out, double *u_out, double *g_out, double *gt_out, double *S_out, double *Y_out);
#define CGO_RESIDENT_PROBE_MAX_PASSES 32
typedef struct cgo_resident_pass {
    int32_t kind, k;
    double a[7];
    double a_acc, beta;
} cgo_resident_pass;
typedef struct cgo_resident_pass_out {
    double ts[7][7];
    double gu, uu;
    int64_t width;
} cgo_resident_pass_out;
typedef struct cgo_resident_probe {
    int32_t npass, reserved;
    cgo_resident_pass pass[CGO_RESIDENT_PROBE_MAX_PASSES];
    int32_t grid, points;
    int64_t chunk, round0;
    uint32_t err_word;
    int32_t wrote_back;
    cgo_resident_pass_out out[CGO_RESIDENT_PROBE_MAX_PASSES];
    char symbol[128];
} cgo_resident_probe;
int cgo_solver_probe_resident(cgo_solver *s, cgo_resident_probe *p, const double *x, const double *u,
                              double *rows, int64_t rows_cap, double *x_out, double *u_out);
#define CGO_ARMED_PROBE_MAX_ROUNDS 32
typedef struct cgo_ctl_state {
    double f_x, gg, a_acc, beta, a[7];
    int32_t npts, go;
    int64_t it;
} cgo_ctl_state;
typedef struct cgo_ctl_args {
    double a_acc, beta, a[7];
    int64_t go;
} cgo_ctl_args;
typedef struct cgo_ctl_record {
    double sums[56], a_acc, beta, a[7];
    int32_t npts, accepted;
    int64_t xwait;
} cgo_ctl_record;
typedef struct cgo_armed_probe {
    int32_t rounds, form, use_eps, reserved;
    int64_t max_iters;
    double eps;
    cgo_ctl_state st;
    double row[56];
    int32_t width, maxp;
    uint64_t round_out;
    cgo_ctl_state st_out;
    cgo_ctl_args args_out;
    double out_dev[56];
    cgo_ctl_record rec[CGO_ARMED_PROBE_MAX_ROUNDS];
    char symbol[4096];
} cgo_armed_probe;
int cgo_solver_probe_armed(cgo_solver *s, cgo_armed_probe *p, const double *x, const double *u, double *x_out, double *u_out);
int cgo_bench_kernel(cgo_ctx *ctx, cgo_objective *obj, int32_t kernel_kind, int64_t n,
                     int32_t reps, double *ms_per_launch, double *bytes_per_launch);

int cgo_bench_stream_mix(cgo_ctx *ctx, int64_t n, int32_t reps, double *median_us, double *best_us);
int cgo_solver_placement_info(cgo_solver *s, double *as_allocated_us, double *chosen_us, int32_t *candidates);

#ifdef __cplusplus
}
#endif
#endif
```

Before: 2295.

## Deepen lazy replay list to 16 steps with deep trial kernel

Lets the lazy-direction replay list grow past the old cap of seven steps, up to fifteen. A second parameter block holds the extra steps and is staged into shared memory, and a new deep trial kernel replays the whole list before evaluating the trial points. Materialization now runs in chunks, the default replay depth for large diagonal quadratics goes from 8 to 12, and replay statistics counters are added. The aim is fewer full-vector store passes of x and u per iteration over HBM, paid for with more recomputation per element and more kernel variants.

New measurement: 2363, median of 6. 3.0% higher.

```diff
diff --git a/conjugategradientoptim.jl_amd/_lib.py b/conjugategradientoptim.jl_amd/_lib.py
--- a/conjugategradientoptim.jl_amd/_lib.py
+++ b/conjugategradientoptim.jl_amd/_lib.py
@@ -200,6 +200,8 @@
     "cgo_solver_probe_set_path": (C.c_int, [_vp, C.c_int32]),
     "cgo_solver_debug_set_path_skew": (C.c_int, [_vp, C.c_double]),
     "cgo_solver_probe_set_replay": (C.c_int, [_vp, C.c_int32, dp, dp]),
+    "cgo_solver_probe_set_deep_trial": (C.c_int, [_vp, C.c_int32]),
+    "cgo_solver_replay_stats": (C.c_int, [_vp, i64p, i64p, i64p, i64p, i64p, i64p, C.POINTER(C.c_int32)]),
     "cgo_solver_kernel_symbol": (C.c_int, [_vp, C.c_int32, C.c_char_p, C.c_int32]),
     "cgo_evalwolfeconditions": (C.c_int, [C.POINTER(LSConfigC), C.c_double, C.c_double, C.c_double, C.c_double,
                                           C.c_double, C.c_double, C.POINTER(C.c_int32), C.POINTER(C.c_int32)]),
diff --git a/conjugategradientoptim.jl_amd/api.py b/conjugategradientoptim.jl_amd/api.py
--- a/conjugategradientoptim.jl_amd/api.py
+++ b/conjugategradientoptim.jl_amd/api.py
@@ -664,6 +664,12 @@
     def set_replay_depth(self, d: int):
         check(_lib.lib().cgo_solver_set_replay_depth(self._h, int(d)))
 
+    def replay_stats(self):
+        v = [C.c_int64(0) for _ in range(6)]
+        mx = C.c_int32(0)
+        check(_lib.lib().cgo_solver_replay_stats(self._h, *[C.byref(q) for q in v], C.byref(mx)))
+        return dict(zip(("n", "s", "t", "m", "t_deep", "m_deep"), (q.value for q in v)), max_list=mx.value)
+
     def set_lean_sums(self, on: bool):
         check(_lib.lib().cgo_solver_set_lean_sums(self._h, int(bool(on))))
 
@@ -680,7 +686,8 @@
         check(_lib.lib().cgo_solver_debug_set_path_skew(self._h, float(factor)))
 
     def probe_launch(self, kind_name: str, variant: int, a_acc: float, beta: float, a: Sequence[float], x, u=None, aux=None,
-                     beta_prev: Optional[float] = None, replay: Optional[Sequence] = None, path_nact: Optional[int] = None):
+                     beta_prev: Optional[float] = None, replay: Optional[Sequence] = None, path_nact: Optional[int] = None,
+                     deep_trial: bool = False):
         L = _lib.lib()
         kk = [L.cgo_kernel_kind_name(k).decode() for k in range(L.cgo_num_kernel_kinds())].index(kind_name)
         if beta_prev is not None:
@@ -691,6 +698,8 @@
             check(L.cgo_solver_probe_set_replay(self._h, len(replay), ra.ctypes.data_as(dp), rb.ctypes.data_as(dp)))
         if path_nact is not None:
             check(L.cgo_solver_probe_set_path(self._h, int(path_nact)))
+        if deep_trial:
+            check(L.cgo_solver_probe_set_deep_trial(self._h, 1))
         n = self.obj.n_local
         vec = lambda v: None if v is None else np.ascontiguousarray(v, dtype=np.float64)
         x, u, aux = vec(x), vec(u), vec(aux)
diff --git a/conjugategradientoptim.jl_amd/csrc/cgo_backend_cg.hip b/conjugategradientoptim.jl_amd/csrc/cgo_backend_cg.hip
--- a/conjugategradientoptim.jl_amd/csrc/cgo_backend_cg.hip
+++ b/conjugategradientoptim.jl_amd/csrc/cgo_backend_cg.hip
@@ -51,9 +51,16 @@
 }
 
 template <class Obj>
-static int launch_cg_path(int mode, int nact, const RParams &P, int grid, hipStream_t st) {
-#define ROW(MODE, NACT) if (mode == (MODE) && nact == (NACT)) { k_cg_path<Obj, (MODE), (NACT), true><<<grid, BLOCK, 0, st>>>(P); return 0; }
+static int launch_cg_path(int mode, int nact, const RParams &P, const RDeep &Q, int grid, hipStream_t st) {
+#define ROW(MODE, NACT) if (mode == (MODE) && nact == (NACT)) { k_cg_path<Obj, (MODE), (NACT), true><<<grid, BLOCK, 0, st>>>(P, Q); return 0; }
     CGO_CG_PATH_ROWS(ROW)
+#undef ROW
+    return -1;
+}
+template <class Obj>
+static int launch_cg_deep_t(int npts, const RParams &P, const RDeep &Q, int grid, hipStream_t st) {
+#define ROW(NPTS) if (npts == (NPTS)) { k_cg_trial_deep<Obj, (NPTS), true><<<grid, BLOCK, 0, st>>>(P, Q); return 0; }
+    CGO_CG_DEEP_T_ROWS(ROW)
 #undef ROW
     return -1;
 }
@@ -68,6 +75,9 @@
     CGO_OBJ_CURV_ROWS(ROW)
 #undef ROW
     return false;
+}
+bool HipBackend::deep_trial(int mode) const {
+    return mode == (R_REPLAY | R_TRIAL) && !path_nact_ && path_objective(obj_->kind) && (rep_n_ > RMAX || deep_t_);
 }
 bool HipBackend::path_rows() const {
     if (!path_on_ || !path_objective(obj_->kind) || replay_depth_ < 2 || !lazy_eligible()) return false;
@@ -111,6 +121,7 @@
         else if (mode & (R_INIT | R_RESET)) u_lag_ = false;
     }
     if (rep_n_ > 0 && !(mode & R_REPLAY)) { if (int rc = materialize_lag()) return rc; }
+    if (rep_n_ > RMAX && (mode & R_REPLAY) && r_base(mode) != R_REPLAY && !path_nact_ && !deep_trial(mode)) { if (int rc = materialize_lag()) return rc; }
     RPlan plan;
     const int npts = path_nact_ ? MAXP : npts_for(k);
     if (int rc = launch_r_kernel(kk, mode, a_acc, beta, a, k, npts, nullptr, &plan)) return rc;
@@ -174,27 +185,35 @@
 
 int HipBackend::materialize_lag() {
     if (int rc = materialize_u()) return rc;
-    if (rep_n_ == 0) return CGO_OK;
     const int64_t asked = total_launches_;
     const int nact = path_nact_;
     path_nact_ = 0;
-    const int rc = launch_rk(KK_MATERIALIZE_XU, 0.0, 0.0, nullptr, 0, false, nullptr);
+    int rc = CGO_OK;
+    while (rep_n_ > 0 && rc == CGO_OK) {
+        const int all = rep_n_, take = std::min(all, (int)RMAX);
+        rep_n_ = take;
+        rc = launch_rk(KK_MATERIALIZE_XU, 0.0, 0.0, nullptr, 0, false, nullptr);
+        rep_n_ = all;
+        if (rc) break;
+        rstats_.m++;
+        if (all > RMAX) rstats_.m_deep++;
+        for (int j = take; j < all; ++j) { rep_a_[j - take] = rep_a_[j]; rep_b_[j - take] = rep_b_[j]; }
+        rep_n_ = all - take;
+    }
     path_nact_ = nact;
     total_launches_ = asked;
-    if (rc) return rc;
-    rep_n_ = 0;
-    return CGO_OK;
+    return rc;
 }
 
 int HipBackend::set_replay_depth_now(int d) {
-    if (d < 1 || d > RMAX + 1) { set_error("replay depth: 1 … 8"); return CGO_EINVAL; }
+    if (d < 1 || d > RCAP + 1) { set_error("replay depth: 1 … 16"); return CGO_EINVAL; }
     if (d != replay_depth_) { if (int rc = materialize_lag()) return rc; }
     replay_depth_ = d;
     return CGO_OK;
 }
 
 void HipBackend::set_probe_replay(int nrep, const double *a, const double *beta) {
-    probe_rep_n_ = std::max(0, std::min(nrep, (int)RMAX));
+    probe_rep_n_ = std::max(0, std::min(nrep, (int)RCAP));
     for (int j = 0; j < probe_rep_n_; ++j) { probe_rep_a_[j] = a[j]; probe_rep_b_[j] = beta[j]; }
 }
 
@@ -202,17 +221,19 @@
     if (!lazy_eligible()) return launch_rk(KK_ACCEPT_DIR_TRIAL, a_acc, beta, a, k, true, s);
     if (replay_depth_ >= 2) {
         if (int rc = materialize_u()) return rc;
-        if (rep_n_ < replay_depth_ - 1 && rep_n_ < RMAX) {
+        if (rep_n_ < replay_depth_ - 1 && rep_n_ < (path_nact_ ? RCAP : RMAX)) {
             const int mode_n = r_mode_of(KK_ACCEPT_TRIAL_NOSTORE);
             if (int rc = launch_r(KK_ACCEPT_TRIAL_NOSTORE, mode_n | lean_for(mode_n), a_acc, beta, a, k, true, s)) return rc;
             if (path_nact_) { path_last_n_ = path_nact_; path_count_[path_nact_]++; }
             rep_a_[rep_n_] = a_acc; rep_b_[rep_n_] = beta; rep_n_++;
+            rstats_.n++;
             return CGO_OK;
         }
         const int mode_s = R_REPLAY | R_ADT;
         if (int rc = launch_r(KK_ACCEPT_DIR_TRIAL, mode_s | lean_for(mode_s), a_acc, beta, a, k, true, s)) return rc;
         if (path_nact_) { path_last_s_ = path_nact_; path_count_[path_nact_]++; }
         rep_n_ = 0;
+        rstats_.s++;
         return CGO_OK;
     }
     if (!u_lag_) {
@@ -225,7 +246,11 @@
     return CGO_OK;
 }
 int HipBackend::trial_r(const double *a, int k, double *s) {
-    if (rep_n_ > 0 && lazy_eligible()) return launch_r(KK_TRIAL, R_REPLAY | R_TRIAL, 0, 0, a, k, true, s);
+    if (rep_n_ > 0 && lazy_eligible()) {
+        rstats_.t++;
+        if (rep_n_ > RMAX) rstats_.t_deep++;
+        return launch_r(KK_TRIAL, R_REPLAY | R_TRIAL, 0, 0, a, k, true, s);
+    }
     if (u_lag_ && lazy_eligible()) return launch_r(KK_TRIAL, R_ULAG | R_TRIAL, 0, 0, a, k, true, s);
     return launch_rk(KK_TRIAL, 0, 0, a, k, true, s);
 }
@@ -258,7 +283,8 @@
     const bool has_sums = r_has_sums(mode);
     const RPlan plan = *plan_out = r_plan(mode, npts);
     const bool big = plan.big; const int grid = plan.grid;
-    last_mode_ = mode; last_npts_ = plan.npts; last_big_ = big; last_nact_ = path_nact_;
+    const bool deep_t = deep_trial(mode);
+    last_mode_ = mode; last_npts_ = plan.npts; last_big_ = big; last_nact_ = deep_t ? -1 : path_nact_;
     if (path_nact_ && (chain() || !big || ctl || !path_row(mode, path_nact_) || !path_objective(obj_->kind))) { set_error("internal: not a path row"); return CGO_EINVAL; }
     if (chain()) {
         if (int rc = prof_begin(kk)) return rc;
@@ -270,8 +296,14 @@
     P.xo = xc_; P.uo = uc_;
     P.a_acc = a_acc; P.beta = beta; P.s0 = obj_->s0; P.partials = ctx_->partials;
     P.beta_prev = beta_lag_;
-    P.nrep = (mode & R_REPLAY) ? rep_n_ : 0;
+    const int nrep = (mode & R_REPLAY) ? rep_n_ : 0;
+    if (nrep > RCAP || (nrep > RMAX && !path_nact_ && !deep_t)) { set_error("internal: more replayed steps than the launch takes"); return CGO_ESTATE; }
+    P.nrep = std::min(nrep, (int)RMAX);
     for (int j = 0; j < RMAX; ++j) { P.ra[j] = j < P.nrep ? rep_a_[j] : 0.0; P.rb[j] = j < P.nrep ? rep_b_[j] : 0.0; }
+    RDeep Q;
+    Q.nrep2 = nrep - P.nrep;
+    for (int j = 0; j < RDEEP; ++j) { Q.ra2[j] = j < Q.nrep2 ? rep_a_[RMAX + j] : 0.0; Q.rb2[j] = j < Q.nrep2 ? rep_b_[RMAX + j] : 0.0; }
+    rstats_.max_list = std::max(rstats_.max_list, nrep);
     P.ctl = ctl;
     P.x2 = xn_;
     for (int j = 0; j < MAXP; ++j) P.a[j] = (a && j < k) ? a[j] : ((a && k > 0) ? a[k - 1] : 0.0);
@@ -296,7 +328,15 @@
     int r = -2;
     if (path_nact_) {
         switch (obj_->kind) {
-#define ROW(KIND, T) case KIND: r = launch_cg_path<T>(mode, path_nact_, P, grid, st); break;
+#define ROW(KIND, T) case KIND: r = launch_cg_path<T>(mode, path_nact_, P, Q, grid, st); break;
+        CGO_OBJ_CURV_ROWS(ROW)
+#undef ROW
+        default: break;
+        }
+    } else if (deep_t) {
+        if (!big) { set_error("internal: not a deep trial row"); return CGO_EINVAL; }
+        switch (obj_->kind) {
+#define ROW(KIND, T) case KIND: r = launch_cg_deep_t<T>(plan.npts, P, Q, grid, st); break;
         CGO_OBJ_CURV_ROWS(ROW)
 #undef ROW
         default: break;
@@ -354,6 +394,7 @@
 std::string HipBackend::r_symbol(int mode, int npts, bool big, int nact) const {
     char buf[160];
     if (chain()) snprintf(buf, sizeof buf, "k_chain<%d, %d, %s>", mode, npts, big ? "true" : "false");
+    else if (nact < 0) snprintf(buf, sizeof buf, "k_cg_trial_deep<%s, %d, true>", obj_tname(), npts);
     else if (nact) snprintf(buf, sizeof buf, "k_cg_path<%s, %d, %d, true>", obj_tname(), mode, nact);
     else snprintf(buf, sizeof buf, "k_cg<%s, %d, %d, %s>", obj_tname(), mode, npts, big ? "true" : "false");
     return buf;
@@ -375,12 +416,14 @@
     case KK_ACCEPT_TRIAL_NOSTORE: case KK_MATERIALIZE_XU: if (!lazy || replay_depth_ < 2) return ""; break;
     default: break;
     }
+    if (kk == KK_TRIAL && lazy && rep_n_ > RMAX) mode |= R_REPLAY;
     const RPlan plan = r_plan(mode, rk->pts == PTS_ONE ? 1 : npts_for(rk->pts == PTS_MAX ? max_points() : std::min(max_points(), 3)));
     if ((mode & R_REPLAY) && (mode & R_ACCEPT)) mode |= lean_for(mode);
     if ((mode & R_REPLAY) && (mode & R_ACCEPT) && path_rows()) {
         const int last = kk == KK_ACCEPT_TRIAL_NOSTORE ? path_last_n_ : path_last_s_;
         return r_symbol(mode, plan.npts, plan.big, last ? last : MAXP);
     }
+    if (kk == KK_TRIAL && deep_trial(mode)) return r_symbol(mode, plan.npts, plan.big, -1);
     return r_symbol(mode, plan.npts, plan.big);
 }
 
@@ -725,6 +768,8 @@
     *sums_len = 0;
     const int want_nact = probe_nact_;
     probe_nact_ = 0;
+    const bool want_deep = probe_deep_t_;
+    probe_deep_t_ = false;
     const bool lse = obj_->two_phase();
     if (k < 0 || k > MAXP || (k > 0 && !a)) { set_error("probe: 0 ≤ k ≤ 7 trial steps"); return CGO_EINVAL; }
     if (!rmode_ && !lse) return probe_launch_stored(kk, variant, a_acc, beta, a, k, x, u, aux, sums, sums_cap, sums_len, x_out, u_out, g_out, symbol);
@@ -795,12 +840,18 @@
         symbol = buf;
     } else {
         double s[64];
+        if (want_deep && (mode != (R_REPLAY | R_TRIAL) || want_nact || !path_objective(obj_->kind))) { rep_n_ = 0; set_error("probe: not a deep trial launch of this solver"); return CGO_EINVAL; }
+        if (rep_n_ > RMAX && !want_nact && !(mode == (R_REPLAY | R_TRIAL) && path_objective(obj_->kind))) {
+            rep_n_ = 0; set_error("probe: more than 7 replayed steps: path rows and the deep trial launch only"); return CGO_EINVAL;
+        }
+        deep_t_ = want_deep;
         if (want_nact) {
             if (!path_row(mode, want_nact) || !path_objective(obj_->kind) || k > want_nact) { rep_n_ = 0; set_error("probe: not a path row of this solver, or more steps than it evaluates"); return CGO_EINVAL; }
             path_nact_ = want_nact;
         }
         rc = launch_r(kk, mode, a_acc, beta, a, k, true, s);
         path_nact_ = 0;
+        deep_t_ = false;
         rep_n_ = 0;
         if (rc) return rc;
         symbol = r_symbol(last_mode_, last_npts_, last_big_, last_nact_);
diff --git a/conjugategradientoptim.jl_amd/csrc/cgo_capi.hip b/conjugategradientoptim.jl_amd/csrc/cgo_capi.hip
--- a/conjugategradientoptim.jl_amd/csrc/cgo_capi.hip
+++ b/conjugategradientoptim.jl_amd/csrc/cgo_capi.hip
@@ -338,7 +338,7 @@
     API_GUARD_END
 }
 
-static const int kReplayDepth = 8;
+static const int kReplayDepth = 12;
 static const bool kLeanSums = true;
 static const bool kPathPredict = true;
 static int env_tri(const char *name) { const char *e = getenv(name); return e ? (e[0] != '0' ? 1 : 0) : -1; }
@@ -480,7 +480,7 @@
     {
         int depth = 1;
         if (obj->o.kind == CGO_OBJ_QUAD_DIAG && 8.0 * (double)obj->o.n_local * 5.0 > 1.4e9) depth = kReplayDepth;
-        if (const char *e = getenv("CGO_REPLAY_DEPTH")) { const int v = atoi(e); if (v >= 1 && v <= 8) depth = v; }
+        if (const char *e = getenv("CGO_REPLAY_DEPTH")) { const int v = atoi(e); if (v >= 1 && v <= 16) depth = v; }
         s->be->set_replay_depth(depth);
     }
     {
@@ -712,8 +712,24 @@
 int cgo_solver_set_replay_depth(cgo_solver *s, int32_t d) {
     API_GUARD_BEGIN
     REQUIRE(s, "null argument");
-    REQUIRE(d >= 1 && d <= 8, "replay depth: 1 … 8");
+    REQUIRE(d >= 1 && d <= 16, "replay depth: 1 … 16");
     return s->be->set_replay_depth_now(d);
+    API_GUARD_END
+}
+
+int cgo_solver_replay_stats(cgo_solver *s, int64_t *n, int64_t *s_launches, int64_t *t, int64_t *m, int64_t *t_deep, int64_t *m_deep,
+                            int32_t *max_list) {
+    API_GUARD_BEGIN
+    REQUIRE(s, "null argument");
+    const auto &r = s->be->replay_stats();
+    if (n) *n = r.n;
+    if (s_launches) *s_launches = r.s;
+    if (t) *t = r.t;
+    if (m) *m = r.m;
+    if (t_deep) *t_deep = r.t_deep;
+    if (m_deep) *m_deep = r.m_deep;
+    if (max_list) *max_list = r.max_list;
+    return CGO_OK;
     API_GUARD_END
 }
 
@@ -768,8 +784,16 @@
 int cgo_solver_probe_set_replay(cgo_solver *s, int32_t nrep, const double *a, const double *beta) {
     API_GUARD_BEGIN
     REQUIRE(s, "null argument");
-    REQUIRE(nrep >= 0 && nrep <= 7 && (nrep == 0 || (a && beta)), "probe replay list: 0 … 7 (a*, β) pairs");
+    REQUIRE(nrep >= 0 && nrep <= 15 && (nrep == 0 || (a && beta)), "probe replay list: 0 … 15 (a*, β) pairs (more than 7: path rows and the deep trial launch)");
     s->be->set_probe_replay(nrep, a, beta);
+    return CGO_OK;
+    API_GUARD_END
+}
+
+int cgo_solver_probe_set_deep_trial(cgo_solver *s, int32_t on) {
+    API_GUARD_BEGIN
+    REQUIRE(s, "null argument");
+    s->be->set_probe_deep_trial(on != 0);
     return CGO_OK;
     API_GUARD_END
 }
diff --git a/conjugategradientoptim.jl_amd/csrc/cgo_hip_backend.hpp b/conjugategradientoptim.jl_amd/csrc/cgo_hip_backend.hpp
--- a/conjugategradientoptim.jl_amd/csrc/cgo_hip_backend.hpp
+++ b/conjugategradientoptim.jl_amd/csrc/cgo_hip_backend.hpp
@@ -215,10 +215,13 @@
     bool lazy_direction() const { return lazy_on_; }
     int set_lazy_direction_now(bool on) { if (!on) { if (int rc = materialize_lag()) return rc; } lazy_on_ = on; return 0; }
     void set_probe_beta_prev(double b) { probe_beta_prev_ = b; }
-    void set_replay_depth(int d) { replay_depth_ = d < 1 ? 1 : (d > 8 ? 8 : d); }
+    void set_replay_depth(int d) { replay_depth_ = d < 1 ? 1 : (d > 16 ? 16 : d); }
     int replay_depth() const { return replay_depth_; }
     int set_replay_depth_now(int d);
     void set_probe_replay(int nrep, const double *a, const double *beta);
+    void set_probe_deep_trial(bool on) { probe_deep_t_ = on; }
+    struct ReplayStats { int64_t n = 0, s = 0, t = 0, m = 0, t_deep = 0, m_deep = 0; int max_list = 0; };
+    const ReplayStats &replay_stats() const { return rstats_; }
     void set_beta_unread(int bits) { lean_mask_ = bits; if (lean_bits_) lean_bits_ = bits; }
     void set_lean_sums(bool on) { lean_bits_ = on ? lean_mask_ : 0; }
     bool lean_sums() const { return lean_bits_ != 0; }
@@ -317,7 +320,10 @@
     bool lazy_eligible() const;
     int materialize_u();
     int replay_depth_ = 1, rep_n_ = 0, probe_rep_n_ = 0;
-    double rep_a_[7] = {}, rep_b_[7] = {}, probe_rep_a_[7] = {}, probe_rep_b_[7] = {};
+    double rep_a_[15] = {}, rep_b_[15] = {}, probe_rep_a_[15] = {}, probe_rep_b_[15] = {};
+    bool probe_deep_t_ = false, deep_t_ = false;
+    bool deep_trial(int mode) const;
+    ReplayStats rstats_;
     int materialize_lag();
     int lean_mask_ = 0, lean_bits_ = 0;
     int lean_for(int mode) const;
diff --git a/conjugategradientoptim.jl_amd/csrc/cgo_kernels_cg_path.hip.hpp b/conjugategradientoptim.jl_amd/csrc/cgo_kernels_cg_path.hip.hpp
--- a/conjugategradientoptim.jl_amd/csrc/cgo_kernels_cg_path.hip.hpp
+++ b/conjugategradientoptim.jl_amd/csrc/cgo_kernels_cg_path.hip.hpp
@@ -17,9 +17,23 @@
            (mode & R_NOYY) != 0;
 }
 
-template <class Obj, int MODE, int NACT>
-__device__ inline void cg_path_pair(const RParams &P, d2 &x, d2 &u, const PV<Obj> &p, double (&acc)[RW<MAXP>::W], bool &wx, bool &wu) {
-    constexpr int R_GU = RW<MAXP>::GU, R_UU = RW<MAXP>::UU;
+constexpr int RDEEP = 8;
+constexpr int RCAP = RMAX + RDEEP;
+struct RDeep {
+    int nrep2;
+    double ra2[RDEEP], rb2[RDEEP];
+};
+struct RDeepLds { double a[RDEEP], b[RDEEP]; };
+__device__ inline void rdeep_stage(const RDeep &Q, RDeepLds &L) {
+    if (threadIdx.x == 0) {
+#pragma unroll
+        for (int j = 0; j < RDEEP; ++j) { L.a[j] = Q.ra2[j]; L.b[j] = Q.rb2[j]; }
+    }
+    __syncthreads();
+}
+
+template <class Obj>
+__device__ inline void replay_pair(const RParams &P, const RDeep &Q, const RDeepLds &L, d2 &x, d2 &u, const PV<Obj> &p) {
 #pragma unroll
     for (int j = 0; j < RMAX; ++j) {
         if (j < P.nrep) {
@@ -31,6 +45,42 @@
             u.x = -gr.x + P.rb[j] * u.x; u.y = -gr.y + P.rb[j] * u.y;
         }
     }
+#pragma nounroll
+    for (int j = 0; j < Q.nrep2; ++j) {
+        const double ra = L.a[j], rb = L.b[j];
+        d2 gr;
+        double fr = 0.0;
+        x.x = x.x + ra * u.x;
+        x.y = x.y + ra * u.y;
+        obj_eval2<Obj>(x, p, P.s0, fr, gr);
+        u.x = -gr.x + rb * u.x; u.y = -gr.y + rb * u.y;
+    }
+}
+template <class Obj>
+__device__ inline void replay_single(const RParams &P, const RDeep &Q, const RDeepLds &L, double &x, double &u, const PS<Obj> &p) {
+#pragma unroll
+    for (int j = 0; j < RMAX; ++j) {
+        if (j < P.nrep) {
+            double gr = 0.0, fr = 0.0;
+            x = x + P.ra[j] * u;
+            obj_eval1<Obj>(x, p, P.s0, fr, gr);
+            u = -gr + P.rb[j] * u;
+        }
+    }
+#pragma nounroll
+    for (int j = 0; j < Q.nrep2; ++j) {
+        const double ra = L.a[j], rb = L.b[j];
+        double gr = 0.0, fr = 0.0;
+        x = x + ra * u;
+        obj_eval1<Obj>(x, p, P.s0, fr, gr);
+        u = -gr + rb * u;
+    }
+}
+
+template <class Obj, int MODE, int NACT>
+__device__ inline void cg_path_pair(const RParams &P, const RDeep &Q, const RDeepLds &L, d2 &x, d2 &u, const PV<Obj> &p, double (&acc)[RW<MAXP>::W], bool &wx, bool &wu) {
+    constexpr int R_GU = RW<MAXP>::GU, R_UU = RW<MAXP>::UU;
+    replay_pair<Obj>(P, Q, L, x, u, p);
     x.x = x.x + P.a_acc * u.x;
     x.y = x.y + P.a_acc * u.y;
     wx = r_writes_x(MODE);
@@ -66,20 +116,12 @@
 }
 
 template <class Obj, int MODE, int NACT>
-__device__ inline void cg_path_single(const RParams &P, long long i, double (&acc)[RW<MAXP>::W]) {
+__device__ inline void cg_path_single(const RParams &P, const RDeep &Q, const RDeepLds &L, long long i, double (&acc)[RW<MAXP>::W]) {
     constexpr int R_GU = RW<MAXP>::GU, R_UU = RW<MAXP>::UU;
     double x = P.x[i];
     double u = P.u[i];
     const PS<Obj> p = ps_load<Obj>(P, i);
-#pragma unroll
-    for (int j = 0; j < RMAX; ++j) {
-        if (j < P.nrep) {
-            double gr = 0.0, fr = 0.0;
-            x = x + P.ra[j] * u;
-            obj_eval1<Obj>(x, p, P.s0, fr, gr);
-            u = -gr + P.rb[j] * u;
-        }
-    }
+    replay_single<Obj>(P, Q, L, x, u, p);
     x = x + P.a_acc * u;
     if (r_writes_x(MODE)) P.xo[i] = x;
     double g = 0.0, f0 = 0.0;
@@ -104,7 +146,7 @@
 }
 
 template <class Obj, int MODE, int NACT, bool BIG>
-__global__ __launch_bounds__(BLOCK) void k_cg_path(const RParams P) {
+__global__ __launch_bounds__(BLOCK) void k_cg_path(const RParams P, const RDeep Q) {
     static_assert(BIG, "path launches exist as pure-HBM streams only");
     static_assert(path_mode(MODE), "a path row is launch N or S of the replay cycle in a lean form that leaves the y·y slot free");
     static_assert(NACT >= 1 && NACT <= MAXP, "1 … 7 of the row's seven points");
@@ -112,6 +154,8 @@
     double acc[W];
 #pragma unroll
     for (int s = 0; s < W; ++s) acc[s] = 0.0;
+    __shared__ RDeepLds L;
+    rdeep_stage(Q, L);
     const long long n2 = P.n >> 1;
     const long long per = big_chunk_pairs(n2, gridDim.x);
     long long i = per * blockIdx.x + threadIdx.x;
@@ -122,8 +166,8 @@
         d2 ua = ldg2<true>(P.u, i), ub = ldg2<true>(P.u, i + step);
         const PV<Obj> pa = pv_load<Obj, true>(P, i), pb = pv_load<Obj, true>(P, i + step);
         bool wxa = false, wua = false, wxb = false, wub = false;
-        cg_path_pair<Obj, MODE, NACT>(P, xa, ua, pa, acc, wxa, wua);
-        cg_path_pair<Obj, MODE, NACT>(P, xb, ub, pb, acc, wxb, wub);
+        cg_path_pair<Obj, MODE, NACT>(P, Q, L, xa, ua, pa, acc, wxa, wua);
+        cg_path_pair<Obj, MODE, NACT>(P, Q, L, xb, ub, pb, acc, wxb, wub);
         if (wxa) stg2<true>(P.xo, i, xa);
         if (wua) stg2<true>(P.uo, i, ua);
         if (wxb) stg2<true>(P.xo, i + step, xb);
@@ -134,11 +178,11 @@
         d2 ua = ldg2<true>(P.u, i);
         const PV<Obj> pa = pv_load<Obj, true>(P, i);
         bool wxa = false, wua = false;
-        cg_path_pair<Obj, MODE, NACT>(P, xa, ua, pa, acc, wxa, wua);
+        cg_path_pair<Obj, MODE, NACT>(P, Q, L, xa, ua, pa, acc, wxa, wua);
         if (wxa) stg2<true>(P.xo, i, xa);
         if (wua) stg2<true>(P.uo, i, ua);
     }
-    if ((P.n & 1) && blockIdx.x == 0 && threadIdx.x == 0) cg_path_single<Obj, MODE, NACT>(P, P.n - 1, acc);
+    if ((P.n & 1) && blockIdx.x == 0 && threadIdx.x == 0) cg_path_single<Obj, MODE, NACT>(P, Q, L, P.n - 1, acc);
     if constexpr (LateF<Obj, MODE>::on) {
 #pragma unroll
         for (int j = 0; j < NACT; ++j) acc[RS_PER_POINT * j + RS_F] *= ObjFScale<Obj>::scale;
@@ -146,5 +190,83 @@
     store_partials_n<W, false>(acc, P.partials, P.tail);
 }
 
-}
-}
+template <class Obj, int NPTS>
+__device__ inline void cg_trial_points2(const RParams &P, const d2 &x, const d2 &u, const PV<Obj> &p, double (&acc)[RW<NPTS>::W]) {
+    d2 g;
+    double f0 = 0.0;
+    obj_eval2<Obj>(x, p, P.s0, f0, g);
+#pragma unroll
+    for (int j = 0; j < NPTS; ++j) {
+        const int b = RS_PER_POINT * j;
+        d2 xp, gt;
+        xp.x = x.x + P.a[j] * u.x;
+        xp.y = x.y + P.a[j] * u.y;
+        obj_term2<Obj, false>(xp, p, P.s0, acc[b + RS_F], gt);
+        const double y0 = gt.x - g.x, y1 = gt.y - g.y;
+        acc[b + RS_GTU] = dsum(acc[b + RS_GTU], gt.x, u.x);   acc[b + RS_GTU] = dsum(acc[b + RS_GTU], gt.y, u.y);
+        acc[b + RS_GTGT] = dsum(acc[b + RS_GTGT], gt.x, gt.x); acc[b + RS_GTGT] = dsum(acc[b + RS_GTGT], gt.y, gt.y);
+        acc[b + RS_GTG] = dsum(acc[b + RS_GTG], gt.x, g.x);   acc[b + RS_GTG] = dsum(acc[b + RS_GTG], gt.y, g.y);
+        acc[b + RS_YY] = dsum(acc[b + RS_YY], y0, y0);       acc[b + RS_YY] = dsum(acc[b + RS_YY], y1, y1);
+        acc[b + RS_UY] = dsum(acc[b + RS_UY], u.x, y0);      acc[b + RS_UY] = dsum(acc[b + RS_UY], u.y, y1);
+        acc[b + RS_YGT] = dsum(acc[b + RS_YGT], y0, gt.x);    acc[b + RS_YGT] = dsum(acc[b + RS_YGT], y1, gt.y);
+    }
+}
+
+template <class Obj, int NPTS, bool BIG>
+__global__ __launch_bounds__(BLOCK) void k_cg_trial_deep(const RParams P, const RDeep Q) {
+    static_assert(BIG, "replay launches exist as pure-HBM streams only");
+    static_assert(NPTS == 1 || NPTS == 3 || NPTS == 5 || NPTS == 7, "a launch evaluates 1, 3, 5 or 7 trial points");
+    constexpr int W = RW<NPTS>::W;
+    double acc[W];
+#pragma unroll
+    for (int s = 0; s < W; ++s) acc[s] = 0.0;
+    __shared__ RDeepLds L;
+    rdeep_stage(Q, L);
+    const long long n2 = P.n >> 1;
+    const long long per = big_chunk_pairs(n2, gridDim.x);
+    long long i = per * blockIdx.x + threadIdx.x;
+    const long long hi = (per * blockIdx.x + per < n2) ? per * blockIdx.x + per : n2;
+    const long long step = BLOCK;
+    for (; i + step < hi; i += 2 * step) {
+        d2 xa = ldg2<true>(P.x, i), xb = ldg2<true>(P.x, i + step);
+        d2 ua = ldg2<true>(P.u, i), ub = ldg2<true>(P.u, i + step);
+        const PV<Obj> pa = pv_load<Obj, true>(P, i), pb = pv_load<Obj, true>(P, i + step);
+        replay_pair<Obj>(P, Q, L, xa, ua, pa);
+        cg_trial_points2<Obj, NPTS>(P, xa, ua, pa, acc);
+        replay_pair<Obj>(P, Q, L, xb, ub, pb);
+        cg_trial_points2<Obj, NPTS>(P, xb, ub, pb, acc);
+    }
+    if (i < hi) {
+        d2 xa = ldg2<true>(P.x, i);
+        d2 ua = ldg2<true>(P.u, i);
+        const PV<Obj> pa = pv_load<Obj, true>(P, i);
+        replay_pair<Obj>(P, Q, L, xa, ua, pa);
+        cg_trial_points2<Obj, NPTS>(P, xa, ua, pa, acc);
+    }
+    if ((P.n & 1) && blockIdx.x == 0 && threadIdx.x == 0) {
+        const long long e = P.n - 1;
+        double x = P.x[e];
+        double u = P.u[e];
+        const PS<Obj> p = ps_load<Obj>(P, e);
+        replay_single<Obj>(P, Q, L, x, u, p);
+        double g = 0.0, f0 = 0.0;
+        obj_eval1<Obj>(x, p, P.s0, f0, g);
+#pragma unroll
+        for (int j = 0; j < NPTS; ++j) {
+            const int b = RS_PER_POINT * j;
+            const double xp = x + P.a[j] * u;
+            double gt;
+            obj_term1<Obj, false>(xp, p, P.s0, acc[b + RS_F], gt);
+            const double y = gt - g;
+            acc[b + RS_GTU] = dsum(acc[b + RS_GTU], gt, u); acc[b + RS_GTGT] = dsum(acc[b + RS_GTGT], gt, gt);
+            acc[b + RS_GTG] = dsum(acc[b + RS_GTG], gt, g);
+            acc[b + RS_YY] = dsum(acc[b + RS_YY], y, y);
+            acc[b + RS_UY] = dsum(acc[b + RS_UY], u, y);
+            acc[b + RS_YGT] = dsum(acc[b + RS_YGT], y, gt);
+        }
+    }
+    store_partials_n<W, false>(acc, P.partials, P.tail);
+}
+
+}
+}
diff --git a/include/cgo.h b/include/cgo.h
--- a/include/cgo.h
+++ b/include/cgo.h
@@ -228,6 +228,8 @@
 int cgo_num_kernel_kinds(void);
 int cgo_solver_set_lazy_direction(cgo_solver *s, int32_t on);
 int cgo_solver_set_replay_depth(cgo_solver *s, int32_t d);
+int cgo_solver_replay_stats(cgo_solver *s, int64_t *n, int64_t *s_launches, int64_t *t, int64_t *m, int64_t *t_deep, int64_t *m_deep,
+                            int32_t *max_list);
 int cgo_solver_set_lean_sums(cgo_solver *s, int32_t on);
 int cgo_solver_kernel_symbol(cgo_solver *s, int32_t kernel_kind, char *buf, int32_t cap);
 
@@ -386,6 +388,7 @@
                      double *g_next_out, double *out2);
 int cgo_solver_probe_set_beta_prev(cgo_solver *s, double beta_prev);
 int cgo_solver_probe_set_replay(cgo_solver *s, int32_t nrep, const double *a, const double *beta);
+int cgo_solver_probe_set_deep_trial(cgo_solver *s, int32_t on);
 int cgo_solver_probe_launch(cgo_solver *s, int32_t kernel_kind, int32_t variant, double a_acc, double beta,
                             const double *a, int32_t k,
                             const double *x, const double *u, const double *aux,
```
